# haidog-yaqub/EzAudio

Hardware: AMD Instinct MI355X
Metric: denoising steps/sec (EzAudio-XL, 10 s latent, CFG on) (higher is better)
Workload: dtype bf16

## Files before the change

ezaudio_amd/build.py:

```python
import concurrent.futures
import os
import subprocess
import sys

HERE = os.path.dirname(os.path.abspath(__file__))
CSRC = os.path.join(HERE, 'csrc')
OBJ = os.path.join(HERE, 'csrc', 'build')
LIB = os.path.join(HERE, 'libezaudio_hip.so')
SOURCES = ['gemm.hip', 'attn.hip', 'rowops.hip', 'api.hip', 'vae.hip', 't5.hip']
FLAGS = ['--offload-arch=gfx950', '-O3', '-std=c++17', '-fPIC', '-Wall', '-Wno-unused-function']
if os.environ.get('EZAUDIO_ABLATE'):
    FLAGS.append('-DEZ_ABLATE')
if os.environ.get('EZAUDIO_DIAG'):
    FLAGS.append('-DEZ_DIAG')


def source_hash():
    import hashlib
    h = hashlib.sha256()
    files = sorted(os.path.join(CSRC, f) for f in os.listdir(CSRC) if f.endswith(('.hip', '.h')))
    files.append(os.path.join(HERE, '..', 'include', 'ezdit.h'))
    for f in files:
        h.update(os.path.basename(f).encode())
        with open(f, 'rb') as fh:
            h.update(fh.read())
    return h.hexdigest()[:16]


def _hipcc():
    for cand in (os.environ.get('HIPCC'), '/opt/rocm/bin/hipcc', 'hipcc'):
        if cand and (os.path.isabs(cand) and os.path.exists(cand) or not os.path.isabs(cand)):
            return cand
    raise RuntimeError('hipcc not found')


def _stale(target, deps):
    if not os.path.exists(target):
        return True
    t = os.path.getmtime(target)
    return any(os.path.getmtime(d) > t for d in deps)


def build(force=False, verbose=True):
    os.makedirs(OBJ, exist_ok=True)
    headers = [os.path.join(CSRC, f) for f in sorted(os.listdir(CSRC)) if f.endswith('.h')] + [os.path.join(HERE, '..', 'include', 'ezdit.h')]
    hipcc = _hipcc()
    jobs = []
    for src in SOURCES:
        s = os.path.join(CSRC, src)
        o = os.path.join(OBJ, src.replace('.hip', '.o'))
        if force or _stale(o, [s] + headers):
            jobs.append((s, o))

    def compile_one(job):
        s, o = job
        cmd = [hipcc] + FLAGS + ['-c', s, '-o', o]
        r = subprocess.run(cmd, capture_output=True, text=True)
        return job, r

    if jobs:
        with concurrent.futures.ThreadPoolExecutor(max_workers=len(jobs)) as ex:
            for (s, o), r in ex.map(compile_one, jobs):
                if verbose and r.stderr.strip():
                    sys.stderr.write(r.stderr)
                if r.returncode != 0:
                    raise RuntimeError(f'hipcc failed on {s}:\n{r.stderr}')
    objs = [os.path.join(OBJ, s.replace('.hip', '.o')) for s in SOURCES]
    if force or jobs or _stale(LIB, objs):
        cmd = [hipcc, '--offload-arch=gfx950', '-shared', '-fPIC', '-o', LIB] + objs
        r = subprocess.run(cmd, capture_output=True, text=True)
        if r.returncode != 0:
            raise RuntimeError(f'link failed:\n{r.stderr}')
    return LIB


if __name__ == '__main__':
    print(build(force='--force' in sys.argv))
```

ezaudio_amd/csrc/api.hip:

```cpp
#include "../../include/ezdit.h"
#include "common.h"

#include <cmath>
#include <cstdarg>
#include <cstdio>
#include <cstring>
#include <map>
#include <string>
#include <vector>

static thread_local std::string g_err;

int ez_fail(int code, const char* fmt, ...) {
    char buf[512];
    va_list ap;
    va_start(ap, fmt);
    vsnprintf(buf, sizeof buf, fmt, ap);
    va_end(ap);
    g_err = buf;
    return code;
}
#define fail ez_fail

namespace {

#define HIPCHK(expr)                                                                            \
    do {                                                                                        \
        hipError_t e_ = (expr);                                                                 \
        if (e_ != hipSuccess) return fail(EZDIT_E_HIP, "%s failed: %s", #expr, hipGetErrorString(e_)); \
    } while (0)

inline long rup(long x, long a) { return (x + a - 1) / a * a; }

struct Buf {
    size_t off = 0, bytes = 0;
};

}

struct WRef {
    const bf16_t* W = nullptr; int ld = 0; int rows = 0;
};
struct BlkW {
    const float *bskip, *aqnw, *aqnb, *aknw, *aknb, *bo, *n2w, *n2b, *cqnw, *cqnb, *bo2, *b1, *b2, *snw, *snb, *zb;
    WRef wskip, wqkv, wo, wq2, wo2, w1, w2, zw;
};
struct WsPtrs {
    int* ints; float *rope_cos, *rope_sin, *coef, *cfgpart;
    bf16_t* ape; float *h, *skips; bf16_t *u, *ucat; float* qkv; bf16_t *q, *k, *v, *ao, *act; float *part, *y, *pred;
    uint8_t* kmask; bf16_t *kc, *vc; float *mod, *modf;
    float *cembed, *cnres; bf16_t* skipbf;
    float2* zstat; float *zt_qkv, *zt_geglu, *zt_q2;
    float2* zstat_skip; float* zt_skip; bf16_t* ucat_z;
    float* spc;
    float* zd;
};

static void drop_graph(ezdit_handle* h);

template <typename T>
struct Table {
    bool on = false;
    std::vector<T> host;
    T* dev = nullptr;
    const T* read() const { return on ? dev : nullptr; }
    void set(ezdit_handle* owner, bool to, bool rearm = false) {
        if (to != on || (to && rearm)) drop_graph(owner);
        on = to;
    }
};

static unsigned long long* g_gemm_ts = nullptr;
static long g_gemm_ts_cap = 0;

struct ezdit_handle {
    ezdit_config cfg;
    int D, H, dh, nblk, nhalf, I, C, Cin, Cctx, r6;
    int DQK, DV;
    int ldD, ld2D, ldI, ldPE, ldCtx;
    float scaling;

    std::vector<ezdit_param_info_t> params;
    std::map<std::string, int> pidx;
    size_t param_bytes = 0;
    const char* wblob = nullptr;

    char* ws = nullptr;
    size_t ws_bytes = 0;
    int B = 0, L = 0, Lc = 0, n_slots = 0, M = 0, Mp = 0, Lp = 0, Lcp = 0, Mc = 0;
    std::map<std::string, Buf> bufs;
    bool ctx_ready = false, ts_ready = false, cond_ready = false;
    bool z_tables_ready = false;
    bool skip_tables_ready = false;
    int n_ts = 0, per_row = 0;

    float* latents = nullptr;
    const float* noise = nullptr;
    const float* s_gt = nullptr;
    const uint8_t* s_gt_mask = nullptr;
    int P = 0, n_steps = 0;
    float gscale = 0.f, grescale = 0.f;
    hipGraphExec_t graph_exec = nullptr;
    hipGraph_t graph = nullptr;

    Table<int> lens;
    const int* lens_dev() const { return lens.read(); }
    Table<float> cns;
    Table<float> tl;
    int2* tlsup = nullptr;
    int tl_S = 0;
    Table<float> sp;
    static int sp_cap(int B) { return B / 2 + 1; }
    Table<float> coef;
    float* ms_hist = nullptr;
    Table<int> start;
    int start_min = 0;
    Table<int> canvas;
    int canvas_T = 0, canvas_ramp = 1;
    bool canvas_loop = false;
    Table<float> cw;
    int cw_K = 1;

    int launches = 0;
    bool is_cn = false;
    int c0 = 0, c0m = 0, c1 = 0;
    ezdit_handle* cn = nullptr;
    float cn_scale = 1.0f;
    float fwd_cn_scale = 1.0f;
    std::vector<ezdit_handle*> cn_users;
    const float* ext_mask_embed = nullptr;
    static constexpr int kSplitK = 3, kTileF32 = 25, kTilePE = 70, kTileFin = 73;
    static constexpr int kTilePartialBig = 60, kSplitBig = 2, kZTile = 70, kZBigM = 2048;
    int opt_tile_partial = 9;
    int opt_gemm_pp = 3;
    int opt_zfuse = 1;
    int opt_skip_z = 1;
    bool skip_z_usable() const { return opt_skip_z && !is_cn && nhalf > 0 && zparts() <= (ztile() == kZTile ? 16 : 8); }
    int opt_geglu_co = 0;
    int opt_qkv_co = 1;
    int opt_qkv_form = 1;
    int qkv_tile() const { return (opt_qkv_co == 2 || (opt_qkv_co == 1 && M > kCoM)) ? 66 : (opt_qkv_form == 1 && M <= kCoM) ? 67 : 61; }
    static constexpr int kCoM = 2048;
    int geglu_tile() const { return !(opt_gemm_pp & 1) ? 13 : (opt_geglu_co == 2 || (opt_geglu_co == 1 && M > kCoM)) ? 66 : 60; }
    int opt_xkey1 = 1;
    bool xkey1 = false;
    int act_b0 = 0, act_b1 = 0;
#ifdef EZ_DIAG
    int opt_zfake = 0;
#endif
    bool qk_perm() const { return D % (2 * dh) == 0; }
    int qkv_mode() const { return qk_perm() ? 2 : 0; }
    bool q2_fused(int nb) const { return opt_fuse_q2 && ((long)nb * H * ((L + 63) / 64) <= 512 || opt_fuse_q2 == 2) && Lcp % 128 == 0; }
    bool zfuse_usable() const {
        return opt_zfuse && zparts() <= Z_MAXP && (opt_gemm_pp & 1) && qkv_mode() == 2 && (q2_fused(B) || opt_q2_pp);
    }
    int ztile() const { return (M > kZBigM && !per_row) ? 61 : kZTile; }
    int zwidth() const { return ztile() == 61 ? 144 : 96; }
    int zparts() const { return (D + zwidth() - 1) / zwidth(); }
    struct ZTab { float *G, *C; long slot_stride; };
    static long ztab_floats(int items, long N) { return (long)items * 2 * N; }
    static ZTab ztab(float* base, int item, long N, long slot_stride) { float* G = base + ztab_floats(item, N); return {G, G + N, slot_stride}; }
    ZTab zt_qkv_of(int b) const { return ztab(p.zt_qkv, b, 3L * D, ztab_floats(nblk, 3L * D)); }
    ZTab zt_geglu_of(int b) const { return ztab(p.zt_geglu, b, 2L * I, ztab_floats(nblk, 2L * I)); }
    ZTab zt_q2_of(int b) const { return ztab(p.zt_q2, b, D, 0); }
    ZTab zt_skip_of(int j) const { return ztab(p.zt_skip, j, D, 0); }
    static size_t zrange(long Mp_) { return (size_t)Z_MAXP * Mp_; }
    float2* zstat_xhalf() const { return p.zstat + zrange(Mp); }
    float2* zstat_skip_of(int i) const { return p.zstat_skip + (size_t)i * zrange(Mp); }
    size_t ucat_elems(long Mp_) const { return (size_t)Mp_ * ld2D; }
    bf16_t* ucat_of(int j) const { return p.ucat_z + (size_t)j * ucat_elems(Mp); }
    int opt_wt = 2;
    int wt() const { return opt_wt == 2 ? (B * L <= 2048) : opt_wt; }
    int opt_fuse_q2 = 1;
    int opt_attn_nkh = 0;
    int opt_q2_pp = 1;
// ... 116 lines not shown
        const long c0 = h->c0, c0m = h->c0m, c1 = h->c1, ci = h->cfg.cond_in;
        add_param(h, "cn.cin.w", {"controlnet_pre.conv_in.weight"}, F, c0, ci);
        add_param(h, "cn.cin.b", {"controlnet_pre.conv_in.bias"}, F, 1, c0);
        if (h->cfg.cond_mask) add_param(h, "cn.mask_embed", {"controlnet_pre.mask_embed"}, F, 1, c0);
        add_param(h, "cn.c0.w", {"controlnet_pre.blocks.0.0.weight"}, F, c0m, c0m * 3);
        add_param(h, "cn.c0.b", {"controlnet_pre.blocks.0.0.bias"}, F, 1, c0m);
        add_param(h, "cn.c1.w", {"controlnet_pre.blocks.0.2.weight"}, F, c1, c0m * 3);
        add_param(h, "cn.c1.b", {"controlnet_pre.blocks.0.2.bias"}, F, 1, c1);
        add_param(h, "cn.cout.w", {"controlnet_pre.conv_out.weight"}, F, D, c1);
        add_param(h, "cn.cout.b", {"controlnet_pre.conv_out.bias"}, F, 1, D);
        for (int b = 0; b < h->nblk; ++b) {
            char k[64];
            snprintf(k, sizeof k, "controlnet_zero_blocks.%d", b);
            add_param(h, bn(b, "zw"), {std::string(k) + ".weight"}, Bf, D, D);
            add_param(h, bn(b, "zb"), {std::string(k) + ".bias"}, F, 1, D);
        }
    }
    struct V { const char* name; const char* key; long n; };
    const V vecs[] = {
        {"n1w", "norm1.weight", D}, {"n1b", "norm1.bias", D}, {"n2w", "norm2.weight", D}, {"n2b", "norm2.bias", D},
        {"n3w", "norm3.weight", D}, {"n3b", "norm3.bias", D}, {"ncw", "norm_context.weight", D},
        {"ncb", "norm_context.bias", D},
        {"a.qnw", "attn.norm_q.weight", dh}, {"a.qnb", "attn.norm_q.bias", dh}, {"a.knw", "attn.norm_k.weight", dh},
        {"a.knb", "attn.norm_k.bias", dh}, {"c.qnw", "cross_attn.norm_q.weight", dh},
        {"c.qnb", "cross_attn.norm_q.bias", dh}, {"c.knw", "cross_attn.norm_k.weight", dh},
        {"c.knb", "cross_attn.norm_k.bias", dh},
        {"bo", "attn.proj.bias", D}, {"bo2", "cross_attn.proj.bias", D}, {"b2", "mlp.net.2.bias", D},
        {"table", "adaln.scale_shift_table", 6 * D},
    };
    for (const V& v : vecs)
        for (int b = 0; b < h->nblk; ++b) add_param(h, bn(b, v.name), {blk_prefix(h, b) + "." + v.key}, F, 1, v.n);
    for (int b = 0; b < h->nblk; ++b) {
        const std::string p = blk_prefix(h, b);
        add_param(h, bn(b, "b1"), {p + ".mlp.net.0.proj.bias"}, F, 1, 2 * I, EZDIT_T_GEGLU8);
        if (b > h->nhalf) {
            add_param(h, bn(b, "snw"), {p + ".skip_norm.weight"}, F, 1, 2 * D);
            add_param(h, bn(b, "snb"), {p + ".skip_norm.bias"}, F, 1, 2 * D);
            add_param(h, bn(b, "wskip"), {p + ".skip_linear.weight"}, Bf, D, 2 * D);
            add_param(h, bn(b, "bskip"), {p + ".skip_linear.bias"}, F, 1, D);
        }
        add_param(h, bn(b, "wqkv"), {p + ".attn.to_q.weight", p + ".attn.to_k.weight", p + ".attn.to_v.weight"}, Bf, 3 * D, D, h->qk_perm() ? EZDIT_T_QKROPE : EZDIT_T_NONE);
        add_param(h, bn(b, "wo"), {p + ".attn.proj.weight"}, Bf, D, D);
        add_param(h, bn(b, "wq2"), {p + ".cross_attn.to_q.weight"}, Bf, D, D);
        add_param(h, bn(b, "wo2"), {p + ".cross_attn.proj.weight"}, Bf, D, D);
        add_param(h, bn(b, "w1"), {p + ".mlp.net.0.proj.weight"}, Bf, 2 * I, D, EZDIT_T_GEGLU8);
        add_param(h, bn(b, "w2"), {p + ".mlp.net.2.weight"}, Bf, D, I);
    }
    for (int b = 0; b < h->nblk; ++b) {
        const std::string p = blk_prefix(h, b);
        add_param(h, bn(b, "wkv2"), {p + ".cross_attn.to_k.weight", p + ".cross_attn.to_v.weight"}, Bf, 2 * D, D);
        add_param(h, bn(b, "lora_a"), {p + ".adaln.lora_a.weight"}, F, r6, D);
        add_param(h, bn(b, "lora_b"), {p + ".adaln.lora_b.weight"}, F, 6 * D, r6);
    }
}

size_t carve(const ezdit_handle* h, int B, int L, int Lc, int n_slots, std::map<std::string, Buf>* out) {
    size_t off = 0;
    auto add = [&](const char* name, size_t bytes) {
        Buf b;
        b.off = off;
        b.bytes = bytes;
        if (out) (*out)[name] = b;
        off += (size_t)rup((long)bytes, 256);
    };
    const long D = h->D, C = h->C, H = h->H;
    const long M = (long)B * L, Mp = rup(M, 128), Lp = rup(L, 128), Lcp = rup(Lc, 128);
    const long Mc = (long)B * Lc, Mcp = rup(Mc, 128);
    const int nblk = h->nblk;
    add("ints", 256 * sizeof(int));
    add("rope_cos", (size_t)h->cfg.max_len * (h->dh / 2) * 4);
    add("rope_sin", (size_t)h->cfg.max_len * (h->dh / 2) * 4);
    add("coef", (size_t)(n_slots > 0 ? n_slots : 1) * 8 * 4);
    add("cfgpart", (size_t)B * 64 * 4 * 4);
    add("sink", 256);
    if (h->is_cn) {
        const long Lc2 = 2L * L;
        add("cn_e0", (size_t)B * h->c0 * Lc2 * 4);
        add("cn_e1", (size_t)B * h->c0m * Lc2 * 4);
        add("cn_e2", (size_t)B * h->c1 * L * 4);
        add("cembed", (size_t)rup((long)B * L, 128) * h->D * 4);
        add("cnres", (size_t)h->nhalf * rup((long)B * L, 128) * h->D * 4);
        add("skipbf", (size_t)rup((long)B * L, 128) * h->ldD * 2);
    }
    add("ape", Mp * h->ldPE * 2);
    add("h", Mp * D * 4);
    add("skips", (size_t)h->nhalf * Mp * D * 4);
    add("u", Mp * h->ldD * 2);
    add("ucat", Mp * h->ld2D * 2);
    add("qkv", Mp * 3 * D * 4);
    add("q", (size_t)B * H * Lp * h->DQK * 2);
    add("k", (size_t)B * H * Lp * h->DQK * 2);
    add("v", (size_t)B * H * Lp * h->DV * 2);
    add("ao", Mp * h->ldD * 2);
    add("act", Mp * h->ldI * 2);
    add("part", (size_t)8 * Mp * D * 4);
    add("y", Mp * C * 4);
    add("pred", (size_t)B * C * L * 4);
    add("kmask", rup(Mc, 256));
    add("ctx_bf", Mcp * h->ldCtx * 2);
    add("c1", Mcp * D * 4);
    add("c1b", Mcp * h->ldD * 2);
    add("c2", Mcp * D * 4);
    add("cu", Mcp * h->ldD * 2);
    add("ckv", Mcp * 2 * D * 4);
    add("kc", (size_t)nblk * B * H * Lcp * h->DQK * 2);
    add("vc", (size_t)nblk * B * H * Lcp * h->DV * 2);
    const long ns = n_slots > 0 ? n_slots : 1;
    add("ts", ns * 4);
    add("t1", ns * D * 4);
    add("tt", ns * D * 4);
    add("ada", ns * 6 * D * 4);
    add("adaf", ns * 2 * D * 4);
    add("la", ns * h->r6 * 4);
    add("lora", ns * nblk * 6 * D * 4);
    add("mod", ns * nblk * 6 * D * 4);
    add("modf", ns * 2 * D * 4);
    {
        const long I2 = 2L * h->I, N3 = 3L * D, nmax = I2 > N3 ? I2 : N3;
        const size_t zr = ezdit_handle::zrange(Mp), z64 = (size_t)Mp * ((2 * D + 63) / 64), nskip = h->nhalf > 0 ? h->nhalf : 1;
        add("zstat", (z64 > 2 * zr ? z64 : 2 * zr) * 8);
        add("zt_qkv", (size_t)ns * ezdit_handle::ztab_floats(nblk, N3) * 4);
        add("zt_geglu", (size_t)ns * ezdit_handle::ztab_floats(nblk, I2) * 4);
        add("zt_q2", (size_t)ezdit_handle::ztab_floats(nblk, D) * 4);
        add("zd", (size_t)nblk * B * D * 4);
        add("zA", (size_t)rup(4 * ns, 128) * h->ldD * 2);
        add("ztmp", (size_t)rup(4 * ns, 128) * nmax * 4);
#ifdef EZ_DIAG
        add("zneutral", zr * 8);
        add("zzeros", (size_t)nmax * 4);
#endif
        add("ucat_z", (h->is_cn ? 1 : nskip) * h->ucat_elems(Mp) * 2);
        add("zstat_skip", nskip * zr * 8);
        add("zt_skip", (size_t)ezdit_handle::ztab_floats((int)nskip, D) * 4);
        add("lens", 256 * sizeof(int));
        add("spg", (size_t)ezdit_handle::sp_cap(B) * 2 * 4);
        add("spc", (size_t)ns * ezdit_handle::sp_cap(B) * 8 * 4);
        add("cns", 256 * sizeof(float));
        add("start", 256 * sizeof(int));
        add("canvas", 256 * sizeof(int));
        add("tlb", (size_t)B * (Lcp / 128) * L * 4);
        add("tlsup", (size_t)B * (Lcp / 128) * 8);
        add("cw", (size_t)B * sizeof(float));
    }
    return off;
}

struct Ctx {
    ezdit_handle* h;
    hipStream_t st;
    const int* cur = nullptr; const int* row_slot = nullptr;
    hipError_t err = hipSuccess;
    int rc = EZDIT_OK;
    const char* where = nullptr;
    unsigned long long* stamps() const { return (g_gemm_ts && h->launches == h->opt_stamp_launch) ? g_gemm_ts : nullptr; }
    void launched(const char* what, int launch_rc = 0) {
        if (h->opt_trace_launches) fprintf(stderr, "launch %d %s\n", h->launches, what);
        h->launches++;
        if (launch_rc != 0 && rc == EZDIT_OK) { rc = launch_rc; where = what; }
        const hipError_t e = hipGetLastError();
        if (e != hipSuccess && err == hipSuccess) { err = e; where = what; }
    }
    bool bad() const { return err != hipSuccess || rc != EZDIT_OK; }
    int result() const {
        if (rc != EZDIT_OK) return fail(rc, "%s: configuration not supported by the HIP kernels", where ? where : "?");
        if (err != hipSuccess) return fail(EZDIT_E_HIP, "launch of %s failed: %s", where ? where : "?", hipGetErrorString(err));
        return EZDIT_OK;
    }
};

struct ZIn {
    ezdit_handle::ZTab t{};
    const float2* stat = nullptr;
    int row0 = 0, b0 = 0;
};

void gemm(Ctx& c, const bf16_t* A, int lda, const WRef& w, const float* bias, void* out, int ldo, int M, int N,
          int epi, int tile, const HeadNormArgs* hn = nullptr, const ZIn& z = ZIn{}, int splitk = 1, long slab = 0, bool panel = false) {
    ezdit_handle* h = c.h;
    GemmArgs g;
    memset(&g, 0, sizeof g);
    g.A = A;
    g.lda = lda;
    g.W = w.W;
    g.ldw = w.ld;
    g.wrows = w.rows;
    g.bias = bias;
    g.out = out;
    g.ldo = ldo;
    g.slab_stride = slab;
    g.M = M;
    g.N = N;
    g.K = w.ld;
    g.splitk = splitk;
    g.epi = epi;
    g.tile = tile;
    g.xcd_map = 1;
    g.part_bf16 = (epi == EPI_PARTIAL) ? 1 : 0;
    g.wt = h->wt();
    g.epi_lds = h->opt_epi_lds;
    g.rows_per_b = 1;
    if (hn) g.hn = *hn;
    g.xcd_panel = panel ? 1 : 0;
#ifdef EZ_DIAG
    if (!z.stat && h->opt_zfake && (epi == EPI_QKV || epi == EPI_GEGLU) && (tile == 60 || tile == 61 || tile == 66) && h->zparts() <= Z_MAXP) {
        g.zw = h->zwidth(); g.zstat_in = h->buf<float2>("zneutral"); g.zs_stride = h->Mp; g.zparts = h->zparts(); g.zD = h->D;
        g.zG = h->buf<float>("zzeros"); g.zC = bias ? bias : g.zG; g.zt_slot_stride = 0; g.zeps = 1e-5f; g.rows_per_b = h->L;
    }
#endif
    if (z.stat) {
        g.zw = h->zwidth(); g.zstat_in = z.stat + z.row0; g.zs_stride = h->Mp; g.zparts = h->zparts(); g.zD = h->D; g.zG = z.t.G; g.zC = z.t.C; g.zt_slot_stride = z.t.slot_stride; g.zeps = 1e-5f;
        g.cur_step = c.cur ? c.cur : h->p.ints; g.row_slot = c.cur ? c.row_slot : (h->per_row ? h->p.ints + 16 : nullptr); g.rows_per_b = h->L;
        if (g.row_slot) g.row_slot += z.b0;
    }
    g.ts = c.stamps(); g.ts_cap = g_gemm_ts_cap;
    c.launched(epi == EPI_GEGLU ? "k_gemm (GEGLU)" : epi == EPI_QKV ? "k_gemm (QKV)" : epi == EPI_PARTIAL ? "k_gemm (split-K slabs)" : "k_gemm", launch_gemm(g, c.st));
}

int tile_for(const ezdit_handle* h, int M, bool partial) {
    if (M <= 2048) return partial ? h->opt_tile_partial : ezdit_handle::kTileF32;
    return partial ? ezdit_handle::kTilePartialBig : ezdit_handle::kTileF32;
}

int pick_splitk(const ezdit_handle* h, int M, int N, int K) {
    const int tiles = ((M + 127) / 128) * ((N + 63) / 64);
    const int nk = K / 64;
    if (M > 2048) return ezdit_handle::kSplitBig < nk ? ezdit_handle::kSplitBig : nk;
    if (tiles >= 256) return 1;
    return ezdit_handle::kSplitK < nk ? ezdit_handle::kSplitK : nk;
}

int gemm_partial(Ctx& c, const bf16_t* A, int lda, const WRef& w, int M, int N) {
    ezdit_handle* h = c.h;
    const int K = w.ld;
    const int s = pick_splitk(h, M, N, K);
    const int shape_bit = K >= 4 * N ? 4 : K >= 2 * N ? 2 : 1;
    const bool panel = (h->opt_gemm_panel & shape_bit) && M <= 1024;
    gemm(c, A, lda, w, nullptr, h->p.part, h->D, M, N, EPI_PARTIAL, tile_for(h, M, true), nullptr, ZIn{}, s, (long)h->Mp * h->D, panel);
    return s;
}

GemmArgs resid_args(int tile, const bf16_t* A, int lda, const bf16_t* W, int ldw, int wrows, const float* bias, const float* h_in, const float* gate, const float* zg,
                    float* h_out, bf16_t* zu, int ld_zu, float2* zstat_out, long zs_stride, int M, int N, int K) {
    GemmArgs g;
    memset(&g, 0, sizeof g);
    g.A = A; g.lda = lda; g.W = W; g.ldw = ldw; g.wrows = wrows; g.bias = bias;
    g.out = h_out; g.ldo = N; g.M = M; g.N = N; g.K = K; g.splitk = 1; g.epi = EPI_RESID; g.tile = tile; g.xcd_map = 1;
    g.resid = h_in; g.ldr = N; g.gate = gate; g.rows_per_b = 1;
    g.zu = zu; g.ld_zu = ld_zu; g.zg = zg; g.zstat_out = zstat_out; g.zs_stride = zs_stride;
    return g;
}

struct Edge {
    const char* name = nullptr;
    bool algebra = false;
    const bf16_t* A = nullptr; int lda = 0; const WRef* w = nullptr; const float* bias = nullptr;
    const float* h_in = nullptr; float* h_out = nullptr;
    const float* gate = nullptr; long gate_stride = 0;
    const float *ln_g = nullptr, *ln_c = nullptr; long ln_stride = 0;
    int b0 = 0, nb = -1;
    int dual_blk = -1;
    bf16_t* zu = nullptr; int ld_zu = 0;
    float2* zstat_out = nullptr;
    bf16_t* zu2 = nullptr; int ld_zu2 = 0; const float* zg2 = nullptr;
    const float2 *zin = nullptr, *zin2 = nullptr; const float* zG = nullptr;
    const float *skip = nullptr, *cn = nullptr;
};

void resolve_weights(ezdit_handle* h) {
    h->blk.assign(h->nblk, BlkW{});
    for (int b = 0; b < h->nblk; ++b) {
        BlkW& k = h->blk[b];
        k.aqnw = h->w<float>(bn(b, "a.qnw")); k.aqnb = h->w<float>(bn(b, "a.qnb"));
        k.aknw = h->w<float>(bn(b, "a.knw")); k.aknb = h->w<float>(bn(b, "a.knb"));
        k.cqnw = h->w<float>(bn(b, "c.qnw")); k.cqnb = h->w<float>(bn(b, "c.qnb"));
        k.bo = h->w<float>(bn(b, "bo")); k.bo2 = h->w<float>(bn(b, "bo2")); k.b2 = h->w<float>(bn(b, "b2"));
        k.n2w = h->w<float>(bn(b, "n2w")); k.n2b = h->w<float>(bn(b, "n2b"));
        k.b1 = h->w<float>(bn(b, "b1"));
        k.wqkv = h->wref(bn(b, "wqkv")); k.wo = h->wref(bn(b, "wo")); k.wq2 = h->wref(bn(b, "wq2"));
        k.wo2 = h->wref(bn(b, "wo2")); k.w1 = h->wref(bn(b, "w1")); k.w2 = h->wref(bn(b, "w2"));
        if (!h->is_cn && b > h->nhalf) {
            k.snw = h->w<float>(bn(b, "snw")); k.snb = h->w<float>(bn(b, "snb"));
            k.wskip = h->wref(bn(b, "wskip")); k.bskip = h->w<float>(bn(b, "bskip"));
        }
        if (h->is_cn) { k.zw = h->wref(bn(b, "zw")); k.zb = h->w<float>(bn(b, "zb")); }
    }
    h->w_pe = h->wref("pe.w"); h->b_pe = h->w<float>("pe.b");
    if (!h->is_cn) {
        h->w_fin = h->wref("fin.w"); h->b_fin = h->w<float>("fin.b");
        h->w_fin_cw = h->w<float>("fin.cw"); h->w_fin_cb = h->w<float>("fin.cb");
        h->w_mask_embed = h->w<float>("mask_embed");
    }
}

void resolve_workspace(ezdit_handle* h) {
    WsPtrs& p = h->p;
    memset(&p, 0, sizeof p);
    p.ints = h->buf<int>("ints"); p.rope_cos = h->buf<float>("rope_cos"); p.rope_sin = h->buf<float>("rope_sin");
    p.coef = h->buf<float>("coef"); p.cfgpart = h->buf<float>("cfgpart");
    p.ape = h->buf<bf16_t>("ape"); p.h = h->buf<float>("h"); p.skips = h->buf<float>("skips"); p.u = h->buf<bf16_t>("u"); p.ucat = h->buf<bf16_t>("ucat");
    p.qkv = h->buf<float>("qkv"); p.q = h->buf<bf16_t>("q"); p.k = h->buf<bf16_t>("k"); p.v = h->buf<bf16_t>("v");
    p.ao = h->buf<bf16_t>("ao"); p.act = h->buf<bf16_t>("act"); p.part = h->buf<float>("part"); p.y = h->buf<float>("y");
    p.pred = h->buf<float>("pred"); p.kmask = h->buf<uint8_t>("kmask"); p.kc = h->buf<bf16_t>("kc"); p.vc = h->buf<bf16_t>("vc");
    p.mod = h->buf<float>("mod"); p.modf = h->buf<float>("modf");
    p.zd = h->buf<float>("zd"); p.spc = h->buf<float>("spc");
    h->lens.dev = h->buf<int>("lens"); h->cns.dev = h->buf<float>("cns"); h->sp.dev = h->buf<float>("spg"); h->coef.dev = p.coef;
    h->start.dev = h->buf<int>("start"); h->canvas.dev = h->buf<int>("canvas");
    h->tl.dev = h->buf<float>("tlb"); h->tlsup = h->buf<int2>("tlsup");
    h->cw.dev = h->buf<float>("cw");
    p.zstat = h->buf<float2>("zstat"); p.zt_qkv = h->buf<float>("zt_qkv"); p.zt_geglu = h->buf<float>("zt_geglu"); p.zt_q2 = h->buf<float>("zt_q2");
    p.zstat_skip = h->buf<float2>("zstat_skip"); p.zt_skip = h->buf<float>("zt_skip"); p.ucat_z = h->buf<bf16_t>("ucat_z");
    if (h->is_cn) { p.cembed = h->buf<float>("cembed"); p.cnres = h->buf<float>("cnres"); p.skipbf = h->buf<bf16_t>("skipbf"); }
}

template <typename Launch>
int hook_launch(const char* kernel, const char* config, Launch launch) {
    (void)hipGetLastError();
    if (launch()) return fail(EZDIT_E_UNSUPPORTED, "%s not supported", config);
    const hipError_t e = hipGetLastError();
    if (e != hipSuccess) return fail(EZDIT_E_HIP, "launch of %s failed: %s", kernel, hipGetErrorString(e));
    return EZDIT_OK;
}

CfgDdimArgs standalone_step(const float* pred, float* latents, const float* noise, int P, int n, const int32_t* lens = nullptr, int L = 0) {
    CfgDdimArgs a;
    a.pred = pred; a.latents = latents; a.noise = noise;
    a.P = P; a.n = n;
    a.lens = lens; a.L = lens ? L : n;
    return a;
}

enum class Needs { Bound, BoundBackbone, Begun };

int setter_checks(const ezdit_handle* h, const char* fn, Needs needs, hipStream_t st) {
    if (!h) return fail(EZDIT_E_INVALID, "null handle");
    if (needs == Needs::BoundBackbone && h->is_cn) return fail(EZDIT_E_INVALID, "first argument must be a backbone handle");
    if (needs == Needs::Begun ? !h->latents : !h->ws) return fail(EZDIT_E_STATE, needs == Needs::Begun ? "ezdit_sampler_begin first" : "bind workspace first");
    hipStreamCaptureStatus cs = hipStreamCaptureStatusNone;
    if (hipStreamIsCapturing(st, &cs) != hipSuccess) { (void)hipGetLastError(); cs = hipStreamCaptureStatusNone; }
    if (cs != hipStreamCaptureStatusNone) return fail(EZDIT_E_STATE, "%s inside a stream capture (it uploads from host memory and waits)", fn);
    return EZDIT_OK;
}

template <typename T>
int upload_table(Table<T>& t, std::vector<T> v, hipStream_t st, size_t head = 0, T* tail = nullptr) {
    HIPCHK(hipStreamSynchronize(st));
    t.host.swap(v);
    if (!tail) head = t.host.size();
    HIPCHK(hipMemcpyAsync(t.dev, t.host.data(), head * sizeof(T), hipMemcpyHostToDevice, st));
    if (tail) HIPCHK(hipMemcpyAsync(tail, t.host.data() + head, (t.host.size() - head) * sizeof(T), hipMemcpyHostToDevice, st));
    HIPCHK(hipStreamSynchronize(st));
    return EZDIT_OK;
}

template <typename T>
std::vector<T> per_row(const T* src, int n, int B) {
    std::vector<T> v((size_t)B);
    for (int b = 0; b < B; ++b) v[b] = src[b % n];
    return v;
}

int expand_lengths(const ezdit_handle* h, const int32_t* lengths, int n, std::vector<int>* v) {
    if (n < 0 || n > h->B || h->B % n) return fail(EZDIT_E_INVALID, "%d lengths do not divide B = %d", n, h->B);
    for (int i = 0; i < n; ++i)
        if (lengths[i] < 1 || lengths[i] > h->L) return fail(EZDIT_E_INVALID, "lengths[%d] = %d outside [1, L = %d]", i, (int)lengths[i], h->L);
    *v = per_row<int>(lengths, n, h->B);
    return EZDIT_OK;
}

int timeline_table(const float* w, int B, int S, int L, const int* lens, const uint8_t* mask, std::vector<float>* out) {
    const size_t nb = (size_t)B * S * L;
    out->assign(nb + (size_t)B * S * 2, 0.f);
    std::vector<int> sup((size_t)B * S * 2, 0);
    for (int b = 0; b < B; ++b) {
        const int len = lens ? lens[b] : L;
        bool has_key[TL_MAXS];
        for (int s = 0; s < S; ++s) {
            has_key[s] = !mask;
            for (int j = 0; mask && j < 128 && !has_key[s]; ++j) has_key[s] = mask[((size_t)b * S + s) * 128 + j] != 0;
        }
        for (int i = 0; i < L; ++i) {
            const int f = i < len ? i : len - 1;
            double mx = 0.0;
            bool seen = false;
            for (int s = 0; s < S; ++s) {
                const float x = w[((size_t)b * S + s) * L + f];
                if (!std::isfinite(x) || x < 0.f) return fail(EZDIT_E_INVALID, "weights[%d][%d][%d] = %g: a weight is finite and >= 0", b, s, f, (double)x);
                mx = x > mx ? x : mx;
                seen = seen || (x > 0.f && has_key[s]);
            }
            if (!seen) return fail(EZDIT_E_INVALID, "frame %d of batch element %d weights no prompt that has a valid key", f, b);
            for (int s = 0; s < S; ++s) {
                const float x = w[((size_t)b * S + s) * L + f];
                (*out)[((size_t)b * S + s) * L + i] = x > 0.f ? (float)std::log2((double)x / mx) : TL_OFF;
                if (x > 0.f) {
                    int* fs = &sup[((size_t)b * S + s) * 2];
                    if (fs[1] == 0) fs[0] = i;
                    fs[1] = i + 1;
                }
            }
        }
    }
    memcpy(out->data() + nb, sup.data(), sup.size() * sizeof(int));
    return EZDIT_OK;
}

void clear_cn_lengths(ezdit_handle* cn) {
    if (cn->lens.on) cn->cond_ready = false;
    cn->lens.set(cn, false);
    cn->lens.host.clear();
}

void reset_call_state(ezdit_handle* h) {
    h->sp.set(h, false);
    h->coef.set(h, false); h->ms_hist = nullptr;
    h->start.set(h, false); h->start_min = 0;
    h->canvas.set(h, false); h->canvas_loop = false;
    h->cw.set(h, false); h->cw_K = 1;
}

int check_compose_weights(const float* w, int P, int K) {
    for (int p = 0; p < P; ++p)
        for (int k = 0; k < K; ++k) {
            const float x = w[(size_t)p * K + k];
            if (!std::isfinite(x)) return fail(EZDIT_E_INVALID, "weights[%d][%d] is not finite", p, k);
            if (k == 0 && !(x > 0.f)) return fail(EZDIT_E_INVALID, "weights[%d][0] = %g: the primary condition's weight is above 0", p, (double)x);
        }
    return EZDIT_OK;
}

void reset_bind_state(ezdit_handle* h) {
    h->lens.set(h, false); h->lens.host.clear();
    h->cns.set(h, false);
    h->tl.set(h, false); h->tl.host.clear(); h->tl_S = 0;
    h->coef.host.clear();
    h->latents = nullptr; h->noise = nullptr; h->s_gt = nullptr; h->s_gt_mask = nullptr;
    h->P = 0; h->n_steps = 0;
    drop_graph(h);
}

}

extern "C" {

int ezdit_abi_version(void) { return EZDIT_ABI_VERSION; }
const char* ezdit_last_error(void) { return g_err.c_str(); }

int ezdit_create(const ezdit_config* cfg, ezdit_handle** out) {
    if (!cfg || !out) return fail(EZDIT_E_INVALID, "null argument");
    if (cfg->embed_dim <= 0 || cfg->num_heads <= 0 || cfg->embed_dim % cfg->num_heads)
        return fail(EZDIT_E_INVALID, "embed_dim %d not divisible by num_heads %d", cfg->embed_dim, cfg->num_heads);
    const int dh = cfg->embed_dim / cfg->num_heads;
    if (dh != 64 && dh != 72) return fail(EZDIT_E_UNSUPPORTED, "head_dim %d: only 64 and 72 are implemented", dh);
    if (cfg->embed_dim > 1280 || cfg->embed_dim % 4) return fail(EZDIT_E_UNSUPPORTED, "embed_dim %d > 1280", cfg->embed_dim);
    if (cfg->in_chans != 2 * cfg->out_chans + 1)
        return fail(EZDIT_E_UNSUPPORTED, "in_chans %d != 2*out_chans+1 (MaskDiT concat)", cfg->in_chans);
    if (cfg->depth < 2 || cfg->depth % 2) return fail(EZDIT_E_UNSUPPORTED, "depth %d must be even", cfg->depth);
    if (cfg->mlp_ratio != 4.0f) return fail(EZDIT_E_UNSUPPORTED, "mlp_ratio %g", (double)cfg->mlp_ratio);
    ezdit_handle* h = new ezdit_handle();
    h->cfg = *cfg;
    if (h->cfg.max_len <= 0) h->cfg.max_len = 2048;
    h->D = cfg->embed_dim;
    h->H = cfg->num_heads;
    h->dh = dh;
    h->nhalf = cfg->depth / 2;
    h->is_cn = cfg->controlnet != 0;
    h->nblk = h->is_cn ? cfg->depth / 2 : cfg->depth + 1;
    if (h->is_cn) {
        if (cfg->cond_in <= 0 || cfg->cond_c0 <= 0 || cfg->cond_c1 <= 0) {
            delete h;
            return fail(EZDIT_E_INVALID, "controlnet needs cond_in / cond_blocks");
// ... 1542 lines not shown
```

ezaudio_amd/csrc/common.h:

```cpp
#pragma once
#include <hip/hip_runtime.h>
#include <stdint.h>

typedef __attribute__((ext_vector_type(8))) __bf16 bf16x8;
typedef __attribute__((ext_vector_type(4))) __bf16 bf16x4;
typedef __attribute__((ext_vector_type(16))) float f32x16;
typedef __attribute__((ext_vector_type(2))) float f32x2;
typedef __attribute__((ext_vector_type(4))) float f32x4;
typedef uint16_t bf16_t;

#define EZ_WAVE 64

typedef __attribute__((ext_vector_type(2))) __bf16 bf16x2;
__device__ __forceinline__ uint16_t f2bf(float f) { return __builtin_bit_cast(uint16_t, (__bf16)f); }
__device__ __forceinline__ float bf2f(uint16_t b) { return __uint_as_float(((uint32_t)b) << 16); }
__device__ __forceinline__ uint32_t pack_bf2(float lo, float hi) {
    bf16x2 v;
    v[0] = (__bf16)lo;
    v[1] = (__bf16)hi;
    return __builtin_bit_cast(uint32_t, v);
}

__device__ __forceinline__ void st16_wt(void* p, float4 v) {
    f32x4 x = {v.x, v.y, v.z, v.w};
    asm volatile("global_store_dwordx4 %0, %1, off sc1\n\ts_nop 1" ::"v"(p), "v"(x) : "memory");
}
typedef __attribute__((ext_vector_type(2))) unsigned u32x2_t;
__device__ __forceinline__ void st8_wt(void* p, uint2 v) {
    u32x2_t x = {v.x, v.y};
    asm volatile("global_store_dwordx2 %0, %1, off sc1\n\ts_nop 1" ::"v"(p), "v"(x) : "memory");
}
__device__ __forceinline__ void st4_wt(void* p, uint32_t v) {
    asm volatile("global_store_dword %0, %1, off sc1\n\ts_nop 0" ::"v"(p), "v"(v) : "memory");
}

__device__ __forceinline__ float wave_sum(float v) {
#pragma unroll
    for (int o = 32; o > 0; o >>= 1) v += __shfl_xor(v, o, 64);
    return v;
}

__device__ __forceinline__ unsigned long long ez_stamp_start() {
    const unsigned hw = __builtin_amdgcn_s_getreg((31 << 11) | 4), xcc = __builtin_amdgcn_s_getreg((31 << 11) | 20);
    const unsigned long long id = ((unsigned long long)(xcc & 15u) << 8) | ((hw >> 8) & 255u);
    return (__builtin_amdgcn_s_memrealtime() & 0xffffffffffffull) | (id << 48);
}

inline unsigned ez_magic(int d) { return d <= 1 ? 0u : (unsigned)((0x100000000ull + (unsigned)d - 1) / (unsigned)d); }
__device__ __forceinline__ int ez_div(int x, unsigned m) { return m ? (int)__umulhi((unsigned)x, m) : x; }


int ez_fail(int code, const char* fmt, ...);

enum GemmEpi {
    EPI_F32 = 0,
    EPI_PARTIAL = 1,
    EPI_GEGLU = 2,
    EPI_RESID = 4,
    EPI_QKV = 3
};

constexpr int BK = 64;
constexpr int Z_MAXP = 12;

constexpr int Z_PT = Z_MAXP / 4;
static_assert(Z_PT * 4 == Z_MAXP, "four threads per row");
struct ZStatRegs { float2 v[Z_PT]; };
__device__ __forceinline__ float quad_xor1(float x) { return __builtin_bit_cast(float, __builtin_amdgcn_update_dpp(0, __builtin_bit_cast(int, x), 0xB1, 0xF, 0xF, true)); }
__device__ __forceinline__ float quad_xor2(float x) { return __builtin_bit_cast(float, __builtin_amdgcn_update_dpp(0, __builtin_bit_cast(int, x), 0x4E, 0xF, 0xF, true)); }
__device__ __forceinline__ float oct_sum(float s) {
    s += quad_xor1(s);
    s += quad_xor2(s);
    return s + __builtin_bit_cast(float, __builtin_amdgcn_update_dpp(0, __builtin_bit_cast(int, s), 0x141, 0xF, 0xF, true));
}
__device__ __forceinline__ uint32_t quad_xor1_u32(uint32_t x) { return (uint32_t)__builtin_amdgcn_update_dpp(0, (int)x, 0xB1, 0xF, 0xF, true); }
__device__ __forceinline__ void z_row_stats_load(const float2* __restrict__ st , long stride, int parts, int pg, ZStatRegs& z) {
#pragma unroll
    for (int k = 0; k < Z_PT; ++k) {
        const int p = pg + 4 * k;
        z.v[k] = st[(p < parts ? p : parts - 1) * stride];
    }
}
__device__ __forceinline__ float2 z_row_stats_finish(ZStatRegs& z, int parts, int pg, int D, float eps) {
#pragma unroll
    for (int k = 0; k < Z_PT; ++k) asm volatile("" : "+v"(z.v[k].x), "+v"(z.v[k].y));
    const float inv_d = __builtin_amdgcn_rcpf((float)D);
    float s = 0.f, q = 0.f;
#pragma unroll
    for (int k = 0; k < Z_PT; ++k) {
        const bool on = pg + 4 * k < parts;
        s += on ? z.v[k].x : 0.f;
        q += on ? z.v[k].y : 0.f;
    }
    s += quad_xor1(s); s += quad_xor2(s);
    q += quad_xor1(q); q += quad_xor2(q);
    const float mu = s * inv_d;
    const float var = fmaxf(fmaf(q, inv_d, -mu * mu), 0.f);
    return make_float2(mu, rsqrtf(var + eps));
}

template <int ROWS, int NT>
__device__ __forceinline__ void stage_offsets(uint32_t (&off)[(ROWS * 8 + NT - 1) / NT], int ld, int row0, int max_row, int tid) {
#pragma unroll
    for (int i = 0; i < (ROWS * 8 + NT - 1) / NT; ++i) {
        const int q = i * NT + tid;
        const int row = q >> 3;
        const int c = q & 7;
        int grow = row0 + row;
        grow = grow < max_row ? grow : max_row;
        const int gc = c ^ ((row >> 1) & 7);
        off[i] = (uint32_t)(grow * ld + gc * 8) * 2u;
    }
}

template <int ROWS, int NT>
__device__ __forceinline__ void stage_tile(const char* __restrict__ gbase ,
                                           const uint32_t (&off)[(ROWS * 8 + NT - 1) / NT], char* lds_wave , int tid) {
#pragma unroll
    for (int i = 0; i < (ROWS * 8 + NT - 1) / NT; ++i) {
        if ((ROWS * 8) % NT != 0 && i * NT + tid >= ROWS * 8) break;
        __builtin_amdgcn_global_load_lds((const __attribute__((address_space(1))) void*)(gbase + off[i]),
                                         (__attribute__((address_space(3))) void*)(lds_wave + i * NT * 16), 16, 0, 0);
    }
}


struct HeadNormArgs {
    const float* x; int ldx;
    int q_col, k_col, v_col;
    const float* qn_w; const float* qn_b; const float* kn_w; const float* kn_b;
    const float* rope_cos; const float* rope_sin;
    bf16_t* q; bf16_t* k; bf16_t* v;
    int B, H, L, Lp, dh;
    int perm;
};

struct RowArgs {
    const float* h_in; float* h_out;
    const float* part; int nsplit; long part_stride; int ld_part;
    int part_bf16;
    const float* bias;
    const float* gate; long gate_slot_stride;
    int mode;
    const float* ln_g; const float* ln_c; long ln_slot_stride;
    float cn_scale;
    const float* skip; const float* cn;
    bf16_t* u; int ld_u;
    int M, D, L;
    const int* cur_step; const int* row_slot;
    int wt;
    int variant;
    int affine;
    const float* cn_tab;
};

struct GemmArgs {
    const bf16_t* A; int lda;
    const bf16_t* W; int ldw;
    int wrows;
    const float* bias;
    void* out; int ldo;
    long slab_stride;
    int M, N, K;
    int splitk;
    int epi;
    int tile;
    int debug;
    int conv_cpb; long conv_tap_bytes;
    const float* resid; int ldr;
    const float* gate; long gate_slot_stride; const int* cur_step; const int* row_slot; int rows_per_b;
    int xcd_map; int pm, pn, pz, bm, bn, bz;
    unsigned mbm, mbn, msplit, mG;
    int wt;
    HeadNormArgs hn;
    int part_bf16;
    int xcd_panel;
    bf16_t* zu; int ld_zu;
    const float* zg; long zg_slot_stride;
    float2* zstat_out;
    long zs_stride;
    const float* zd; long zd_stride; const float* zg2; long zg2_slot_stride; int act_row0, act_row1;
    const float2* zstat_in; int zparts; int zD; int zw;
    const float* zG; const float* zC; long zt_slot_stride;
    float zeps;
    unsigned long long* ts;
    long ts_cap;
    int epi_lds;
    bf16_t* zu2; int ld_zu2;
    const float2* zstat_in2;
};
int launch_gemm(const GemmArgs& a, hipStream_t st);

struct AttnArgs {
    const bf16_t* q;
    const bf16_t* k;
    const bf16_t* v;
    const uint8_t* kmask;
    bf16_t* out; int ldo;
    int B, H, Lq, Lk, Lqp, Lkp, dh;
    const float* q_raw; int ld_qraw; const float* qn_w; const float* qn_b;
    int nkh;
    const bf16_t* xu; int ldu; const bf16_t* xw; int ldw; int xw_rows; int xK;
    int xcd_map; int nq, ppx;
    unsigned mnq, mH;
    int wt;
// ... 109 lines not shown
```

ezaudio_amd/csrc/gemm.hip:

```cpp
#include "common.h"
#include "gemm_pp.h"
#include "gemm_ks.h"
#include "gemm_co.h"

#include <atomic>
#include <type_traits>

namespace {

template <int PER, int MAXY>
__device__ __forceinline__ void wait_tiles(int younger) {
    if constexpr (MAXY >= 5) { if (younger >= 5) { wait_vmcnt<5 * PER>(); return; } }
    if constexpr (MAXY >= 4) { if (younger >= 4) { wait_vmcnt<4 * PER>(); return; } }
    if constexpr (MAXY >= 3) { if (younger >= 3) { wait_vmcnt<3 * PER>(); return; } }
    if constexpr (MAXY >= 2) { if (younger >= 2) { wait_vmcnt<2 * PER>(); return; } }
    if constexpr (MAXY >= 1) { if (younger >= 1) { wait_vmcnt<PER>(); return; } }
    wait_vmcnt<0>();
}

template <int FM, int FN, int TM, int TN, int EPI>
__device__ __forceinline__ void store_tile(const GemmArgs& a, f32x16 (&acc)[FM][FN], int row0, int col0, int wm, int wn, int lane, int z) {
    const int row_in = lane & 31, hi = lane >> 5;
    if constexpr (EPI == EPI_GEGLU) {
        bf16_t* out = reinterpret_cast<bf16_t*>(a.out);
// ... 149 lines not shown
    constexpr int TM = BM / WM, TN = BN / WN;
    constexpr int FM = TM / 32, FN = TN / 32;
    constexpr int A_BYTES = BM * 128, B_BYTES = BN * 128;
    constexpr int STAGE_BYTES = A_BYTES + B_BYTES;
    extern __shared__ __attribute__((aligned(16))) char smem[];

    const int tid = threadIdx.x;
    const int lane = tid & 63;
    const int wave = tid >> 6;
    const int wm = wave / WN, wn = wave % WN;

    const int tilesM = (a.M + BM - 1) / BM;
    const int tilesN = (a.N + BN - 1) / BN;
    int tm, tn, z;
    if (EPI == EPI_PARTIAL && a.xcd_panel) {
        panel_of_block(a, tilesN, tm, tn, z);
        if (tm >= tilesM) return;
    } else if (!tile_of_block(a, tilesM, tilesN, tm, tn, z)) return;
    const int row0 = tm * BM, col0 = tn * BN;

    const int nk = a.K / BK;
    int kb, ke;
    ksplit_range(a, nk, z, kb, ke);
    const int nt = ke - kb;

    f32x16 acc[FM][FN];
#pragma unroll
    for (int i = 0; i < FM; ++i)
#pragma unroll
        for (int j = 0; j < FN; ++j)
#pragma unroll
            for (int r = 0; r < 16; ++r) acc[i][j][r] = 0.f;

    uint32_t aoff[(BM * 8 + NT - 1) / NT], boff[(BN * 8 + NT - 1) / NT];
    stage_offsets<BM, NT>(aoff, a.lda, row0, a.M - 1, tid);
    stage_offsets<BN, NT>(boff, a.ldw, col0, a.wrows - 1, tid);
    const int wave_u = __builtin_amdgcn_readfirstlane(wave);
    const char* gA = reinterpret_cast<const char*>(a.A);
    const char* gW = reinterpret_cast<const char*>(a.W) + (long)kb * BK * 2;
    auto stage = [&](int t) {
        char* dst = smem + (t % NS) * STAGE_BYTES + wave_u * 1024;
        const long a_off = a.conv_cpb ? (long)((kb + t) / a.conv_cpb) * a.conv_tap_bytes + (long)((kb + t) % a.conv_cpb) * (BK * 2)
                                      : (long)(kb + t) * (BK * 2);
        stage_tile<BM, NT>(gA + a_off, aoff, dst, tid);
        stage_tile<BN, NT>(gW + t * (BK * 2), boff, dst + A_BYTES, tid);
    };
#pragma unroll
    for (int t = 0; t < NS - 1; ++t)
        if (t < nt) stage(t);

    const int r32 = lane & 31, hi = lane >> 5;
    uint32_t foff[4];
#pragma unroll
    for (int ks = 0; ks < 4; ++ks) foff[ks] = r32 * 128 + (((2 * ks + hi) ^ ((r32 >> 1) & 7)) << 4);
    const int a_base = wm * TM * 128, b_base = A_BYTES + wn * TN * 128;

    auto wait_landed = [&](int t) {
        const int younger = nt - 1 - t;
        if constexpr (((BM + BN) * 8) % NT != 0) {
            constexpr int REM_WAVES = (((BM * 8) % NT) + ((BN * 8) % NT)) / 64;
            static_assert(((BM * 8) % NT == 0) || ((BN * 8) % NT == 0), "at most one ragged operand");
            constexpr int LO = (BM * 8) / NT + (BN * 8) / NT;
            static_assert(NS <= 3, "ragged staging supports rings up to 3");
            if (NS >= 3 && younger >= 1) {
                if (wave_u < REM_WAVES) wait_vmcnt<LO + 1>(); else wait_vmcnt<LO>();
            } else {
                wait_vmcnt<0>();
            }
        } else {
            constexpr int MAXY = NS - 2 < 5 ? NS - 2 : 5;
            static_assert(MAXY * LPT < 64, "ring too deep for the 6-bit vmcnt");
            wait_tiles<LPT, MAXY>(younger);
        }
    };
    auto tile_top = [&](int t) {
        wait_landed(t);
        __builtin_amdgcn_s_barrier();
    };
    auto ktile = [&](int t, auto RF) {
        constexpr bool rf = decltype(RF)::value;
        f32x16 (&acc_r)[FM][FN] = acc;
        const char* cT = smem + (t % NS) * STAGE_BYTES;
        if constexpr (rf) stage(t + NS - 1);
        bf16x8 af[2][FM], bfr[2][FN];
#pragma unroll
        for (int i = 0; i < FM; ++i) af[0][i] = *reinterpret_cast<const bf16x8*>(cT + foff[0] + a_base + i * 4096);
#pragma unroll
        for (int j = 0; j < FN; ++j) bfr[0][j] = *reinterpret_cast<const bf16x8*>(cT + foff[0] + b_base + j * 4096);
        __builtin_amdgcn_sched_group_barrier(0x100, FM + FN, 0);
#pragma unroll
        for (int ks = 0; ks < 4; ++ks) {
            if (ks < 3) {
#pragma unroll
                for (int i = 0; i < FM; ++i)
                    af[(ks + 1) & 1][i] = *reinterpret_cast<const bf16x8*>(cT + foff[ks + 1] + a_base + i * 4096);
#pragma unroll
                for (int j = 0; j < FN; ++j)
                    bfr[(ks + 1) & 1][j] = *reinterpret_cast<const bf16x8*>(cT + foff[ks + 1] + b_base + j * 4096);
            }
#pragma unroll
            for (int i = 0; i < FM; ++i)
#pragma unroll
                for (int j = 0; j < FN; ++j)
                    acc[i][j] = __builtin_amdgcn_mfma_f32_32x32x16_bf16(bfr[ks & 1][j], af[ks & 1][i], acc[i][j], 0, 0, 0);
            if (ks < 3) __builtin_amdgcn_sched_group_barrier(0x100, FM + FN, 0);
            __builtin_amdgcn_sched_group_barrier(0x008, FM * FN, 0);
        }
#pragma unroll
        for (int i = 0; i < FM; ++i)
#pragma unroll
            for (int j = 0; j < FN; ++j) asm volatile("" : "+a"(acc_r[i][j]));
    };
    const int nt_refill = nt - (NS - 1) > 0 ? nt - (NS - 1) : 0;
    {
        int t = 0;
        for (; t < nt_refill; ++t) { tile_top(t); ktile(t, std::true_type{}); }
        for (; t < nt; ++t) { tile_top(t); ktile(t, std::false_type{}); }
    }

    {
        constexpr bool lds_ok = (EPI == EPI_GEGLU || EPI == EPI_PARTIAL) && BM * ((EPI == EPI_GEGLU ? BN / 2 : BN) + 8) * 2 <= NS * STAGE_BYTES;
        if constexpr (lds_ok) {
            if (a.epi_lds && (EPI == EPI_GEGLU || a.part_bf16)) {
                store_tile_lds<BM, BN, FM, FN, TM, TN, NT, EPI>(a, acc, smem, row0, col0, wm, wn, lane, tid, z);
                return;
            }
        }
        store_tile<FM, FN, TM, TN, EPI>(a, acc, row0, col0, wm, wn, lane, z);
    }
}

int pick_boxes(GemmArgs& a, int BM, int BN) {
    const int tilesM = (a.M + BM - 1) / BM;
    const int tilesN = (a.N + BN - 1) / BN;
    const int S = a.splitk;
    double best = 1e30;
    for (int pm = 1; pm <= 8; pm *= 2)
        for (int pn = 1; pm * pn <= 8; pn *= 2) {
            const int pz = 8 / (pm * pn);
            if (pz > S && pz != 1) continue;
            if (a.xcd_map == 0 && !(pm == 1 && pn == 8)) continue;
            const int bm = (tilesM + pm - 1) / pm, bn = (tilesN + pn - 1) / pn, bz = (S + pz - 1) / pz;
            const double rows = (double)(bm * BM < a.M ? bm * BM : a.M) + (double)(bn * BN < a.N ? bn * BN : a.N);
            double fp = rows * ((double)a.K * bz / S) * 2.0;
            const int slots = bm * bn * bz * 8, work = tilesM * tilesN * S;
            fp *= (double)slots / work;
            if (pm == 1 && pn == 8) fp *= 0.9;
            if (fp < best) { best = fp; a.pm = pm; a.pn = pn; a.pz = pz; a.bm = bm; a.bn = bn; a.bz = bz; }
        }
    a.mbm = ez_magic(a.bm); a.mbn = ez_magic(a.bn); a.msplit = ez_magic(a.splitk); a.mG = ez_magic(((a.N + BN - 1) / BN) * a.splitk);
    return 8 * a.bm * a.bn * a.bz;
}

template <int BM, int BN, int WM, int WN, int NS, int EPI, int SCHED, int VAR = 0>
int launch_pp(const GemmArgs& a0, hipStream_t st) {
    GemmArgs a = a0;
    dim3 grid(pick_boxes(a, BM, BN), 1, 1);
    if (EPI == EPI_PARTIAL && a.xcd_panel && BM == 128) grid.x = 8 * ((a.N + BN - 1) / BN) * a.splitk * (((a.M + BM - 1) / BM + 7) / 8);
    else a.xcd_panel = 0;
    constexpr int SMEM = pp_smem_bytes<BM, BN, NS, EPI>();
    static_assert(SMEM <= 160 * 1024, "LDS budget of a CU");
    static std::atomic<bool> attr_set[32];
    int dev = 0;
    (void)hipGetDevice(&dev);
    if (dev < 0 || dev >= 32) return 1;
    if (!attr_set[dev].load(std::memory_order_acquire)) {
        if (hipFuncSetAttribute(reinterpret_cast<const void*>(k_gemm_pp<BM, BN, WM, WN, NS, EPI, SCHED, VAR>),
                                hipFuncAttributeMaxDynamicSharedMemorySize, SMEM) != hipSuccess) return 1;
        attr_set[dev].store(true, std::memory_order_release);
    }
    if (a.ts && (long)grid.x > a.ts_cap) a.ts = nullptr;
    hipLaunchKernelGGL((k_gemm_pp<BM, BN, WM, WN, NS, EPI, SCHED, VAR>), grid, dim3(512), SMEM, st, a);
    return 0;
}

template <int BM, int BN, int EPI, int VAR = 0>
int launch_co(const GemmArgs& a0, hipStream_t st) {
    GemmArgs a = a0;
    a.xcd_panel = 0;
    dim3 grid(pick_boxes(a, BM, BN), 1, 1);
    constexpr int SMEM = co_smem_bytes<BM, BN>();
    static std::atomic<bool> attr_set[32];
    int dev = 0;
    (void)hipGetDevice(&dev);
    if (dev < 0 || dev >= 32) return 1;
    if (!attr_set[dev].load(std::memory_order_acquire)) {
        if (hipFuncSetAttribute(reinterpret_cast<const void*>(k_gemm_co<BM, BN, EPI, VAR>), hipFuncAttributeMaxDynamicSharedMemorySize, SMEM) != hipSuccess) return 1;
        attr_set[dev].store(true, std::memory_order_release);
    }
    if (a.ts && (long)grid.x > a.ts_cap) a.ts = nullptr;
    hipLaunchKernelGGL((k_gemm_co<BM, BN, EPI, VAR>), grid, dim3(256), SMEM, st, a);
    return 0;
}

template <int FM, int FN, int EPI, bool GATE, bool RES, int CK, int X = KS_PLAIN>
int launch_ks(const GemmArgs& a0, hipStream_t st) {
    GemmArgs a = a0;
    a.xcd_panel = 0; a.splitk = 1;
    constexpr int BM = 16 * FM, BN = 16 * FN;
    (void)pick_boxes(a, BM, BN);
    const int tilesM = (a.M + BM - 1) / BM, tilesN = (a.N + BN - 1) / BN;
    const int gw = a.bn < tilesN ? a.bn : tilesN;
    dim3 grid(8 * ((tilesM * gw + a.pm - 1) / a.pm), 1, 1);
    constexpr int SMEM = 8 * (BM + BN) * 128;
    static_assert(SMEM <= 160 * 1024, "LDS budget of a CU");
    static std::atomic<bool> attr_set[32];
    int dev = 0;
    (void)hipGetDevice(&dev);
    if (dev < 0 || dev >= 32) return 1;
    if (!attr_set[dev].load(std::memory_order_acquire)) {
        if (hipFuncSetAttribute(reinterpret_cast<const void*>(k_gemm_ks<FM, FN, EPI, GATE, RES, CK, X>),
                                hipFuncAttributeMaxDynamicSharedMemorySize, SMEM) != hipSuccess) return 1;
        attr_set[dev].store(true, std::memory_order_release);
    }
    if (a.ts && (long)grid.x > a.ts_cap) a.ts = nullptr;
    hipLaunchKernelGGL((k_gemm_ks<FM, FN, EPI, GATE, RES, CK, X>), grid, dim3(512), SMEM, st, a);
    return 0;
}
template <int EPI, bool GATE, bool RES>
int launch_ks_tile(const GemmArgs& a, hipStream_t st) {
    switch (a.tile) {
        case 70: return launch_ks<3, 6, EPI, GATE, RES, 64>(a, st);
        case 72: return launch_ks<2, 6, EPI, GATE, RES, 64>(a, st);
        case 73: return launch_ks<3, 4, EPI, GATE, RES, 64>(a, st);
        default: return 1;
    }
}

template <int BM, int BN, int WM, int WN, int NS, int EPI>
int launch_t(const GemmArgs& a0, hipStream_t st) {
    GemmArgs a = a0;
    const int tilesM = (a.M + BM - 1) / BM;
    const int tilesN = (a.N + BN - 1) / BN;
    const int S = a.splitk;
    dim3 grid(pick_boxes(a, BM, BN), 1, 1);
    if (EPI == EPI_PARTIAL && a.xcd_panel) grid.x = 8 * tilesN * S * ((tilesM + 7) / 8);
    else a.xcd_panel = 0;
    constexpr int SMEM = NS * (BM + BN) * 128;
    static_assert(SMEM <= 160 * 1024, "LDS budget of a CU");
    static std::atomic<bool> attr_set[32];
    int dev = 0;
    (void)hipGetDevice(&dev);
    if (dev < 0 || dev >= 32) return 1;
    if (!attr_set[dev].load(std::memory_order_acquire)) {
        if (hipFuncSetAttribute(reinterpret_cast<const void*>(k_gemm<BM, BN, WM, WN, NS, EPI>),
                                hipFuncAttributeMaxDynamicSharedMemorySize, SMEM) != hipSuccess) return 1;
        attr_set[dev].store(true, std::memory_order_release);
    }
    hipLaunchKernelGGL((k_gemm<BM, BN, WM, WN, NS, EPI>), grid, dim3(64 * WM * WN), SMEM, st, a);
    return 0;
}

template <int EPI>
int launch_e(const GemmArgs& a, hipStream_t st) {
#ifdef EZ_ABLATE
#define EZ_PP_ABL(BM_, BN_, WM_, WN_, NS_, SC_)                                                    \
            case 8: return launch_pp<BM_, BN_, WM_, WN_, NS_, EPI, SC_, 8>(a, st);                \
            case 16: return launch_pp<BM_, BN_, WM_, WN_, NS_, EPI, SC_, 16>(a, st);              \
            case 32: return launch_pp<BM_, BN_, WM_, WN_, NS_, EPI, SC_, 32>(a, st);              \
            case 24: return launch_pp<BM_, BN_, WM_, WN_, NS_, EPI, SC_, 24>(a, st);              \
            case 40: return launch_pp<BM_, BN_, WM_, WN_, NS_, EPI, SC_, 40>(a, st);              \
            case 48: return launch_pp<BM_, BN_, WM_, WN_, NS_, EPI, SC_, 48>(a, st);              \
            case 56: return launch_pp<BM_, BN_, WM_, WN_, NS_, EPI, SC_, 56>(a, st);
#else
#define EZ_PP_ABL(BM_, BN_, WM_, WN_, NS_, SC_)
#endif
#define EZ_PP(BM_, BN_, WM_, WN_, NS_, SC_)                                                        \
        switch (a.debug >> 8) {                                                                    \
            case 0: return launch_pp<BM_, BN_, WM_, WN_, NS_, EPI, SC_, 0>(a, st);                \
            EZ_PP_ABL(BM_, BN_, WM_, WN_, NS_, SC_)                                                \
            default: return 1;                                                                     \
        }
    switch (a.tile) {
        case 6: return launch_t<128, 64, 4, 1, 2, EPI>(a, st);
        case 9: return launch_t<128, 128, 4, 2, 3, EPI>(a, st);
        case 13: return launch_t<128, 288, 4, 3, 3, EPI>(a, st);
        case 25: return launch_t<128, 64, 4, 2, 4, EPI>(a, st);
        case 60: EZ_PP(128, 288, 4, 2, 3, 1)
        case 61: EZ_PP(128, 144, 4, 1, 4, 2)
        case 62: EZ_PP(128, 128, 4, 2, 3, 1)
        case 66:
            if constexpr (EPI == EPI_GEGLU) {
                if ((a.debug >> 8) == 1) return launch_co<128, 144, EPI, 1>(a, st);
                if ((a.debug >> 8) == 2) return launch_co<128, 144, EPI, 2>(a, st);
            }
            return launch_co<128, 144, EPI>(a, st);
        default: break;
    }
#undef EZ_PP
#undef EZ_PP_ABL
    return 1;
}

}

int launch_gemm(const GemmArgs& a, hipStream_t st) {
    if (a.K <= 0 || a.K % BK) return 1;
    if (a.epi == EPI_QKV && a.tile >= 60) {
        if (a.zstat_in && !(a.zG && a.zC && a.zparts > 0 && a.zparts <= Z_MAXP && a.zs_stride > 0 && a.zw > 0)) return 1;
        if (a.tile == 66) {
            if (!a.hn.perm) return 1;
            if (a.hn.dh == 72) return a.zstat_in ? launch_co<128, 144, EPI_QKV, 64>(a, st) : launch_co<128, 144, EPI_QKV, 0>(a, st);
            if (a.hn.dh == 64) return a.zstat_in ? launch_co<128, 128, EPI_QKV, 64>(a, st) : launch_co<128, 128, EPI_QKV, 0>(a, st);
            return 1;
        }
        if (a.tile == 67) {
            if (!a.hn.perm) return 1;
            if (a.hn.dh == 72) return a.zstat_in ? launch_pp<128, 144, 8, 1, 4, EPI_QKV, 1, 64>(a, st) : launch_pp<128, 144, 8, 1, 4, EPI_QKV, 1>(a, st);
            if (a.hn.dh == 64) return a.zstat_in ? launch_pp<128, 128, 8, 1, 4, EPI_QKV, 1, 64>(a, st) : launch_pp<128, 128, 8, 1, 4, EPI_QKV, 1>(a, st);
            return 1;
        }
        if (a.hn.dh == 72) return a.zstat_in ? launch_pp<128, 144, 4, 1, 4, EPI_QKV, 2, 64>(a, st) : launch_pp<128, 144, 4, 1, 4, EPI_QKV, 2>(a, st);
        if (a.hn.dh == 64) return a.zstat_in ? launch_pp<128, 128, 4, 1, 4, EPI_QKV, 2, 64>(a, st) : launch_pp<128, 128, 4, 1, 4, EPI_QKV, 2>(a, st);
        return 1;
    }
    if (a.epi == EPI_QKV) return 1;
    if (a.epi == EPI_RESID && a.tile >= 70) {
        if (!a.zu || !a.zg || !a.zstat_out || a.zs_stride <= 0 || !a.bias || a.splitk != 1 || (a.gate && !a.resid)) return 1;
        if (a.zd) {
            if (!a.gate || !a.zg2 || a.tile != 70 || a.rows_per_b <= 0) return 1;
            return launch_ks<3, 6, EPI_RESID, true, true, 64, KS_DUAL>(a, st);
        }
        if (a.zu2) {
            if (!a.gate || !a.zg2 || a.tile != 70 || a.ld_zu2 <= 0) return 1;
            return launch_ks<3, 6, EPI_RESID, true, true, 64, KS_COPY2>(a, st);
        }
        if (a.zstat_in2) {
            if (a.gate || a.resid || a.tile != 70 || !a.zstat_in || !a.zG || a.zparts <= 0 || a.zparts > 16 || a.zD <= 0) return 1;
            return launch_ks<3, 6, EPI_RESID, false, false, 64, KS_ZIN>(a, st);
        }
        if (a.gate) return launch_ks_tile<EPI_RESID, true, true>(a, st);
        if (a.resid) return launch_ks_tile<EPI_RESID, false, true>(a, st);
        return launch_ks_tile<EPI_RESID, false, false>(a, st);
    }
    if (a.epi == EPI_F32 && a.tile >= 70 && a.tile < 80) {
        if (a.resid || a.conv_cpb) return 1;
        return launch_ks_tile<EPI_F32, false, false>(a, st);
    }
    if (a.epi == EPI_RESID && a.tile == 61) {
        if (!a.zu || !a.zg || !a.zstat_out || a.zs_stride <= 0 || !a.bias || a.splitk != 1 || (a.gate && !a.resid) || a.row_slot) return 1;
        if (a.zd) {
            if (!a.gate || !a.zg2 || a.rows_per_b <= 0) return 1;
            return launch_pp<128, 144, 4, 1, 4, EPI_RESID, 2, 64 + 128 + 256>(a, st);
        }
        if (a.zu2) {
            if (!a.gate || !a.zg2 || a.ld_zu2 <= 0) return 1;
            return launch_pp<128, 144, 4, 1, 4, EPI_RESID, 2, 64 + 128 + 512>(a, st);
        }
        if (a.zstat_in2) {
            if (a.gate || a.resid || !a.zstat_in || !a.zG || a.zparts <= 0 || a.zparts > 8 || a.zD <= 0) return 1;
            return launch_pp<128, 144, 4, 1, 4, EPI_RESID, 2, 1024>(a, st);
        }
        if (a.gate) return launch_pp<128, 144, 4, 1, 4, EPI_RESID, 2, 64 + 128>(a, st);
        if (a.resid) return launch_pp<128, 144, 4, 1, 4, EPI_RESID, 2, 128>(a, st);
        return launch_pp<128, 144, 4, 1, 4, EPI_RESID, 2, 0>(a, st);
    }
    if (a.epi == EPI_RESID) return 1;
    if (a.epi == EPI_GEGLU && a.zstat_in) {
        if ((a.tile != 60 && a.tile != 66) || !(a.zG && a.zC && a.zparts > 0 && a.zparts <= Z_MAXP && a.zs_stride > 0 && a.zw > 0)) return 1;
        if (a.tile == 66) return launch_co<128, 144, EPI_GEGLU, 64>(a, st);
        return launch_pp<128, 288, 4, 2, 3, EPI_GEGLU, 1, 64>(a, st);
    }
    if (a.epi == EPI_GEGLU) return launch_e<EPI_GEGLU>(a, st);
    if (a.epi == EPI_PARTIAL) return launch_e<EPI_PARTIAL>(a, st);
    if (a.epi == EPI_F32) return launch_e<EPI_F32>(a, st);
    return 1;
}
```

ezaudio_amd/csrc/gemm_co.h:

```cpp
#pragma once
#include "gemm_pp.h"

namespace {

template <int BM, int BN>
constexpr int co_smem_bytes() {
    return 2 * ((BM + BN + 31) / 32) * 4096 + BM * 8 + 2 * BN * 4 + 1024;
}

template <int BM, int BN, int EPI, int VAR>
__global__ __launch_bounds__(256, 2) void k_gemm_co(GemmArgs a) {
    constexpr int NT = 256;
    constexpr int WM = 4, TM = BM / WM, TN = BN, FM = TM / 16, FN = TN / 16;
    static_assert(TM * WM == BM && TM % 16 == 0 && TN % 16 == 0, "tile geometry: four waves, each TM rows x the whole tile width");
    constexpr int NP = (BM + BN + 31) / 32;
    constexpr int PA = BM / 32;
    constexpr int STAGE = NP * 4096;
    static_assert(BM % 32 == 0, "whole A pieces");
    static_assert(2 * co_smem_bytes<BM, BN>() <= 160 * 1024, "TWO workgroups per CU");
    static_assert(NP < 32, "vmcnt range");
    extern __shared__ __attribute__((aligned(16))) char smem[];

    int M_ = a.M;
    asm("" : "+s"(M_) : "s"(a.A), "s"(a.W), "s"(a.lda), "s"(a.ldw), "s"(a.wrows), "s"(a.N), "s"(a.K), "s"(a.splitk), "s"(a.pm), "s"(a.pn), "s"(a.bm), "s"(a.bn), "s"(a.bz),
        "s"(a.cur_step), "s"(a.ts), "s"(a.row_slot), "s"(a.mbm), "s"(a.mbn), "s"(a.msplit));
    const int slot0 = a.cur_step ? *a.cur_step : 0;
    const float *zG_ = a.zG, *zC_ = a.zC;
    asm("" : "+s"(M_), "+s"(zG_), "+s"(zC_));
    const int tid = threadIdx.x;
    const int lane = tid & 63;
    const int wave = __builtin_amdgcn_readfirstlane(tid >> 6);
    const int wm = wave;

    const int tilesM = (M_ + BM - 1) / BM;
    const int tilesN = (a.N + BN - 1) / BN;
    int tm, tn, z;
    if (!tile_of_block(a, tilesM, tilesN, tm, tn, z)) return;
    const int row0 = tm * BM, col0 = tn * BN;
    const int nk = a.K / BK;
    int kb, ke;
    ksplit_range(a, nk, z, kb, ke);
    const int nt = ke - kb;

    constexpr bool ZM = (VAR & 64) != 0 && (EPI == EPI_GEGLU || EPI == EPI_QKV);
    float* zgc = reinterpret_cast<float*>(smem + 2 * STAGE + BM * 8);
    constexpr int NZT = ZM ? FM * Z_PT : 0;
    ZLaneRegs<FM> zlr;
    const bool z_shared_slot = a.row_slot == nullptr;
    constexpr int ZNV = 2 * (BN / 4);
    const bool zx = ZM && z_shared_slot && wave * 64 < ZNV;
    auto z_late_load = [&]() {
        if constexpr (ZM) {
            static_assert(2 * (BN / 4) <= NT, "one float4 of G' or C' per thread");
            if (z_shared_slot && tid < ZNV) {
                const int which = tid >= BN / 4, t4 = tid - which * (BN / 4);
                int cp = col0 + 4 * t4;
                cp = cp < a.N - 4 ? cp : a.N - 4;
                __builtin_amdgcn_global_load_lds((const __attribute__((address_space(1))) void*)((which ? zC_ : zG_) + (long)slot0 * a.zt_slot_stride + cp),
                                                 (__attribute__((address_space(3))) void*)(reinterpret_cast<char*>(zgc) + wave * 1024), 16, 0, 0);
            }
            z_lane_load<FM>(a.zstat_in, a.zs_stride, a.zparts, row0 + wm * TM + (lane & 15), a.M - 1, lane >> 4, zlr);
        }
    };
    unsigned long long* ts = (a.ts && wave == 0) ? a.ts + 8 * (long)blockIdx.x : nullptr;
    if (ts && lane == 0) { ts[0] = __builtin_readcyclecounter(); ts[6] = ez_stamp_start(); }
    f32x4 acc[FM][FN];
#pragma unroll
    for (int i = 0; i < FM; ++i)
#pragma unroll
        for (int j = 0; j < FN; ++j) acc[i][j] = f32x4{0.f, 0.f, 0.f, 0.f};

    uint32_t poff[NP];
#pragma unroll
    for (int p = 0; p < NP; ++p) {
        const int q = p * NT + tid;
        const int row = q >> 3, c = q & 7;
        if (p < PA) {
            int grow = row0 + row;
            grow = grow < a.M ? grow : a.M - 1;
            poff[p] = (uint32_t)(grow * a.lda + ((c ^ ((row >> 1) & 7)) << 3)) * 2u;
        } else {
            const int r2 = row - BM;
            int gr = col0 + r2;
            gr = gr < a.wrows ? gr : a.wrows - 1;
            poff[p] = (uint32_t)(gr * a.ldw + ((c ^ ((r2 >> 1) & 7)) << 3)) * 2u;
        }
    }
    const char* gA = reinterpret_cast<const char*>(a.A) + (long)kb * (BK * 2);
    const char* gW = reinterpret_cast<const char*>(a.W) + (long)kb * (BK * 2);
    auto issue = [&](int t) {
        char* dst = smem + (t & 1) * STAGE + wave * 1024;
        const long koff = (long)t * (BK * 2);
#pragma unroll
        for (int p = 0; p < NP; ++p) {
            const char* src = (p < PA ? gA : gW) + koff + poff[p];
            __builtin_amdgcn_global_load_lds((const __attribute__((address_space(1))) void*)src,
                                             (__attribute__((address_space(3))) void*)(dst + p * 4096), 16, 0, 0);
        }
    };
    const int r16 = lane & 15, kq = lane >> 4;
    uint32_t foff[2];
#pragma unroll
    for (int ks = 0; ks < 2; ++ks) foff[ks] = r16 * 128 + (((4 * ks + kq) ^ (r16 >> 1)) << 4);
    const int a_base = wm * TM * 128, b_base = BM * 128;
    auto barrier = [&]() {
        __builtin_amdgcn_sched_barrier(0);
        __builtin_amdgcn_s_barrier();
        __builtin_amdgcn_sched_barrier(0);
    };

    if constexpr ((VAR & 3) != 0) {
        const unsigned lds_base = __builtin_amdgcn_s_getreg((7 << 11) | 6) ;
        if (lds_base != 0) {
            if constexpr ((VAR & 1) != 0) __builtin_amdgcn_s_sleep(12);
            if constexpr ((VAR & 2) != 0) { if (blockIdx.x < 512) { __builtin_amdgcn_s_sleep(100); __builtin_amdgcn_s_sleep(100); __builtin_amdgcn_s_sleep(100); } }
        }
    }
    issue(0);
    z_late_load();
    if (nt > 1) issue(1);
    if (nt > 1) { if (zx) wait_vmcnt<NP + NZT + 1>(); else wait_vmcnt<NP + NZT>(); } else wait_vmcnt<0>();
    barrier();
    if (ts && lane == 0) ts[1] = __builtin_readcyclecounter();
    auto step = [&](int t, auto MODE_) {
        constexpr int MODE = decltype(MODE_)::value;
        const char* cT = smem + (t & 1) * STAGE;
        bf16x8 af[FM][2], bfr[FN][2];
#pragma unroll
        for (int ks = 0; ks < 2; ++ks) {
#pragma unroll
            for (int i = 0; i < FM; ++i) af[i][ks] = *reinterpret_cast<const bf16x8*>(cT + foff[ks] + a_base + i * 2048);
#pragma unroll
            for (int j = 0; j < FN; ++j) bfr[j][ks] = *reinterpret_cast<const bf16x8*>(cT + foff[ks] + b_base + j * 2048);
        }
        __builtin_amdgcn_sched_barrier(0);
        asm volatile("s_waitcnt lgkmcnt(0)" ::: "memory");
        if constexpr (MODE == 2) {
            barrier();
            issue(t + 2);
        }
        __builtin_amdgcn_sched_barrier(0);
#pragma unroll
        for (int ks = 0; ks < 2; ++ks)
#pragma unroll
            for (int i = 0; i < FM; ++i)
#pragma unroll
                for (int j = 0; j < FN; ++j)
                    asm volatile("v_mfma_f32_16x16x32_bf16 %0, %1, %2, %0" : "+a"(acc[i][j]) : "v"(bfr[j][ks]), "v"(af[i][ks]));
        __builtin_amdgcn_sched_barrier(0);
        if constexpr (MODE >= 1) {
            if constexpr (MODE == 2) wait_vmcnt<NP>(); else wait_vmcnt<0>();
            barrier();
        }
    };
    {
        int t = 0;
        for (; t + 2 < nt; ++t) step(t, std::integral_constant<int, 2>{});
        if (t + 1 < nt) { step(t, std::integral_constant<int, 1>{}); ++t; }
        step(t, std::integral_constant<int, 0>{});
    }
    if (ts && lane == 0) ts[2] = __builtin_readcyclecounter();

#pragma unroll
    for (int i = 0; i < FM; ++i)
#pragma unroll
        for (int j = 0; j < FN; ++j) asm volatile("" : "+a"(acc[i][j]));
    asm volatile("s_nop 7\n\ts_nop 7\n\ts_nop 3" ::: "memory");
#pragma unroll
    for (int i = 0; i < FM; ++i)
#pragma unroll
        for (int j = 0; j < FN; ++j) asm volatile("" : "+a"(acc[i][j]));
    float2 zmr[FM];
    if constexpr (ZM) {
        asm volatile("s_waitcnt vmcnt(0)" ::: "memory");
        z_lane_finish<FM>(zlr, a.zparts, lane >> 4, a.zD, a.zeps, zmr);
    }
    if constexpr (EPI == EPI_QKV) {
        static_assert(BM * (BN + 8) * 2 <= 2 * STAGE, "bf16 staging tile must fit the ring");
        QkvOperands<BN / 2, FM> qop;
        qkv_request<BN / 2, FM>(a, col0, row0 + wm * TM + (lane & 15), lane, tid, qop);
        pp_store_qkv_reg<BM, BN, BN / 2, FM, FN, TM, TN, NT, ZM>(a, acc, smem, row0, col0, wm, lane, tid, zmr, zgc, reinterpret_cast<float*>(smem + 2 * STAGE + BM * 8 + 2 * BN * 4), slot0, qop, ts);
        if (ts && lane == 0) { asm volatile("s_waitcnt vmcnt(0)" ::: "memory"); ts[3] = __builtin_readcyclecounter(); ts[7] = __builtin_amdgcn_s_memrealtime(); }
        return;
    }
    if constexpr (EPI == EPI_GEGLU || EPI == EPI_PARTIAL) {
        static_assert(BM * ((EPI == EPI_GEGLU ? BN / 2 : BN) + 8) * 2 <= 2 * STAGE, "output tile must fit the ring");
        if (EPI == EPI_GEGLU || a.part_bf16) {
            pp_store_lds<BM, BN, FM, FN, TM, TN, NT, EPI, ZM>(a, acc, smem, row0, col0, wm, 0, lane, tid, z, zmr, zgc, slot0, ts);
            if (ts && lane == 0) { ts[3] = __builtin_readcyclecounter(); ts[7] = __builtin_amdgcn_s_memrealtime(); }
            return;
        }
    }
    if constexpr (EPI == EPI_F32 || EPI == EPI_PARTIAL) pp_store_direct<FM, FN, TM, TN, EPI>(a, acc, row0, col0, wm, 0, lane, z);
    if (ts && lane == 0) { asm volatile("s_waitcnt vmcnt(0)" ::: "memory"); ts[3] = __builtin_readcyclecounter(); ts[7] = __builtin_amdgcn_s_memrealtime(); }
}

}
```

ezaudio_amd/csrc/gemm_ks.h:

```cpp
#pragma once
#include "common.h"

namespace {

template <int SL>
struct KsOperands {
    f32x4 b[SL], r[SL], g[SL], z[SL];
    f32x2 st[4];
};
constexpr int KS_PLAIN = 0;
constexpr int KS_DUAL = 1;
constexpr int KS_COPY2 = 2;
constexpr int KS_ZIN = 3;
__device__ __forceinline__ f32x4 ks_ld16_agpr(const float* p) {
    f32x4 v;
    asm volatile("global_load_dwordx4 %0, %1, off" : "=a"(v) : "v"(p) : "memory");
    return v;
}
__device__ __forceinline__ f32x2 ks_ld8_agpr(const float2* p) {
    f32x2 v;
    asm volatile("global_load_dwordx2 %0, %1, off" : "=a"(v) : "v"(p) : "memory");
    return v;
}
template <int SL, int EPI, bool GATE, bool RES, int X>
__device__ __forceinline__ void ks_operands_wait(KsOperands<SL>& op) {
    if constexpr (X == KS_ZIN) asm volatile("s_waitcnt vmcnt(0)" : "+a"(op.st[0]), "+a"(op.st[1]), "+a"(op.st[2]), "+a"(op.st[3]));
#pragma unroll
    for (int q = 0; q < SL; ++q) {
        if constexpr (EPI == EPI_RESID) {
            if constexpr (X == KS_ZIN) asm volatile("s_waitcnt vmcnt(0)" : "+a"(op.b[q]), "+a"(op.g[q]), "+a"(op.z[q]));
            else if constexpr (GATE && RES) asm volatile("s_waitcnt vmcnt(0)" : "+a"(op.b[q]), "+a"(op.r[q]), "+a"(op.g[q]), "+a"(op.z[q]));
            else if constexpr (RES) asm volatile("s_waitcnt vmcnt(0)" : "+a"(op.b[q]), "+a"(op.r[q]), "+a"(op.z[q]));
            else asm volatile("s_waitcnt vmcnt(0)" : "+a"(op.b[q]), "+a"(op.z[q]));
        } else {
            asm volatile("s_waitcnt vmcnt(0)" : "+a"(op.b[q]));
        }
    }
}

template <int SL>
__device__ __forceinline__ int ks_slot_of(int q, int j) {
    constexpr int NP = SL / 2;
    return q < 2 * NP ? 16 * (q >> 1) + 2 * j + (q & 1) : 16 * NP + j;
}

__device__ __forceinline__ bool ks_tile_of_block(const GemmArgs& a, int tilesM, int tilesN, int& tm, int& tn) {
    const int xcd = blockIdx.x & 7, l = blockIdx.x >> 3;
    const int lpm = __builtin_ctz(a.pm);
    const int xm = xcd & (a.pm - 1), gn = xcd >> lpm;
    const int n0 = gn * a.bn;
    int gw = tilesN - n0;
    gw = gw < a.bn ? gw : a.bn;
    if (gw <= 0) return false;
    const int T = tilesM * gw, run = (T + a.pm - 1) >> lpm;
    const int t = xm * run + l;
    if (l >= run || t >= T) return false;
    tm = (int)(((float)t + 0.5f) * __builtin_amdgcn_rcpf((float)gw));
    tn = n0 + (t - tm * gw);
    return true;
}

template <int FM, int FN, int EPI, bool GATE, bool RES, int CK, int X = KS_PLAIN>
__global__ __launch_bounds__(512) void k_gemm_ks(GemmArgs a) {
    constexpr bool DUAL = X == KS_DUAL;
    static_assert(EPI == EPI_F32 || EPI == EPI_RESID, "epilogues");
    static_assert(!DUAL || (EPI == EPI_RESID && GATE && RES), "DUAL: the gated residual projection only");
    static_assert(X == KS_PLAIN || EPI == EPI_RESID, "forms of the residual epilogue");
    static_assert(X != KS_ZIN || (!GATE && !RES), "ZIN: the gate's register slot carries G'");
    static_assert(FN % 2 == 0 && FM >= 1 && FM <= 4, "tile geometry: 8 lanes per output row, FN / 2 column slots each");
    static_assert(CK == 64 || CK == 32, "chunk width");
    constexpr int BM = 16 * FM, BN = 16 * FN;
    constexpr int RPP = 1024 / (2 * CK);
    constexpr int LPR = 64 / RPP;
    constexpr int NPC = (BM + BN) / RPP;
    constexpr int PA = BM / RPP;
    static_assert(BM % RPP == 0 && BN % RPP == 0, "whole pieces");
    constexpr int NSL = 64 / CK;
    constexpr int CHUNK = (BM + BN) * 2 * CK;
    constexpr int SLOT = NSL * CHUNK;
    constexpr int KSTEPS = CK / 32;
    static_assert(BM * BN * 4 <= SLOT, "partial tile must fit the slot");
    static_assert(8 * SLOT <= 160 * 1024, "LDS budget of a CU");
    constexpr int SL = FN / 2;
    constexpr int S4 = BN / 4;
    extern __shared__ __attribute__((aligned(16))) char smem[];

    const int tid = threadIdx.x;
    const int lane = tid & 63;
    const int wave = __builtin_amdgcn_readfirstlane(tid >> 6);

    int M_ = a.M;
    asm("" : "+s"(M_) : "s"(a.A), "s"(a.W), "s"(a.lda), "s"(a.ldw), "s"(a.wrows), "s"(a.N), "s"(a.K), "s"(a.pm), "s"(a.bn), "s"(a.cur_step), "s"(a.ts), "s"(a.ts_cap),
        "s"(a.row_slot), "s"(a.bias), "s"(a.resid), "s"(a.ldr), "s"(a.gate), "s"(a.zg));
    int slot0 = 0;
    if constexpr (EPI == EPI_RESID) slot0 = a.cur_step ? *a.cur_step : 0;
    const int tilesM = (M_ + BM - 1) / BM;
    const int tilesN = (a.N + BN - 1) / BN;
    int tm, tn;
    if (!ks_tile_of_block(a, tilesM, tilesN, tm, tn)) return;
    const int row0 = tm * BM, col0 = tn * BN;
    const int nk = a.K / CK;
    unsigned long long* ts = (a.ts && wave == 0) ? a.ts + 8 * (long)blockIdx.x : nullptr;
    unsigned long long t_start = 0, t_sum = 0;
    if (ts && lane == 0) { t_start = __builtin_readcyclecounter(); ts[0] = t_start; ts[6] = ez_stamp_start(); }

    const int er = tid >> 3, ej = tid & 7;
    const bool epi_thread = tid < 8 * BM;
    int erow = row0 + er;
    const bool row_ok = epi_thread && erow < a.M;
    erow = erow < a.M ? erow : a.M - 1;
    const int ncl = a.N - 4;

    const char* gA = reinterpret_cast<const char*>(a.A);
    const char* gW = reinterpret_cast<const char*>(a.W);
    char* slot = smem + wave * SLOT;
    const int nmine = wave < nk ? (nk - wave + 7) / 8 : 0;
    uint32_t poff[NPC];
#pragma unroll
    for (int p = 0; p < NPC; ++p) {
        const int row = RPP * p + lane / LPR, c = lane % LPR;
        const int r2 = p < PA ? row : row - BM;
        const int gc = CK == 64 ? (c ^ ((r2 >> 1) & 7)) : (c ^ ((r2 >> 2) & 3));
        if (p < PA) {
            int grow = row0 + row;
            grow = grow < a.M ? grow : a.M - 1;
            poff[p] = (uint32_t)(grow * a.lda + (gc << 3)) * 2u;
        } else {
            int gr = col0 + r2;
            gr = gr < a.wrows ? gr : a.wrows - 1;
            poff[p] = (uint32_t)(gr * a.ldw + (gc << 3)) * 2u;
        }
        if (nmine > 0)
            __builtin_amdgcn_global_load_lds((const __attribute__((address_space(1))) void*)((p < PA ? gA : gW) + (long)wave * (CK * 2) + poff[p]),
                                             (__attribute__((address_space(3))) void*)(slot + p * 1024), 16, 0, 0);
    }
    auto issue = [&](int c, char* dst) {
        const long koff = (long)c * (CK * 2);
#pragma unroll
        for (int p = 0; p < NPC; ++p) {
            const char* src = (p < PA ? gA : gW) + koff + poff[p];
            __builtin_amdgcn_global_load_lds((const __attribute__((address_space(1))) void*)src,
                                             (__attribute__((address_space(3))) void*)(dst + p * 1024), 16, 0, 0);
        }
    };
    const int r16 = lane & 15, kq = lane >> 4;
    uint32_t foff[KSTEPS];
#pragma unroll
    for (int ks = 0; ks < KSTEPS; ++ks)
        foff[ks] = CK == 64 ? r16 * 128 + (((4 * ks + kq) ^ (r16 >> 1)) << 4) : r16 * 64 + ((kq ^ ((r16 >> 2) & 3)) << 4);
    constexpr int FRAG = 16 * 2 * CK;

    f32x4 acc[FM][FN];
#pragma unroll
    for (int i = 0; i < FM; ++i)
#pragma unroll
        for (int j = 0; j < FN; ++j) acc[i][j] = f32x4{0.f, 0.f, 0.f, 0.f};

#pragma unroll
    for (int i = 1; i < NSL; ++i)
        if (i < nmine) issue(wave + 8 * i, slot + i * CHUNK);
    constexpr int NOPL = SL * (1 + (EPI == EPI_RESID ? 1 + (RES ? 1 : 0) + (GATE || X == KS_ZIN ? 1 : 0) : 0)) + (X == KS_ZIN ? 4 : 0);
    KsOperands<SL> op;
    bool alt = false;
    int brow = 0;
    __builtin_amdgcn_sched_barrier(0);
    {
        const float* bsrc = a.bias ? a.bias : reinterpret_cast<const float*>(a.W);
        const float* gsrc = nullptr;
        const float* zsrc = nullptr;
        auto request = [&](int slot_m) {
            if constexpr (EPI == EPI_RESID) {
                if constexpr (GATE) gsrc = a.gate + (long)slot_m * a.gate_slot_stride;
                zsrc = a.zg + (long)slot_m * a.zg_slot_stride;
                if constexpr (DUAL) {
                    alt = erow < a.act_row0 || erow >= a.act_row1;
                    brow = (int)(((float)erow + 0.5f) * __builtin_amdgcn_rcpf((float)a.rows_per_b));
                    if (alt) zsrc = a.zg2 + (long)slot_m * a.zg2_slot_stride;
                }
            }
#pragma unroll
            for (int q = 0; q < SL; ++q) {
                int col = col0 + 4 * ks_slot_of<SL>(q, ej);
                col = col < ncl ? col : ncl;
                op.b[q] = ks_ld16_agpr(bsrc + col);
                if constexpr (EPI == EPI_RESID) {
                    if constexpr (RES) op.r[q] = ks_ld16_agpr(a.resid + (long)erow * a.ldr + col);
                    if constexpr (GATE) op.g[q] = ks_ld16_agpr(gsrc + col);
                    if constexpr (X == KS_ZIN) op.g[q] = ks_ld16_agpr(a.zG + col);
                    op.z[q] = ks_ld16_agpr(zsrc + col);
                }
            }
            if constexpr (X == KS_ZIN) {
                const int p0 = ej < a.zparts ? ej : a.zparts - 1;
                const int p1 = ej + 8 < a.zparts ? ej + 8 : a.zparts - 1;
                op.st[0] = ks_ld8_agpr(a.zstat_in + (long)p0 * a.zs_stride + erow);
                op.st[1] = ks_ld8_agpr(a.zstat_in + (long)p1 * a.zs_stride + erow);
                op.st[2] = ks_ld8_agpr(a.zstat_in2 + (long)p0 * a.zs_stride + erow);
                op.st[3] = ks_ld8_agpr(a.zstat_in2 + (long)p1 * a.zs_stride + erow);
            }
        };
        if (EPI == EPI_RESID && a.row_slot) {
            request(slot0 + a.row_slot[erow / a.rows_per_b]);
            asm volatile("; per-row slot" ::: "memory");
        } else {
            request(slot0);
            asm volatile("; shared slot" ::: "memory");
        }
    }
    __builtin_amdgcn_sched_barrier(0);
    if (ts && lane == 0) ts[1] = __builtin_readcyclecounter();
    for (int i = 0; i < nmine; ++i) {
        {
            const bool nxt = NSL == 2 && i + 1 < nmine;
            if (i < NSL) {
                if (nxt) asm volatile("s_waitcnt vmcnt(%0)" ::"n"(NPC + NOPL) : "memory");
                else asm volatile("s_waitcnt vmcnt(%0)" ::"n"(NOPL) : "memory");
            } else {
                if (nxt) asm volatile("s_waitcnt vmcnt(%0)" ::"n"(NPC) : "memory");
                else asm volatile("s_waitcnt vmcnt(0)" ::: "memory");
            }
        }
        char* cur = slot + (NSL == 2 ? (i & 1) * CHUNK : 0);
        bf16x8 af[FM][KSTEPS], bfr[FN][KSTEPS];
#pragma unroll
        for (int ks = 0; ks < KSTEPS; ++ks) {
#pragma unroll
            for (int ii = 0; ii < FM; ++ii) af[ii][ks] = *reinterpret_cast<const bf16x8*>(cur + foff[ks] + ii * FRAG);
#pragma unroll
            for (int j = 0; j < FN; ++j) bfr[j][ks] = *reinterpret_cast<const bf16x8*>(cur + BM * 2 * CK + foff[ks] + j * FRAG);
        }
        __builtin_amdgcn_sched_barrier(0);
        asm volatile("s_waitcnt lgkmcnt(0)" ::: "memory");
        __builtin_amdgcn_sched_barrier(0);
        if (i + NSL < nmine) issue(wave + 8 * (i + NSL), cur);
        __builtin_amdgcn_sched_barrier(0);
#pragma unroll
        for (int ks = 0; ks < KSTEPS; ++ks)
#pragma unroll
            for (int ii = 0; ii < FM; ++ii)
#pragma unroll
                for (int j = 0; j < FN; ++j) {
                    if (ks == KSTEPS - 1 && ii == FM - 1 && j == FN - 1)
                        asm volatile("v_mfma_f32_16x16x32_bf16 %0, %1, %2, %0\n\ts_nop 7\n\ts_nop 7\n\ts_nop 3" : "+a"(acc[ii][j]) : "v"(bfr[j][ks]), "v"(af[ii][ks]));
                    else
                        asm volatile("v_mfma_f32_16x16x32_bf16 %0, %1, %2, %0" : "+a"(acc[ii][j]) : "v"(bfr[j][ks]), "v"(af[ii][ks]));
                }
    }
    if (ts && lane == 0) ts[2] = __builtin_readcyclecounter();

    ks_operands_wait<SL, EPI, GATE, RES, X>(op);
    {
        float4* mine = reinterpret_cast<float4*>(slot);
#pragma unroll
        for (int i = 0; i < FM; ++i)
#pragma unroll
            for (int j = 0; j < FN; ++j) {
                const int r = 16 * i + r16, s = 4 * j + kq;
                mine[r * S4 + (s ^ (r & 7))] = make_float4(acc[i][j][0], acc[i][j][1], acc[i][j][2], acc[i][j][3]);
            }
    }
    f32x4 dv[SL];
    if constexpr (DUAL || X == KS_COPY2) {
        const float* dsrc = DUAL ? a.zd + (long)brow * a.zd_stride : a.zg2;
#pragma unroll
        for (int q = 0; q < SL; ++q) {
            int col = col0 + 4 * ks_slot_of<SL>(q, ej);
            col = col < ncl ? col : ncl;
            asm volatile("global_load_dwordx4 %0, %1, off" : "=v"(dv[q]) : "v"(dsrc + col) : "memory");
        }
    }
    __syncthreads();
    if (ts && lane == 0) ts[4] = __builtin_readcyclecounter();
    if constexpr (X == KS_COPY2) {
#pragma unroll
        for (int q = 0; q < SL; ++q) asm volatile("s_waitcnt vmcnt(0)" : "+v"(dv[q]));
    }
    if (!epi_thread) return;

    float4 v[SL];
#pragma unroll
    for (int q = 0; q < SL; ++q) {
        const int s = ks_slot_of<SL>(q, ej);
        const float4* p0 = reinterpret_cast<const float4*>(smem) + er * S4 + (s ^ (er & 7));
        float4 t = p0[0];
#pragma unroll
        for (int w = 1; w < 8; ++w) {
            const float4 u = p0[w * (SLOT / 16)];
            t.x += u.x; t.y += u.y; t.z += u.z; t.w += u.w;
        }
        v[q] = t;
    }
    if (ts && lane == 0) {
        asm volatile("" :: "v"(v[SL - 1].w));
        t_sum = __builtin_readcyclecounter();
    }
    float* out = reinterpret_cast<float*>(a.out);
    if constexpr (DUAL) {
#pragma unroll
        for (int q = 0; q < SL; ++q) asm volatile("s_waitcnt vmcnt(0)" : "+v"(dv[q]));
    }
    if constexpr (EPI == EPI_F32) {
#pragma unroll
        for (int q = 0; q < SL; ++q) {
            const int col = col0 + 4 * ks_slot_of<SL>(q, ej);
            const f32x4 bb = a.bias ? op.b[q] : f32x4{0.f, 0.f, 0.f, 0.f};
            const float4 o = make_float4(v[q].x + bb[0], v[q].y + bb[1], v[q].z + bb[2], v[q].w + bb[3]);
            if (row_ok && col < a.N) {
                float* dst = out + (long)erow * a.ldo + col;
                if (a.wt) st16_wt(dst, o); else *reinterpret_cast<float4*>(dst) = o;
            }
        }
    } else {
        float zmu = 0.f, zr = 1.f;
        if constexpr (X == KS_ZIN) {
            const bool one = ej < a.zparts, two = ej + 8 < a.zparts;
            float zs = ((one ? op.st[0][0] : 0.f) + (two ? op.st[1][0] : 0.f)) + ((one ? op.st[2][0] : 0.f) + (two ? op.st[3][0] : 0.f));
            float zq = ((one ? op.st[0][1] : 0.f) + (two ? op.st[1][1] : 0.f)) + ((one ? op.st[2][1] : 0.f) + (two ? op.st[3][1] : 0.f));
            zs = oct_sum(zs);
            zq = oct_sum(zq);
            const float inv_d = __builtin_amdgcn_rcpf((float)a.zD);
            zmu = zs * inv_d;
            zr = rsqrtf(fmaxf(fmaf(zq, inv_d, -zmu * zmu), 0.f) + a.zeps);
        }
        float s1 = 0.f;
#pragma unroll
        for (int q = 0; q < SL; ++q) {
            const int col = col0 + 4 * ks_slot_of<SL>(q, ej);
            const bool ok = col < a.N;
            if constexpr (X == KS_ZIN) {
                v[q].x = zr * fmaf(-zmu, op.g[q][0], v[q].x); v[q].y = zr * fmaf(-zmu, op.g[q][1], v[q].y);
                v[q].z = zr * fmaf(-zmu, op.g[q][2], v[q].z); v[q].w = zr * fmaf(-zmu, op.g[q][3], v[q].w);
            }
            float4 x = make_float4(v[q].x + op.b[q][0], v[q].y + op.b[q][1], v[q].z + op.b[q][2], v[q].w + op.b[q][3]);
            if constexpr (GATE) { x.x *= op.g[q][0]; x.y *= op.g[q][1]; x.z *= op.g[q][2]; x.w *= op.g[q][3]; }
            if constexpr (RES) { x.x += op.r[q][0]; x.y += op.r[q][1]; x.z += op.r[q][2]; x.w += op.r[q][3]; }
            if constexpr (DUAL) {
                x.x += alt ? dv[q][0] : 0.f; x.y += alt ? dv[q][1] : 0.f; x.z += alt ? dv[q][2] : 0.f; x.w += alt ? dv[q][3] : 0.f;
            }
            v[q] = ok ? x : make_float4(0.f, 0.f, 0.f, 0.f);
            s1 += (v[q].x + v[q].y) + (v[q].z + v[q].w);
            if (row_ok && ok && out) {
                float* dst = out + (long)erow * a.ldo + col;
                if (a.wt) st16_wt(dst, v[q]); else *reinterpret_cast<float4*>(dst) = v[q];
            }
        }
        float s2 = 0.f;
#pragma unroll
        for (int q = 0; q < SL; ++q) s2 = fmaf(v[q].x, v[q].x, fmaf(v[q].y, v[q].y, fmaf(v[q].z, v[q].z, fmaf(v[q].w, v[q].w, s2))));
        s1 = oct_sum(s1);
        s2 = oct_sum(s2);
        if (ej == 0 && row_ok) a.zstat_out[(long)tn * a.zs_stride + erow] = make_float2(s1, s2);
        uint2 pk[SL];
#pragma unroll
        for (int q = 0; q < SL; ++q) {
            pk[q].x = pack_bf2(v[q].x * op.z[q][0], v[q].y * op.z[q][1]);
            pk[q].y = pack_bf2(v[q].z * op.z[q][2], v[q].w * op.z[q][3]);
        }
        bf16_t* zrow = a.zu + (long)erow * a.ld_zu;
        auto store8 = [&](int col, uint2 lo, uint2 hi, bf16_t* rowp) {
            if (!row_ok || col >= a.N) return;
            bf16_t* dst = rowp + col;
            if (col + 8 <= a.N) {
                const float4 f = make_float4(__uint_as_float(lo.x), __uint_as_float(lo.y), __uint_as_float(hi.x), __uint_as_float(hi.y));
                if (a.wt) st16_wt(dst, f); else *reinterpret_cast<float4*>(dst) = f;
            } else {
                *reinterpret_cast<uint2*>(dst) = lo;
            }
        };
        auto store_row = [&](bf16_t* rowp) {
#pragma unroll
            for (int q = 0; q + 1 < 2 * (SL / 2); q += 2) store8(col0 + 4 * ks_slot_of<SL>(q, ej), pk[q], pk[q + 1], rowp);
            if constexpr (SL & 1) {
                const uint2 mine = pk[SL - 1];
                uint2 other;
                other.x = quad_xor1_u32(mine.x);
                other.y = quad_xor1_u32(mine.y);
                if ((ej & 1) == 0) store8(col0 + 4 * ks_slot_of<SL>(SL - 1, ej), mine, other, rowp);
            }
        };
        store_row(zrow);
        if constexpr (X == KS_COPY2) {
#pragma unroll
            for (int q = 0; q < SL; ++q) {
                pk[q].x = pack_bf2(v[q].x * dv[q][0], v[q].y * dv[q][1]);
                pk[q].y = pack_bf2(v[q].z * dv[q][2], v[q].w * dv[q][3]);
            }
            store_row(a.zu2 + (long)erow * a.ld_zu2);
        }
    }
    if (ts && lane == 0) {
        const unsigned long long t_iss = __builtin_readcyclecounter();
        asm volatile("s_waitcnt vmcnt(0)" ::: "memory");
        ts[3] = __builtin_readcyclecounter(); ts[7] = __builtin_amdgcn_s_memrealtime();
        ts[5] = ((t_iss - t_start) << 32) | ((t_sum - t_start) & 0xffffffffull);
    }
}

}
```

ezaudio_amd/csrc/gemm_pp.h:

```cpp
#pragma once
#include "common.h"

#include <type_traits>

namespace {

template <int N>
__device__ __forceinline__ void wait_vmcnt() {
    static_assert(N >= 0 && N < 64, "vmcnt is a 6-bit counter");
    asm volatile("s_waitcnt vmcnt(%0)" ::"n"(N) : "memory");
}

template <int PER, int MAXY, int EXTRA = 0>
__device__ __forceinline__ void wait_younger(int younger) {
    if constexpr (MAXY >= 3) { if (younger >= 3) { wait_vmcnt<3 * PER + EXTRA>(); return; } }
    if constexpr (MAXY >= 2) { if (younger >= 2) { wait_vmcnt<2 * PER + EXTRA>(); return; } }
    if constexpr (MAXY >= 1) { if (younger >= 1) { wait_vmcnt<PER + EXTRA>(); return; } }
    wait_vmcnt<EXTRA>();
}

__device__ __forceinline__ f32x2 ld8_blind(const void* p) {
    f32x2 v;
    asm volatile("global_load_dwordx2 %0, %1, off" : "=a"(v) : "v"(p) : "memory");
    return v;
}

template <int PER, int MAXY, int BASE>
__device__ __forceinline__ void wait_younger_x(int younger, int extra ) {
    if (extra >= 2) wait_younger<PER, MAXY, BASE + 2>(younger);
    else if (extra == 1) wait_younger<PER, MAXY, BASE + 1>(younger);
    else wait_younger<PER, MAXY, BASE>(younger);
}

__device__ __forceinline__ float gelu_erf(float x) {
    const float z = fabsf(x) * 0.70710678118654752440f;
    const float t = __builtin_amdgcn_rcpf(fmaf(0.3275911f, z, 1.0f));
    float p = fmaf(1.061405429f, t, -1.453152027f);
    p = fmaf(p, t, 1.421413741f);
    p = fmaf(p, t, -0.284496736f);
    p = fmaf(p, t, 0.254829592f);
    const float e = __builtin_amdgcn_exp2f(-1.4426950408889634f * z * z);
    const float erf_abs = 1.0f - p * t * e;
    return 0.5f * x * (1.0f + copysignf(erf_abs, x));
}

__device__ __forceinline__ f32x2 gelu_erf2(f32x2 x) {
    const f32x2 z = __builtin_elementwise_abs(x) * f32x2{0.70710678118654752440f, 0.70710678118654752440f};
    const f32x2 d = __builtin_elementwise_fma(f32x2{0.3275911f, 0.3275911f}, z, f32x2{1.0f, 1.0f});
    const f32x2 t = {__builtin_amdgcn_rcpf(d[0]), __builtin_amdgcn_rcpf(d[1])};
    f32x2 p = __builtin_elementwise_fma(f32x2{1.061405429f, 1.061405429f}, t, f32x2{-1.453152027f, -1.453152027f});
    p = __builtin_elementwise_fma(p, t, f32x2{1.421413741f, 1.421413741f});
    p = __builtin_elementwise_fma(p, t, f32x2{-0.284496736f, -0.284496736f});
    p = __builtin_elementwise_fma(p, t, f32x2{0.254829592f, 0.254829592f});
    const f32x2 a = (z * f32x2{-1.4426950408889634f, -1.4426950408889634f}) * z;
    const f32x2 e = {__builtin_amdgcn_exp2f(a[0]), __builtin_amdgcn_exp2f(a[1])};
    const f32x2 erf_abs = __builtin_elementwise_fma(-(p * t), e, f32x2{1.0f, 1.0f});
    const f32x2 s = {copysignf(erf_abs[0], x[0]), copysignf(erf_abs[1], x[1])};
    return (x * f32x2{0.5f, 0.5f}) * (s + f32x2{1.0f, 1.0f});
}

__device__ __forceinline__ bool tile_of_block(const GemmArgs& a, int tilesM, int tilesN, int& tm, int& tn, int& z) {
    const int xcd = blockIdx.x & 7;
    const int l = blockIdx.x >> 3;
    const int lpm = __builtin_ctz(a.pm), lpn = __builtin_ctz(a.pn);
    const int xm = xcd & (a.pm - 1), xn = (xcd >> lpm) & (a.pn - 1), xz = xcd >> (lpm + lpn);
    const int t1 = ez_div(l, a.mbm), lm = l - t1 * a.bm;
    const int lz = ez_div(t1, a.mbn), ln = t1 - lz * a.bn;
    tm = xm * a.bm + lm;
    tn = xn * a.bn + ln;
    z = xz * a.bz + lz;
    return tm < tilesM && tn < tilesN && z < a.splitk;
}
__device__ __forceinline__ void panel_of_block(const GemmArgs& a, int tilesN, int& tm, int& tn, int& z) {
    const int G = tilesN * a.splitk, l = blockIdx.x >> 3;
    const int lg = ez_div(l, a.mG), r = l - lg * G;
    tm = (blockIdx.x & 7) + 8 * lg;
    tn = ez_div(r, a.msplit);
    z = r - tn * a.splitk;
}
__device__ __forceinline__ void ksplit_range(const GemmArgs& a, int nk, int z, int& kb, int& ke) {
    if (a.splitk == 1) { kb = 0; ke = nk; return; }
    kb = ez_div(nk * z, a.msplit);
    ke = ez_div(nk * (z + 1), a.msplit);
}

template <int NT>
__device__ __forceinline__ void copy_out_bf16(const bf16_t* tile, int pitch, int rows, int oc , bf16_t* out, int ldo,
                                              int grow0, int gcol0, int M, int ncols, int wt, int tid) {
    const int cpr = oc / 8;
    for (int q = tid; q < rows * cpr; q += NT) {
        const int r = q / cpr, c = (q % cpr) * 8;
        const int grow = grow0 + r, gcol = gcol0 + c;
        if (grow < M && gcol < ncols) {
            const uint4 v = *reinterpret_cast<const uint4*>(tile + r * pitch + c);
            bf16_t* dst = out + (long)grow * ldo + gcol;
            if (gcol + 8 <= ncols) {
                if (wt) st16_wt(dst, make_float4(__uint_as_float(v.x), __uint_as_float(v.y), __uint_as_float(v.z), __uint_as_float(v.w)));
                else *reinterpret_cast<uint4*>(dst) = v;
            } else {
                const bf16_t* src = tile + r * pitch + c;
                for (int e = 0; e < ncols - gcol; ++e) dst[e] = src[e];
            }
        }
    }
}

__device__ __forceinline__ void divmod_rows(int m, int L, float rcpL, int& b, int& l) {
    b = (int)(((float)m + 0.5f) * rcpL);
    l = m - b * L;
}

__device__ __forceinline__ int z_slot(const GemmArgs& a, int slot0, int rowc) {
    return slot0 + (a.row_slot ? a.row_slot[rowc / a.rows_per_b] : 0);
}

template <int FM, int FN, int TM, int TN, int EPI>
__device__ __forceinline__ void pp_store_direct(const GemmArgs& a, f32x4 (&acc)[FM][FN], int row0, int col0, int wm, int wn, int lane, int z) {
    static_assert(EPI == EPI_F32 || EPI == EPI_PARTIAL, "fp32 outputs");
    const int m_in = lane & 15, cg = lane >> 4;
    float* out = reinterpret_cast<float*>(a.out);
    if constexpr (EPI == EPI_PARTIAL) out += (long)z * a.slab_stride;
    float4 b4[FN], g4[FN];
    const int ncl = a.N - 4;
    if constexpr (EPI == EPI_F32) {
#pragma unroll
        for (int j = 0; j < FN; ++j) {
            int col = col0 + wn * TN + j * 16 + 4 * cg;
            col = col < ncl ? col : ncl;
            b4[j] = a.bias ? *reinterpret_cast<const float4*>(a.bias + col) : make_float4(0.f, 0.f, 0.f, 0.f);
        }
    }
#pragma unroll
    for (int i = 0; i < FM; ++i) {
        const int row = row0 + wm * TM + i * 16 + m_in;
        const int rowc = row < a.M ? row : a.M - 1;
        float4 r4[FN];
        if constexpr (EPI == EPI_F32) {
            if (a.resid) {
#pragma unroll
                for (int j = 0; j < FN; ++j) {
                    int col = col0 + wn * TN + j * 16 + 4 * cg;
                    col = col < ncl ? col : ncl;
                    r4[j] = *reinterpret_cast<const float4*>(a.resid + (long)rowc * a.ldr + col);
                }
                if (a.gate) {
                    const int slot = (a.cur_step ? *a.cur_step : 0) + (a.row_slot ? a.row_slot[rowc / a.rows_per_b] : 0);
#pragma unroll
                    for (int j = 0; j < FN; ++j) {
                        int col = col0 + wn * TN + j * 16 + 4 * cg;
                        col = col < ncl ? col : ncl;
                        g4[j] = *reinterpret_cast<const float4*>(a.gate + (long)slot * a.gate_slot_stride + col);
                    }
                }
            }
        }
#pragma unroll
        for (int j = 0; j < FN; ++j) {
            const int col = col0 + wn * TN + j * 16 + 4 * cg;
            float4 v = make_float4(acc[i][j][0], acc[i][j][1], acc[i][j][2], acc[i][j][3]);
            if constexpr (EPI == EPI_F32) {
                v.x += b4[j].x; v.y += b4[j].y; v.z += b4[j].z; v.w += b4[j].w;
                if (a.resid) {
                    if (a.gate) { v.x *= g4[j].x; v.y *= g4[j].y; v.z *= g4[j].z; v.w *= g4[j].w; }
                    v.x += r4[j].x; v.y += r4[j].y; v.z += r4[j].z; v.w += r4[j].w;
                }
            }
            if (row < a.M && col < a.N) {
                float* dst = out + (long)row * a.ldo + col;
                if (a.wt) st16_wt(dst, v); else *reinterpret_cast<float4*>(dst) = v;
            }
        }
    }
}

template <int BM, int BN, int FM, int FN, int TM, int TN, int NT, int EPI, bool ZC>
__device__ __forceinline__ void pp_store_lds(const GemmArgs& a, f32x4 (&acc)[FM][FN], char* smem, int row0, int col0, int wm, int wn, int lane, int tid, int z,
                                             const float2* zmr , const float* zgc, int slot0, unsigned long long* ts = nullptr) {
    static_assert(EPI == EPI_GEGLU || EPI == EPI_PARTIAL, "bf16 outputs only");
    constexpr int OC = EPI == EPI_GEGLU ? BN / 2 : BN;
    static_assert(OC % 8 == 0, "16-byte row chunks");
    constexpr int PITCH = OC + 8;
    bf16_t* tile = reinterpret_cast<bf16_t*>(smem);
    const int m_in = lane & 15, cg = lane >> 4;
    uint32_t pk[FM][FN];
    if constexpr (EPI == EPI_GEGLU) {
        const int ncl = a.N - 4;
        float4 c4[FN], g4[FN];
        const bool shared_slot = !ZC || !a.row_slot;
        if (shared_slot) {
            const long so = ZC ? (long)slot0 * a.zt_slot_stride : 0;
#pragma unroll
            for (int j = 0; j < FN; ++j) {
                int cp = col0 + wn * TN + j * 16 + 4 * cg;
                cp = cp < ncl ? cp : ncl;
                if constexpr (ZC) {
                    (void)so;
                    g4[j] = *reinterpret_cast<const float4*>(zgc + (wn * TN + j * 16 + 4 * cg));
                    c4[j] = *reinterpret_cast<const float4*>(zgc + BN + (wn * TN + j * 16 + 4 * cg));
                } else {
                    g4[j] = make_float4(0.f, 0.f, 0.f, 0.f);
                    c4[j] = a.bias ? *reinterpret_cast<const float4*>(a.bias + cp) : make_float4(0.f, 0.f, 0.f, 0.f);
                }
            }
        }
#pragma unroll
        for (int i = 0; i < FM; ++i) {
            float mu = 0.f, r = 1.f;
            if constexpr (ZC) {
                const int rl = wm * TM + i * 16 + m_in;
                if (!shared_slot) {
                    int row = row0 + rl;
                    row = row < a.M ? row : a.M - 1;
                    const long so = (long)z_slot(a, slot0, row) * a.zt_slot_stride;
#pragma unroll
                    for (int j = 0; j < FN; ++j) {
                        int cp = col0 + wn * TN + j * 16 + 4 * cg;
                        cp = cp < ncl ? cp : ncl;
                        g4[j] = *reinterpret_cast<const float4*>(a.zG + so + cp);
                        c4[j] = *reinterpret_cast<const float4*>(a.zC + so + cp);
                    }
                }
                const float2 mr = zmr[i];
                mu = mr.x; r = mr.y;
            }
// ... 343 lines not shown
    const HeadNormArgs& hn = a.hn;
    const int cg = lane >> 4;
    const int part = col0 / (hn.H * DH);
    const bool rope = part < 2 && hn.rope_cos != nullptr;
    const float* w = part == 1 ? hn.kn_w : hn.qn_w;
    {
        const int t = tid < 32 * NF ? tid : 0;
        op.aff = ((t & 4) ? (part == 1 ? hn.kn_b : hn.qn_b) : w)[qkv_aff_index<DH>(t)];
    }
    const float rcpL = __builtin_amdgcn_rcpf((float)hn.L);
#pragma unroll
    for (int i = 0; i < FM; ++i) {
        int m = first_row + i * 16;
        m = m < a.M ? m : a.M - 1;
        int b_, l;
        divmod_rows(m, hn.L, rcpL, b_, l);
        const float* ct = (rope ? hn.rope_cos + (long)l * HALF : w);
        const float* st = (rope ? hn.rope_sin + (long)l * HALF : w);
#pragma unroll
        for (int q = 0; q < NF; ++q) {
            const int f = q < FH ? 8 * q + 2 * cg : 8 * FH + 2 * (cg & 1);
            op.cs[i][q] = *reinterpret_cast<const f32x2*>(ct + f);
            op.sn[i][q] = *reinterpret_cast<const f32x2*>(st + f);
        }
    }
}

template <int BM, int BN, int DH, int FM, int FN, int TM, int TN, int NT, bool ZC>
__device__ __forceinline__ void pp_store_qkv_reg(const GemmArgs& a, f32x4 (&acc)[FM][FN], char* smem, int row0, int col0, int wm, int lane, int tid,
                                                 const float2* zmr, const float* zgc, float* aff_l, int slot0, const QkvOperands<DH, FM>& op, unsigned long long* ts = nullptr) {
    constexpr int NH = 2, DQK = DH == 72 ? 80 : 64, DV = DH == 72 ? 96 : 64, FH = DH / 16, MID = (DH % 16) != 0;
    static_assert(NH * DH == BN && TN == BN && FN == 2 * FH + MID && (DH % 16 == 0 || DH % 16 == 8), "two whole heads per tile, a wave holds whole rows");
    constexpr int PITCH = BN + 8;
    bf16_t* tile = reinterpret_cast<bf16_t*>(smem);
    if (ts && lane == 0) ts[4] = __builtin_readcyclecounter();
    const int m_in = lane & 15, cg = lane >> 4;
    const HeadNormArgs& hn = a.hn;
    const float rcpL = __builtin_amdgcn_rcpf((float)hn.L);
    const int D = hn.H * DH;
    const int part = col0 / D;
    const int head0 = (col0 % D) / DH;
    const bool rope = part < 2 && hn.rope_cos != nullptr;
    const auto& cs = op.cs; const auto& sn = op.sn;
    constexpr int NF = QkvOperands<DH, FM>::NF;
    static_assert(32 * NF <= NT, "one table element per thread");
    if (tid < 32 * NF) aff_l[tid] = op.aff;
    const float4* aff4 = reinterpret_cast<const float4*>(aff_l) + cg * NF * 2;
    __syncthreads();
    const bool mid0 = cg < 2;
#pragma unroll
    for (int i = 0; i < FM; ++i) {
        if constexpr (ZC) {
            const int ncl = a.N - 4;
            const int rl = wm * TM + i * 16 + m_in;
            const float2 mr = zmr[i];
            const float r = mr.y, rm = mr.y * mr.x;
            if (!a.row_slot) {
#pragma unroll
                for (int j = 0; j < FN; ++j) {
                    const float4 g4 = *reinterpret_cast<const float4*>(zgc + (j * 16 + 4 * cg)), c4 = *reinterpret_cast<const float4*>(zgc + BN + (j * 16 + 4 * cg));
                    acc[i][j][0] = fmaf(r, acc[i][j][0], fmaf(-rm, g4.x, c4.x));
                    acc[i][j][1] = fmaf(r, acc[i][j][1], fmaf(-rm, g4.y, c4.y));
                    acc[i][j][2] = fmaf(r, acc[i][j][2], fmaf(-rm, g4.z, c4.z));
                    acc[i][j][3] = fmaf(r, acc[i][j][3], fmaf(-rm, g4.w, c4.w));
                }
            } else {
                int row = row0 + rl;
                row = row < a.M ? row : a.M - 1;
                const long so = (long)z_slot(a, slot0, row) * a.zt_slot_stride;
#pragma unroll
                for (int j = 0; j < FN; ++j) {
                    int cp = col0 + j * 16 + 4 * cg;
                    cp = cp < ncl ? cp : ncl;
                    const float4 g4 = *reinterpret_cast<const float4*>(a.zG + so + cp), c4 = *reinterpret_cast<const float4*>(a.zC + so + cp);
                    acc[i][j][0] = fmaf(r, acc[i][j][0], fmaf(-rm, g4.x, c4.x));
                    acc[i][j][1] = fmaf(r, acc[i][j][1], fmaf(-rm, g4.y, c4.y));
                    acc[i][j][2] = fmaf(r, acc[i][j][2], fmaf(-rm, g4.z, c4.z));
                    acc[i][j][3] = fmaf(r, acc[i][j][3], fmaf(-rm, g4.w, c4.w));
                }
            }
        }
        bf16_t* trow = tile + (wm * TM + i * 16 + m_in) * PITCH + 4 * cg;
        if (part < 2) {
            float s0 = 0.f, s1 = 0.f, sm = 0.f;
#pragma unroll
            for (int j = 0; j < FH; ++j) {
                s0 += (acc[i][j][0] + acc[i][j][1]) + (acc[i][j][2] + acc[i][j][3]);
                s1 += (acc[i][FH + MID + j][0] + acc[i][FH + MID + j][1]) + (acc[i][FH + MID + j][2] + acc[i][FH + MID + j][3]);
            }
            if constexpr (MID) sm = (acc[i][FH][0] + acc[i][FH][1]) + (acc[i][FH][2] + acc[i][FH][3]);
            const float mean0 = row4_sum(s0 + (mid0 ? sm : 0.f)) * (1.f / DH), mean1 = row4_sum(s1 + (mid0 ? 0.f : sm)) * (1.f / DH);
            float q0 = 0.f, q1 = 0.f, qm = 0.f;
            const float meanm = mid0 ? mean0 : mean1;
#pragma unroll
            for (int j = 0; j < FH; ++j)
#pragma unroll
                for (int x = 0; x < 4; ++x) {
                    const float d0 = acc[i][j][x] - mean0, d1 = acc[i][FH + MID + j][x] - mean1;
                    q0 = fmaf(d0, d0, q0); q1 = fmaf(d1, d1, q1);
                }
            if constexpr (MID) {
#pragma unroll
                for (int x = 0; x < 4; ++x) { const float d = acc[i][FH][x] - meanm; qm = fmaf(d, d, qm); }
            }
            const float rstd0 = rsqrtf(row4_sum(q0 + (mid0 ? qm : 0.f)) * (1.f / DH) + 1e-5f), rstd1 = rsqrtf(row4_sum(q1 + (mid0 ? 0.f : qm)) * (1.f / DH) + 1e-5f);
#pragma unroll
            for (int j = 0; j < FN; ++j) {
                const bool is_mid = MID && j == FH;
                const int q = is_mid ? FH : (j < FH ? j : j - FH - MID);
                const float mean = is_mid ? meanm : (j < FH ? mean0 : mean1);
                const float rstd = is_mid ? (mid0 ? rstd0 : rstd1) : (j < FH ? rstd0 : rstd1);
                const float4 w4 = aff4[2 * q], b4 = aff4[2 * q + 1];
                float y0 = (acc[i][j][0] - mean) * rstd * w4.x + b4.x, y1 = (acc[i][j][1] - mean) * rstd * w4.z + b4.z;
                float y2 = (acc[i][j][2] - mean) * rstd * w4.y + b4.y, y3 = (acc[i][j][3] - mean) * rstd * w4.w + b4.w;
                if (rope) {
                    const float o0 = y0 * cs[i][q][0] - y1 * sn[i][q][0], o1 = y1 * cs[i][q][0] + y0 * sn[i][q][0];
                    const float o2 = y2 * cs[i][q][1] - y3 * sn[i][q][1], o3 = y3 * cs[i][q][1] + y2 * sn[i][q][1];
                    y0 = o0; y1 = o1; y2 = o2; y3 = o3;
                }
                *reinterpret_cast<uint2*>(trow + j * 16) = make_uint2(pack_bf2(y0, y1), pack_bf2(y2, y3));
            }
        } else {
#pragma unroll
            for (int j = 0; j < FN; ++j)
                *reinterpret_cast<uint2*>(trow + j * 16) = make_uint2(pack_bf2(acc[i][j][0], acc[i][j][1]), pack_bf2(acc[i][j][2], acc[i][j][3]));
        }
    }
    if (ts && lane == 0) ts[5] = __builtin_readcyclecounter();
    __syncthreads();

    constexpr int CP = DH / 8;
    bf16_t* dstbase = part == 0 ? hn.q : part == 1 ? hn.k : hn.v;
    const int pitch = part < 2 ? DQK : DV;
    for (int q = tid; q < BM * NH * CP; q += NT) {
        const int c8 = q % CP, hh = (q / CP) % NH, r = q / (CP * NH);
        const int m = row0 + r;
        if (m < a.M) {
            int b, l;
            divmod_rows(m, hn.L, rcpL, b, l);
            bf16_t* dst = dstbase + (((long)b * hn.H + head0 + hh) * hn.Lp + l) * pitch + c8 * 8;
            const uint4 v = *reinterpret_cast<const uint4*>(tile + r * PITCH + hh * DH + c8 * 8);
            if (a.wt) st16_wt(dst, make_float4(__uint_as_float(v.x), __uint_as_float(v.y), __uint_as_float(v.z), __uint_as_float(v.w)));
            else *reinterpret_cast<uint4*>(dst) = v;
        }
    }
}

template <int BM, int BN, int NS, int EPI>
constexpr int pp_smem_bytes() {
    return NS * ((BM + BN + 31) / 32) * 4096 + BM * 8 + (EPI == EPI_RESID ? 4 : 2) * BN * 4 + (EPI == EPI_QKV ? 8 * 256 + 1024 : 0);
}

template <int BM, int BN, int WM, int WN, int NS, int EPI, int SCHED, int VAR>
__global__ __launch_bounds__(512) void k_gemm_pp(GemmArgs a) {
    static_assert(SCHED == 1 || SCHED == 2, "schedule");
    static_assert(WM * WN == (SCHED == 1 ? 8 : 4), "SCHED 1: 8 waves tile the block; SCHED 2: each group of 4 tiles it");
    constexpr int NT = 512, NTG = 256;
    constexpr int TM = BM / WM, TN = BN / WN, FM = TM / 16, FN = TN / 16;
    static_assert(BM % 32 == 0 && TM % 16 == 0 && TN % 16 == 0 && TM * WM == BM && TN * WN == BN, "tile geometry");
    static_assert(SCHED == 1 || FM % 2 == 0, "SCHED 2 splits the wave tile's row fragments between the groups after the loop");
    constexpr int NP = (BM + BN + 31) / 32;
    constexpr int PA = BM / 32;
    constexpr int STAGE = NP * 4096;
    constexpr int PD = NS - 1;
    static_assert(NS >= 3 && NS <= 6, "ring depth");
    static_assert(pp_smem_bytes<BM, BN, NS, EPI>() <= 160 * 1024, "LDS budget of a CU (ring + per-row LayerNorm statistics + G' / C' (or bias / gate / gain) of the tile's columns [+ EPI_QKV: sink of the table warm-up])");
    constexpr int P0 = SCHED == 1 ? (NP + 1) / 2 : NP;
    extern __shared__ __attribute__((aligned(16))) char smem[];

    int M_ = a.M;
    asm("" : "+s"(M_) : "s"(a.A), "s"(a.W), "s"(a.lda), "s"(a.ldw), "s"(a.wrows), "s"(a.N), "s"(a.K), "s"(a.splitk), "s"(a.pm), "s"(a.pn), "s"(a.bm), "s"(a.bn), "s"(a.bz),
        "s"(a.cur_step), "s"(a.ts), "s"(a.xcd_panel), "s"(a.row_slot), "s"(a.mbm), "s"(a.mbn), "s"(a.msplit), "s"(a.mG));
    const int slot0 = a.cur_step ? *a.cur_step : 0;
    const float *zG_ = a.zG, *zC_ = a.zC;
    asm("" : "+s"(M_), "+s"(zG_), "+s"(zC_));
    const float *rb_ = a.bias, *rg_ = a.gate, *rz_ = a.zg, *rz2_ = a.zg2;
    if constexpr (EPI == EPI_RESID) asm("" : "+s"(M_), "+s"(rb_), "+s"(rg_), "+s"(rz_), "+s"(rz2_));
    const float *rc_ = a.hn.rope_cos, *rs_ = a.hn.rope_sin;
    if constexpr (EPI == EPI_QKV) asm("" : "+s"(M_), "+s"(rc_), "+s"(rs_));
    const int tid = threadIdx.x;
    const int lane = tid & 63;
    const int wave = __builtin_amdgcn_readfirstlane(tid >> 6);
    const int grp = wave >> 2, wg = wave & 3;
    const int tg = tid & (NTG - 1);
    const int wt = SCHED == 1 ? wave : wg;
    const int wm = wt / WN, wn = wt % WN;

    const int tilesM = (M_ + BM - 1) / BM;
    const int tilesN = (a.N + BN - 1) / BN;
    int tm, tn, z;
    if (EPI == EPI_PARTIAL && a.xcd_panel) {
        panel_of_block(a, tilesN, tm, tn, z);
        if (tm >= tilesM) return;
    } else if (!tile_of_block(a, tilesM, tilesN, tm, tn, z)) return;
    const int row0 = tm * BM, col0 = tn * BN;
    const int nk = a.K / BK;
    int kb, ke;
    ksplit_range(a, nk, z, kb, ke);
    const int nt = ke - kb;

    constexpr bool ZM = (VAR & 64) != 0;
    float* zgc = reinterpret_cast<float*>(smem + NS * STAGE + BM * 8);
    constexpr bool ZMC = ZM && (EPI == EPI_GEGLU || EPI == EPI_QKV);
    constexpr int FMR = SCHED == 1 ? FM : FM / 2;
    constexpr int NZT = ZMC ? FMR * Z_PT : 0;
    ZLaneRegs<FMR> zlr;
    const bool z_shared_slot = a.row_slot == nullptr;
    constexpr int ZNV = EPI == EPI_RESID ? ((VAR & (256 | 512)) ? 4 : 3) * (BN / 4) : 2 * (BN / 4);
    const bool z_warm = EPI == EPI_QKV && rc_ && col0 < 2 * a.hn.H * a.hn.dh;
    const int zx = nt >= 2 ? ((((ZMC && z_shared_slot) || EPI == EPI_RESID) && wave * 64 < ZNV) ? 1 : 0) + (z_warm ? 1 : 0) : -1;
    constexpr bool RGATE = EPI == EPI_RESID && (VAR & 64) != 0, RRES = EPI == EPI_RESID && (VAR & 128) != 0, RDUAL = EPI == EPI_RESID && (VAR & 256) != 0;
    constexpr bool RCOPY2 = EPI == EPI_RESID && (VAR & 512) != 0, RZIN = EPI == EPI_RESID && (VAR & 1024) != 0;
    static_assert(!RDUAL || (RGATE && RRES), "DUAL: the gated residual projection only");
    static_assert(!(RDUAL && RCOPY2) && !(RZIN && (RGATE || RRES || RDUAL || RCOPY2)), "forms of the residual epilogue");
    auto z_late_load = [&]() {
        if constexpr (EPI == EPI_QKV) {
            const HeadNormArgs& hn = a.hn;
            if (z_warm) {
                const int r = tid >> 2, which = tid & 3;
                int m = row0 + r;
                m = m < a.M ? m : a.M - 1;
                int b_, l_;
                divmod_rows(m, hn.L, __builtin_amdgcn_rcpf((float)hn.L), b_, l_);
                const char* src = reinterpret_cast<const char*>((which & 2) ? rs_ : rc_) + ((long)l_ * (hn.dh / 2) + ((which & 1) ? hn.dh / 2 - 1 : 0)) * 4;
                __builtin_amdgcn_global_load_lds((const __attribute__((address_space(1))) void*)src,
                                                 (__attribute__((address_space(3))) void*)(smem + NS * STAGE + BM * 8 + 2 * BN * 4 + wave * 256), 4, 0, 0);
            }
        }
        if constexpr (EPI == EPI_RESID) {
            static_assert(4 * (BN / 4) <= NT, "one float4 per thread");
            if (tid < ZNV) {
                const int which = tid / (BN / 4), t4 = tid - which * (BN / 4);
                int cp = col0 + 4 * t4;
                cp = cp < a.N - 4 ? cp : a.N - 4;
                const float* src = which == 0 ? rb_ : which == 1 ? (RGATE ? rg_ + (long)slot0 * a.gate_slot_stride : RZIN ? zG_ : rb_) : which == 2 ? rz_ + (long)slot0 * a.zg_slot_stride
                                   : ((RDUAL || RCOPY2) ? rz2_ + (long)slot0 * a.zg2_slot_stride : rb_);
                __builtin_amdgcn_global_load_lds((const __attribute__((address_space(1))) void*)(src + cp),
                                                 (__attribute__((address_space(3))) void*)(reinterpret_cast<char*>(zgc) + wave * 1024), 16, 0, 0);
            }
        }
        if constexpr (ZM && (EPI == EPI_GEGLU || EPI == EPI_QKV)) {
            static_assert(2 * (BN / 4) <= NT, "one float4 of G' or C' per thread");
            if (z_shared_slot && tid < ZNV) {
                const int which = tid >= BN / 4, t4 = tid - which * (BN / 4);
                int cp = col0 + 4 * t4;
                cp = cp < a.N - 4 ? cp : a.N - 4;
                __builtin_amdgcn_global_load_lds((const __attribute__((address_space(1))) void*)((which ? zC_ : zG_) + (long)slot0 * a.zt_slot_stride + cp),
                                                 (__attribute__((address_space(3))) void*)(reinterpret_cast<char*>(zgc) + wave * 1024), 16, 0, 0);
            }
            const int frow = SCHED == 1 ? row0 + wm * TM + (lane & 15) : row0 + (wm * 2 + grp) * (TM / 2) + (lane & 15);
            z_lane_load<FMR>(a.zstat_in, a.zs_stride, a.zparts, frow, a.M - 1, lane >> 4, zlr);
        }
    };
    unsigned long long* ts = (a.ts && wave == 0) ? a.ts + 8 * (long)blockIdx.x : nullptr;
    if (ts && lane == 0) { ts[0] = __builtin_readcyclecounter(); ts[6] = ez_stamp_start(); }
    f32x4 acc[FM][FN];
#pragma unroll
    for (int i = 0; i < FM; ++i)
#pragma unroll
        for (int j = 0; j < FN; ++j) acc[i][j] = f32x4{0.f, 0.f, 0.f, 0.f};

    constexpr int PMAX = P0;
    uint32_t poff[PMAX];
    const int pbeg = (SCHED == 1 && grp == 1) ? P0 : 0;
#pragma unroll
    for (int i = 0; i < PMAX; ++i) {
        const int p = pbeg + i;
        const int q = p * NTG + tg;
        const int row = q >> 3, c = q & 7;
        if (p < PA) {
            int grow = row0 + row;
            grow = grow < a.M ? grow : a.M - 1;
            poff[i] = (uint32_t)(grow * a.lda + ((c ^ ((row >> 1) & 7)) << 3)) * 2u;
        } else {
            const int r2 = row - BM;
            int gr = col0 + r2;
            gr = gr < a.wrows ? gr : a.wrows - 1;
            poff[i] = (uint32_t)(gr * a.ldw + ((c ^ ((r2 >> 1) & 7)) << 3)) * 2u;
        }
    }
    const char* gA = reinterpret_cast<const char*>(a.A) + (long)kb * (BK * 2);
    const char* gW = reinterpret_cast<const char*>(a.W) + (long)kb * (BK * 2);

    auto issue = [&](int t, auto PB_, auto PE_) {
        constexpr int PB = decltype(PB_)::value, PE = decltype(PE_)::value;
        char* dst = smem + (t % NS) * STAGE + wg * 1024;
        const long koff = (long)t * (BK * 2);
#pragma unroll
        for (int p = PB; p < PE; ++p) {
            const char* src = (p < PA ? gA : gW) + koff + poff[p - PB];
            __builtin_amdgcn_global_load_lds((const __attribute__((address_space(1))) void*)src,
                                             (__attribute__((address_space(3))) void*)(dst + p * 4096), 16, 0, 0);
        }
    };

    const int r16 = lane & 15, kq = lane >> 4;
    uint32_t foff[2];
#pragma unroll
    for (int ks = 0; ks < 2; ++ks) foff[ks] = r16 * 128 + (((4 * ks + kq) ^ (r16 >> 1)) << 4);
    const int a_base = wm * TM * 128, b_base = BM * 128 + wn * TN * 128;

    auto issue_piece = [&](int t, int p, int pi) {
        char* dst = smem + (t % NS) * STAGE + wg * 1024;
        const char* src = (p < PA ? gA : gW) + (long)t * (BK * 2) + poff[pi];
        __builtin_amdgcn_global_load_lds((const __attribute__((address_space(1))) void*)src,
                                         (__attribute__((address_space(3))) void*)(dst + p * 4096), 16, 0, 0);
    };
    bf16x8 af[FM][2], bfr[FN][2];
    if constexpr (VAR & 16) {
        const bf16x8 f0 = *reinterpret_cast<const bf16x8*>(smem + lane * 16);
#pragma unroll
        for (int ks = 0; ks < 2; ++ks) {
#pragma unroll
            for (int i = 0; i < FM; ++i) { af[i][ks] = f0; asm volatile("" : "+v"(af[i][ks])); }
#pragma unroll
            for (int j = 0; j < FN; ++j) { bfr[j][ks] = f0; asm volatile("" : "+v"(bfr[j][ks])); }
        }
    }
    auto load_phase = [&](int t, int tr, bool refill, auto PB_, auto PE_) {
        constexpr int PB = decltype(PB_)::value, PE = decltype(PE_)::value, PG = PE - PB;
        constexpr int NR = 2 * (FM + FN), STRIDE = NR / (PG > 0 ? PG : 1) > 0 ? NR / (PG > 0 ? PG : 1) : 1;
        const char* cT = smem + (t % NS) * STAGE;
#pragma unroll
        for (int r = 0; r < NR; ++r) {
            const int ks = r / (FM + FN), idx = r % (FM + FN);
            if constexpr (!(VAR & 16)) {
                if (idx < FM) af[idx][ks] = *reinterpret_cast<const bf16x8*>(cT + foff[ks] + a_base + idx * 2048);
                else bfr[idx - FM][ks] = *reinterpret_cast<const bf16x8*>(cT + foff[ks] + b_base + (idx - FM) * 2048);
            }
            if constexpr (!(VAR & 32)) {
                if ((r + 1) % STRIDE == 0 && (r + 1) / STRIDE - 1 < PG) {
                    if (refill) issue_piece(tr, PB + (r + 1) / STRIDE - 1, (r + 1) / STRIDE - 1);
                }
            }
        }
        if constexpr (!(VAR & 32)) {
#pragma unroll
            for (int q = NR / STRIDE; q < PG; ++q)
                if (refill) issue_piece(tr, PB + q, q);
        }
    };
    auto mfmas = [&]() {
        if constexpr (VAR & 8) {
#pragma unroll
            for (int ks = 0; ks < 2; ++ks) {
#pragma unroll
                for (int i = 0; i < FM; ++i) asm volatile("" ::"v"(af[i][ks]));
#pragma unroll
                for (int j = 0; j < FN; ++j) asm volatile("" ::"v"(bfr[j][ks]));
            }
            return;
        }
#pragma unroll
        for (int ks = 0; ks < 2; ++ks)
#pragma unroll
            for (int i = 0; i < FM; ++i)
#pragma unroll
                for (int j = 0; j < FN; ++j)
                    asm volatile("v_mfma_f32_16x16x32_bf16 %0, %1, %2, %0" : "+a"(acc[i][j]) : "v"(bfr[j][ks]), "v"(af[i][ks]));
    };
    auto fence_lds = [&]() {
        __builtin_amdgcn_sched_barrier(0);
        asm volatile("s_waitcnt lgkmcnt(0)" ::: "memory");
        __builtin_amdgcn_sched_barrier(0);
    };
    auto barrier = [&]() {
        __builtin_amdgcn_sched_barrier(0);
        __builtin_amdgcn_s_barrier();
        __builtin_amdgcn_sched_barrier(0);
    };

    if constexpr (SCHED == 1) {
        auto run = [&](auto G_) {
            constexpr int G = decltype(G_)::value;
            constexpr int PB = G == 0 ? 0 : P0, PE = G == 0 ? P0 : NP, PG = PE - PB;
            static_assert(PG * (PD - 1) < 64, "vmcnt range");
            using IB = std::integral_constant<int, PB>;
            using IE = std::integral_constant<int, PE>;
#pragma unroll
            for (int t = 0; t < PD; ++t) {
                if (t < nt) issue(t, IB{}, IE{});
                if (t == 0) z_late_load();
            }
            if (zx < 0) wait_vmcnt<0>(); else wait_younger_x<PG, PD - 1, NZT>((nt < PD ? nt : PD) - 1, zx);
            barrier();
            if constexpr (G == 1) barrier();
            auto step = [&](int t, auto RF_) {
                constexpr bool rf = decltype(RF_)::value;
                load_phase(t, t + PD, rf, IB{}, IE{});
                if constexpr (G == 1) {
                    if constexpr (rf) wait_vmcnt<PG * (PD - 1)>();
                    else if (t + 1 < nt) wait_younger<PG, PD - 1>(nt - 2 - t);
                }
                fence_lds();
                barrier();
                mfmas();
                if constexpr (G == 0) {
                    if constexpr (rf) wait_vmcnt<PG * (PD - 1)>();
                    else if (t + 1 < nt) wait_younger<PG, PD - 1>(nt - 2 - t);
                    barrier();
                } else {
                    if (rf || t + 1 < nt) barrier();
                }
            };
            if (ts && lane == 0) ts[1] = __builtin_readcyclecounter();
            int t = 0;
            for (; t + PD < nt; ++t) step(t, std::true_type{});
            for (; t < nt; ++t) step(t, std::false_type{});
            if (ts && lane == 0) ts[2] = __builtin_readcyclecounter();
        };
        if (grp == 0) run(std::integral_constant<int, 0>{});
        else run(std::integral_constant<int, 1>{});
    } else {
        using IB = std::integral_constant<int, 0>;
        using IE = std::integral_constant<int, NP>;
        static_assert(NP * ((PD - 1) / 2 + 1) < 64, "vmcnt range");
        auto own_younger = [&](int u) {
            const int last = u - 1 + PD < nt - 1 ? u - 1 + PD : nt - 1;
            return last >= u + 2 ? (last - u) / 2 : 0;
        };
        auto run = [&](auto G_) {
            constexpr int G = decltype(G_)::value;
            if constexpr ((PD & 1) != G) z_late_load();
#pragma unroll
            for (int u = 0; u < PD; ++u) {
                if (((u + PD) & 1) == G && u < nt) issue(u, IB{}, IE{});
                if (u == 0 && (PD & 1) == G) z_late_load();
            }
            {
                const int last = PD - 1 < nt - 1 ? PD - 1 : nt - 1;
                if constexpr ((PD & 1) == G) { if (zx < 0) wait_vmcnt<0>(); else wait_younger_x<NP, (PD - 1) / 2, NZT>(last >= 2 ? last / 2 : 0, zx); }
            }
            barrier();
            auto end_wait = [&](int i, auto RF_) {
                constexpr bool rf = decltype(RF_)::value;
                if constexpr (rf) {
                    wait_vmcnt<NP * ((PD - 1) / 2)>();
                } else {
                    if (i + 1 < nt) wait_younger<NP, (PD - 1) / 2>(own_younger(i + 1));
                }
            };
            if constexpr (G == 1) {
                if constexpr (PD % 2 == 0) end_wait(0, std::false_type{});
                barrier();
            }
            auto step = [&](int t, auto RF_) {
                constexpr bool rf = decltype(RF_)::value;
                load_phase(t, t + PD, rf || t + PD < nt, IB{}, IE{});
                if constexpr (PD % 2 == 1) end_wait(t, RF_);
                fence_lds();
                barrier();
                mfmas();
                if (rf || t + 1 < nt) {
                    if constexpr (PD % 2 == 0) end_wait(t + 1, RF_);
                    barrier();
                }
            };
            if (ts && lane == 0) ts[1] = __builtin_readcyclecounter();
            int t = G;
            for (; t + 1 + PD < nt; t += 2) step(t, std::true_type{});
            for (; t < nt; t += 2) step(t, std::false_type{});
            if (ts && lane == 0) ts[2] = __builtin_readcyclecounter();
        };
        if (grp == 0) run(std::integral_constant<int, 0>{});
        else run(std::integral_constant<int, 1>{});
    }

#pragma unroll
    for (int i = 0; i < FM; ++i)
#pragma unroll
        for (int j = 0; j < FN; ++j) asm volatile("" : "+a"(acc[i][j]));
    asm volatile("s_nop 7\n\ts_nop 7\n\ts_nop 3" ::: "memory");
#pragma unroll
    for (int i = 0; i < FM; ++i)
#pragma unroll
        for (int j = 0; j < FN; ++j) asm volatile("" : "+a"(acc[i][j]));
    float2 zmr[FMR];
    if constexpr (ZMC) {
        asm volatile("s_waitcnt vmcnt(0)" ::: "memory");
        z_lane_finish<FMR>(zlr, a.zparts, lane >> 4, a.zD, a.zeps, zmr);
    }
    if constexpr (SCHED == 2) {
        constexpr int HF = FM / 2;
        static_assert(8 * HF * FN * 1024 <= NS * STAGE, "exchange area must fit the ring");
        asm volatile("s_waitcnt lgkmcnt(0)" ::: "memory");
        barrier();
        f32x4* xw = reinterpret_cast<f32x4*>(smem) + (long)(wave ^ 4) * (HF * FN * 64);
        f32x4* xr = reinterpret_cast<f32x4*>(smem) + (long)wave * (HF * FN * 64);
        if (grp == 0) {
#pragma unroll
            for (int i = 0; i < HF; ++i)
#pragma unroll
                for (int j = 0; j < FN; ++j) xw[(i * FN + j) * 64 + lane] = acc[HF + i][j];
        } else {
#pragma unroll
            for (int i = 0; i < HF; ++i)
#pragma unroll
                for (int j = 0; j < FN; ++j) xw[(i * FN + j) * 64 + lane] = acc[i][j];
        }
        constexpr int RF = EPI == EPI_RESID ? FM / 2 : 1, RN = EPI == EPI_RESID ? FN : 1;
        float4 rres[RF][RN], dres[RDUAL ? RF : 1][RDUAL ? RN : 1];
        float2 zst[RF][4];
        if constexpr (RZIN) {
            const int m_in = lane & 15, cg = lane >> 4;
            const int p0 = cg < a.zparts ? cg : a.zparts - 1;
            const int p1 = cg + 4 < a.zparts ? cg + 4 : a.zparts - 1;
#pragma unroll
            for (int i = 0; i < RF; ++i) {
                int row = row0 + (wm * 2 + grp) * (TM / 2) + i * 16 + m_in;
                row = row < a.M ? row : a.M - 1;
                zst[i][0] = a.zstat_in[(long)p0 * a.zs_stride + row];
                zst[i][1] = a.zstat_in[(long)p1 * a.zs_stride + row];
                zst[i][2] = a.zstat_in2[(long)p0 * a.zs_stride + row];
                zst[i][3] = a.zstat_in2[(long)p1 * a.zs_stride + row];
            }
        }
        if constexpr (RRES) {
            const int m_in = lane & 15, cg = lane >> 4;
#pragma unroll
            for (int i = 0; i < RF; ++i) {
                int row = row0 + (wm * 2 + grp) * (TM / 2) + i * 16 + m_in;
                row = row < a.M ? row : a.M - 1;
                const float* dsrc = nullptr;
                if constexpr (RDUAL) dsrc = a.zd + (long)(int)(((float)row + 0.5f) * __builtin_amdgcn_rcpf((float)a.rows_per_b)) * a.zd_stride;
#pragma unroll
                for (int j = 0; j < RN; ++j) {
                    int col = col0 + wn * TN + j * 16 + 4 * cg;
                    col = col < a.N - 4 ? col : a.N - 4;
                    rres[i][j] = *reinterpret_cast<const float4*>(a.resid + (long)row * a.ldr + col);
                    if constexpr (RDUAL) dres[i][j] = *reinterpret_cast<const float4*>(dsrc + col);
                }
            }
        }
        constexpr int QDH = EPI == EPI_QKV ? BN / 2 : 64;
        QkvOperands<QDH, EPI == EPI_QKV ? FM / 2 : 1> qop;
        if constexpr (EPI == EPI_QKV) {
            if (a.hn.perm) qkv_request<QDH, FM / 2>(a, col0, row0 + (wm * 2 + grp) * (TM / 2) + (lane & 15), lane, tid, qop);
        }
        asm volatile("s_waitcnt lgkmcnt(0)" ::: "memory");
        barrier();
        f32x4 half[HF][FN];
        if (grp == 0) {
#pragma unroll
            for (int i = 0; i < HF; ++i)
#pragma unroll
                for (int j = 0; j < FN; ++j) half[i][j] = acc[i][j] + xr[(i * FN + j) * 64 + lane];
        } else {
#pragma unroll
            for (int i = 0; i < HF; ++i)
#pragma unroll
                for (int j = 0; j < FN; ++j) half[i][j] = acc[HF + i][j] + xr[(i * FN + j) * 64 + lane];
        }
        const int ewm = wm * 2 + grp;
        if constexpr (EPI == EPI_RESID) {
            static_assert(WN == 1, "EPI_RESID: a wave holds whole tile rows after the exchange");
            static_assert(BM * (BN + 8) * 2 <= NS * STAGE, "A' tile must fit the ring");
            if constexpr (RDUAL) pp_store_resid<BM, BN, HF, FN, TM / 2, TN, NT, RGATE, RRES, true>(a, half, smem, row0, col0, ewm, lane, tid, zgc, rres, dres, zst);
            else pp_store_resid<BM, BN, HF, FN, TM / 2, TN, NT, RGATE, RRES, false, RCOPY2, RZIN>(a, half, smem, row0, col0, ewm, lane, tid, zgc, rres, rres, zst);
        }
        if constexpr (EPI == EPI_QKV) {
            static_assert(BN == 144 || BN == 128, "EPI_QKV tiles hold two whole heads (head_dim 72 / 64)");
            static_assert(BM * (BN + 4) * 4 + BM * BN * 2 <= NS * STAGE, "epilogue tile + staging must fit the ring");
            static_assert(BM * (BN + 8) * 2 <= NS * STAGE, "bf16 staging tile must fit the ring");
            if (a.hn.perm) pp_store_qkv_reg<BM, BN, BN / 2, HF, FN, TM / 2, TN, NT, ZM>(a, half, smem, row0, col0, ewm, lane, tid, zmr, zgc, reinterpret_cast<float*>(smem + NS * STAGE + BM * 8 + 2 * BN * 4 + 8 * 256), slot0, qop, ts);
            else pp_store_qkv<BM, BN, BN / 2, HF, FN, TM / 2, TN, NT, ZM>(a, half, smem, row0, col0, ewm, wn, lane, tid, zmr, zgc, slot0);
        }
        if constexpr (EPI == EPI_GEGLU || EPI == EPI_PARTIAL) {
            constexpr bool lds_ok = BM * ((EPI == EPI_GEGLU ? BN / 2 : BN) + 8) * 2 <= NS * STAGE;
            if constexpr (lds_ok) {
                if (EPI == EPI_GEGLU || a.part_bf16) {
                    pp_store_lds<BM, BN, HF, FN, TM / 2, TN, NT, EPI, ZM>(a, half, smem, row0, col0, ewm, wn, lane, tid, z, zmr, zgc, slot0, ts);
                    if (ts && lane == 0) { ts[3] = __builtin_readcyclecounter(); ts[7] = __builtin_amdgcn_s_memrealtime(); }
                    return;
                }
            }
        }
        if constexpr (EPI == EPI_F32 || EPI == EPI_PARTIAL) pp_store_direct<HF, FN, TM / 2, TN, EPI>(a, half, row0, col0, ewm, wn, lane, z);
    } else {
        if constexpr (EPI == EPI_QKV) {
            static_assert(WN == 1 && FM == 1, "a wave holds one 16-row fragment over the whole tile width");
            static_assert(BN == 144 || BN == 128, "EPI_QKV tiles hold two whole heads (head_dim 72 / 64)");
            static_assert(BM * (BN + 8) * 2 <= NS * STAGE, "bf16 staging tile must fit the ring");
            QkvOperands<BN / 2, FM> qop;
            qkv_request<BN / 2, FM>(a, col0, row0 + wm * TM + (lane & 15), lane, tid, qop);
            pp_store_qkv_reg<BM, BN, BN / 2, FM, FN, TM, TN, NT, ZM>(a, acc, smem, row0, col0, wm, lane, tid, zmr, zgc, reinterpret_cast<float*>(smem + NS * STAGE + BM * 8 + 2 * BN * 4 + 8 * 256), slot0, qop, ts);
        }
        if constexpr (EPI == EPI_GEGLU || EPI == EPI_PARTIAL) {
            constexpr bool lds_ok = BM * ((EPI == EPI_GEGLU ? BN / 2 : BN) + 8) * 2 <= NS * STAGE;
            if constexpr (lds_ok) {
                if (EPI == EPI_GEGLU || a.part_bf16) {
                    pp_store_lds<BM, BN, FM, FN, TM, TN, NT, EPI, ZM>(a, acc, smem, row0, col0, wm, wn, lane, tid, z, zmr, zgc, slot0, ts);
                    if (ts && lane == 0) { ts[3] = __builtin_readcyclecounter(); ts[7] = __builtin_amdgcn_s_memrealtime(); }
                    return;
                }
            }
        }
        if constexpr (EPI == EPI_F32 || EPI == EPI_PARTIAL) pp_store_direct<FM, FN, TM, TN, EPI>(a, acc, row0, col0, wm, wn, lane, z);
    }
    if (ts && lane == 0) { asm volatile("s_waitcnt vmcnt(0)" ::: "memory"); ts[3] = __builtin_readcyclecounter(); ts[7] = __builtin_amdgcn_s_memrealtime(); }
}

}
```

Measured before the change: 278.5.

## Pass hot GEMM arguments as preloaded kernargs and defer the rest

```diff
diff --git a/ezaudio_amd/build.py b/ezaudio_amd/build.py
--- a/ezaudio_amd/build.py
+++ b/ezaudio_amd/build.py
@@ -13,6 +13,8 @@
     FLAGS.append('-DEZ_ABLATE')
 if os.environ.get('EZAUDIO_DIAG'):
     FLAGS.append('-DEZ_DIAG')
+PRELOAD = ['-mllvm', '-amdgpu-kernarg-preload-count=14']
+UNIT_FLAGS = {'gemm.hip': PRELOAD}
 
 
 def source_hash():
@@ -24,6 +26,8 @@
         h.update(os.path.basename(f).encode())
         with open(f, 'rb') as fh:
             h.update(fh.read())
+    for src in sorted(UNIT_FLAGS):
+        h.update((src + ' ' + ' '.join(UNIT_FLAGS[src])).encode())
     return h.hexdigest()[:16]
 
 
@@ -54,7 +58,7 @@
 
     def compile_one(job):
         s, o = job
-        cmd = [hipcc] + FLAGS + ['-c', s, '-o', o]
+        cmd = [hipcc] + FLAGS + UNIT_FLAGS.get(os.path.basename(s), []) + ['-c', s, '-o', o]
         r = subprocess.run(cmd, capture_output=True, text=True)
         return job, r
 
diff --git a/ezaudio_amd/csrc/api.hip b/ezaudio_amd/csrc/api.hip
--- a/ezaudio_amd/csrc/api.hip
+++ b/ezaudio_amd/csrc/api.hip
@@ -21,6 +21,22 @@
     return code;
 }
 #define fail ez_fail
+static thread_local std::string g_refusal;
+int ez_refuse(const char* fmt, ...) {
+    char buf[384];
+    va_list ap;
+    va_start(ap, fmt);
+    vsnprintf(buf, sizeof buf, fmt, ap);
+    va_end(ap);
+    g_refusal = buf;
+    return 1;
+}
+static std::string take_refusal() {
+    std::string r;
+    if (!g_refusal.empty()) r = " (" + g_refusal + ")";
+    g_refusal.clear();
+    return r;
+}
 
 namespace {
 
@@ -443,17 +459,18 @@
     hipError_t err = hipSuccess;
     int rc = EZDIT_OK;
     const char* where = nullptr;
+    std::string why;
     unsigned long long* stamps() const { return (g_gemm_ts && h->launches == h->opt_stamp_launch) ? g_gemm_ts : nullptr; }
     void launched(const char* what, int launch_rc = 0) {
         if (h->opt_trace_launches) fprintf(stderr, "launch %d %s\n", h->launches, what);
         h->launches++;
-        if (launch_rc != 0 && rc == EZDIT_OK) { rc = launch_rc; where = what; }
+        if (launch_rc != 0 && rc == EZDIT_OK) { rc = launch_rc; where = what; why = take_refusal(); }
         const hipError_t e = hipGetLastError();
         if (e != hipSuccess && err == hipSuccess) { err = e; where = what; }
     }
     bool bad() const { return err != hipSuccess || rc != EZDIT_OK; }
     int result() const {
-        if (rc != EZDIT_OK) return fail(rc, "%s: configuration not supported by the HIP kernels", where ? where : "?");
+        if (rc != EZDIT_OK) return fail(rc, "%s: configuration not supported by the HIP kernels%s", where ? where : "?", why.c_str());
         if (err != hipSuccess) return fail(EZDIT_E_HIP, "launch of %s failed: %s", where ? where : "?", hipGetErrorString(err));
         return EZDIT_OK;
     }
@@ -606,7 +623,8 @@
 template <typename Launch>
 int hook_launch(const char* kernel, const char* config, Launch launch) {
     (void)hipGetLastError();
-    if (launch()) return fail(EZDIT_E_UNSUPPORTED, "%s not supported", config);
+    g_refusal.clear();
+    if (launch()) return fail(EZDIT_E_UNSUPPORTED, "%s not supported%s", config, take_refusal().c_str());
     const hipError_t e = hipGetLastError();
     if (e != hipSuccess) return fail(EZDIT_E_HIP, "launch of %s failed: %s", kernel, hipGetErrorString(e));
     return EZDIT_OK;
diff --git a/ezaudio_amd/csrc/common.h b/ezaudio_amd/csrc/common.h
--- a/ezaudio_amd/csrc/common.h
+++ b/ezaudio_amd/csrc/common.h
@@ -40,17 +40,19 @@
     return v;
 }
 
-__device__ __forceinline__ unsigned long long ez_stamp_start() {
+__device__ __forceinline__ unsigned long long ez_stamp_tag(unsigned long long realtime) {
     const unsigned hw = __builtin_amdgcn_s_getreg((31 << 11) | 4), xcc = __builtin_amdgcn_s_getreg((31 << 11) | 20);
     const unsigned long long id = ((unsigned long long)(xcc & 15u) << 8) | ((hw >> 8) & 255u);
-    return (__builtin_amdgcn_s_memrealtime() & 0xffffffffffffull) | (id << 48);
-}
+    return (realtime & 0xffffffffffffull) | (id << 48);
+}
+__device__ __forceinline__ unsigned long long ez_stamp_start() { return ez_stamp_tag(__builtin_amdgcn_s_memrealtime()); }
 
 inline unsigned ez_magic(int d) { return d <= 1 ? 0u : (unsigned)((0x100000000ull + (unsigned)d - 1) / (unsigned)d); }
 __device__ __forceinline__ int ez_div(int x, unsigned m) { return m ? (int)__umulhi((unsigned)x, m) : x; }
 
 
 int ez_fail(int code, const char* fmt, ...);
+int ez_refuse(const char* fmt, ...);
 
 enum GemmEpi {
     EPI_F32 = 0,
diff --git a/ezaudio_amd/csrc/gemm.hip b/ezaudio_amd/csrc/gemm.hip
--- a/ezaudio_amd/csrc/gemm.hip
+++ b/ezaudio_amd/csrc/gemm.hip
@@ -325,6 +325,24 @@
     return 8 * a.bm * a.bn * a.bz;
 }
 
+struct PpLead { const int* step; int K; int box; };
+bool pp_lead(const GemmArgs& a, bool partial, long grid, PpLead& ld) {
+    if (!partial) {
+        if (a.splitk != 1 || a.pz != 1) return ez_refuse("split-K %d (K boxes %d) with an epilogue that writes no slabs", a.splitk, a.pz) == 0;
+        if (a.bm > PP_BOX_BM_MAX || a.bn > PP_BOX_BN_MAX) return ez_refuse("XCD boxes of %d x %d tiles do not fit the packed leading parameter (<= %d x %d)", a.bm, a.bn, PP_BOX_BM_MAX, PP_BOX_BN_MAX) == 0;
+        ld.step = a.cur_step; ld.K = a.K; ld.box = pp_pack_box(a.pm, a.pn, a.bm, a.bn);
+        return true;
+    }
+    if (a.bm > PP_PBOX_BM_MAX || a.bn > PP_PBOX_BN_MAX || a.bz > PP_PBOX_BZ_MAX || a.splitk < 1 || a.splitk > PP_PBOX_S_MAX || a.K > PP_PBOX_K_MAX || a.pm * a.pn * a.pz != 8 ||
+        grid / 8 >= (1 << 20))
+        return ez_refuse("split-K launch beyond the packed leading parameters: boxes %d x %d x %d tiles (<= %d x %d x %d), %d splits (<= %d), K = %d (<= %d), %ld workgroups (< 2^23)",
+                         a.bm, a.bn, a.bz, PP_PBOX_BM_MAX, PP_PBOX_BN_MAX, PP_PBOX_BZ_MAX, a.splitk, PP_PBOX_S_MAX, a.K, PP_PBOX_K_MAX, grid) == 0;
+    ld.step = reinterpret_cast<const int*>(static_cast<uintptr_t>((unsigned long long)a.mbn | ((unsigned long long)a.msplit << 32)));
+    ld.K = a.K | (a.splitk << 24);
+    ld.box = pp_pack_box_partial(a.pm, a.pn, a.bm, a.bn, a.bz, a.xcd_panel);
+    return true;
+}
+
 template <int BM, int BN, int WM, int WN, int NS, int EPI, int SCHED, int VAR = 0>
 int launch_pp(const GemmArgs& a0, hipStream_t st) {
     GemmArgs a = a0;
@@ -343,7 +361,9 @@
         attr_set[dev].store(true, std::memory_order_release);
     }
     if (a.ts && (long)grid.x > a.ts_cap) a.ts = nullptr;
-    hipLaunchKernelGGL((k_gemm_pp<BM, BN, WM, WN, NS, EPI, SCHED, VAR>), grid, dim3(512), SMEM, st, a);
+    PpLead ld;
+    if (!pp_lead(a, EPI == EPI_PARTIAL, (long)grid.x, ld)) return 1;
+    hipLaunchKernelGGL((k_gemm_pp<BM, BN, WM, WN, NS, EPI, SCHED, VAR>), grid, dim3(512), SMEM, st, a.A, a.W, ld.step, a.lda, a.ldw, a.wrows, a.M, a.N, ld.K, ld.box, a.mbm, a);
     return 0;
 }
 
@@ -362,7 +382,9 @@
         attr_set[dev].store(true, std::memory_order_release);
     }
     if (a.ts && (long)grid.x > a.ts_cap) a.ts = nullptr;
-    hipLaunchKernelGGL((k_gemm_co<BM, BN, EPI, VAR>), grid, dim3(256), SMEM, st, a);
+    PpLead ld;
+    if (!pp_lead(a, EPI == EPI_PARTIAL, (long)grid.x, ld)) return 1;
+    hipLaunchKernelGGL((k_gemm_co<BM, BN, EPI, VAR>), grid, dim3(256), SMEM, st, a.A, a.W, ld.step, a.lda, a.ldw, a.wrows, a.M, a.N, ld.K, ld.box, a.mbm, a);
     return 0;
 }
 
@@ -387,7 +409,8 @@
         attr_set[dev].store(true, std::memory_order_release);
     }
     if (a.ts && (long)grid.x > a.ts_cap) a.ts = nullptr;
-    hipLaunchKernelGGL((k_gemm_ks<FM, FN, EPI, GATE, RES, CK, X>), grid, dim3(512), SMEM, st, a);
+    if (a.pm > 255 || a.bn >= (1 << 23)) return ez_refuse("k_gemm_ks: XCD boxes pm = %d, bn = %d do not fit the packed leading parameter", a.pm, a.bn);
+    hipLaunchKernelGGL((k_gemm_ks<FM, FN, EPI, GATE, RES, CK, X>), grid, dim3(512), SMEM, st, a.A, a.W, a.cur_step, a.lda, a.ldw, a.wrows, a.M, a.N, a.K, a.pm | (a.bn << 8), a);
     return 0;
 }
 template <int EPI, bool GATE, bool RES>
diff --git a/ezaudio_amd/csrc/gemm_co.h b/ezaudio_amd/csrc/gemm_co.h
--- a/ezaudio_amd/csrc/gemm_co.h
+++ b/ezaudio_amd/csrc/gemm_co.h
@@ -9,7 +9,8 @@
 }
 
 template <int BM, int BN, int EPI, int VAR>
-__global__ __launch_bounds__(256, 2) void k_gemm_co(GemmArgs a) {
+__global__ __launch_bounds__(256, 2) void k_gemm_co(const bf16_t* kA, const bf16_t* kW, const int* kstep, int klda, int kldw, int kwrows, int kM, int kN, int kK, int kbox, unsigned kmbm,
+                                                    GemmArgs a) {
     constexpr int NT = 256;
     constexpr int WM = 4, TM = BM / WM, TN = BN, FM = TM / 16, FN = TN / 16;
     static_assert(TM * WM == BM && TM % 16 == 0 && TN % 16 == 0, "tile geometry: four waves, each TM rows x the whole tile width");
@@ -21,35 +22,42 @@
     static_assert(NP < 32, "vmcnt range");
     extern __shared__ __attribute__((aligned(16))) char smem[];
 
-    int M_ = a.M;
-    asm("" : "+s"(M_) : "s"(a.A), "s"(a.W), "s"(a.lda), "s"(a.ldw), "s"(a.wrows), "s"(a.N), "s"(a.K), "s"(a.splitk), "s"(a.pm), "s"(a.pn), "s"(a.bm), "s"(a.bn), "s"(a.bz),
-        "s"(a.cur_step), "s"(a.ts), "s"(a.row_slot), "s"(a.mbm), "s"(a.mbn), "s"(a.msplit));
-    const int slot0 = a.cur_step ? *a.cur_step : 0;
-    const float *zG_ = a.zG, *zC_ = a.zC;
-    asm("" : "+s"(M_), "+s"(zG_), "+s"(zC_));
+    int slot0 = 0;
+    if constexpr (EPI != EPI_PARTIAL) slot0 = kstep ? *kstep : 0;
+    const unsigned long long t_start = __builtin_readcyclecounter(), t_real = __builtin_amdgcn_s_memrealtime();
     const int tid = threadIdx.x;
     const int lane = tid & 63;
     const int wave = __builtin_amdgcn_readfirstlane(tid >> 6);
     const int wm = wave;
 
-    const int tilesM = (M_ + BM - 1) / BM;
-    const int tilesN = (a.N + BN - 1) / BN;
-    int tm, tn, z;
-    if (!tile_of_block(a, tilesM, tilesN, tm, tn, z)) return;
+    const int tilesM = (kM + BM - 1) / BM;
+    const int tilesN = (kN + BN - 1) / BN;
+    const int nk = (EPI == EPI_PARTIAL ? kK & PP_PBOX_K_MAX : kK) / BK;
+    int tm, tn, z = 0, kb = 0, ke = nk;
+    if constexpr (EPI == EPI_PARTIAL) {
+        if (!tile_of_block_lead_partial(kbox, kmbm, (unsigned long long)reinterpret_cast<uintptr_t>(kstep), kK, tilesM, tilesN, tm, tn, z, kb, ke)) return;
+    } else if (!tile_of_block_lead(kbox, kmbm, tilesM, tilesN, tm, tn)) return;
     const int row0 = tm * BM, col0 = tn * BN;
-    const int nk = a.K / BK;
-    int kb, ke;
-    ksplit_range(a, nk, z, kb, ke);
     const int nt = ke - kb;
 
     constexpr bool ZM = (VAR & 64) != 0 && (EPI == EPI_GEGLU || EPI == EPI_QKV);
     float* zgc = reinterpret_cast<float*>(smem + 2 * STAGE + BM * 8);
     constexpr int NZT = ZM ? FM * Z_PT : 0;
     ZLaneRegs<FM> zlr;
-    const bool z_shared_slot = a.row_slot == nullptr;
+    bool z_shared_slot = true;
     constexpr int ZNV = 2 * (BN / 4);
-    const bool zx = ZM && z_shared_slot && wave * 64 < ZNV;
+    bool zx = false;
+    unsigned long long* ts = nullptr;
     auto z_late_load = [&]() {
+        long late = 0;
+        asm("; late arguments" : "+s"(late) : "s"(a.ts), "s"(a.row_slot), "s"(a.zstat_in), "s"(a.zs_stride), "s"(a.zparts), "s"(a.zt_slot_stride), "s"(a.zG), "s"(a.zC));
+        const float *zG_ = a.zG + late, *zC_ = a.zC + late;
+        {
+            unsigned long long* ts_ = a.ts ? a.ts + late : nullptr;
+            ts = (ts_ && wave == 0) ? ts_ + 8 * (long)blockIdx.x : nullptr;
+            z_shared_slot = a.row_slot == nullptr;
+            zx = ZM && z_shared_slot && wave * 64 < ZNV;
+        }
         if constexpr (ZM) {
             static_assert(2 * (BN / 4) <= NT, "one float4 of G' or C' per thread");
             if (z_shared_slot && tid < ZNV) {
@@ -62,8 +70,6 @@
             z_lane_load<FM>(a.zstat_in, a.zs_stride, a.zparts, row0 + wm * TM + (lane & 15), a.M - 1, lane >> 4, zlr);
         }
     };
-    unsigned long long* ts = (a.ts && wave == 0) ? a.ts + 8 * (long)blockIdx.x : nullptr;
-    if (ts && lane == 0) { ts[0] = __builtin_readcyclecounter(); ts[6] = ez_stamp_start(); }
     f32x4 acc[FM][FN];
 #pragma unroll
     for (int i = 0; i < FM; ++i)
@@ -77,17 +83,17 @@
         const int row = q >> 3, c = q & 7;
         if (p < PA) {
             int grow = row0 + row;
-            grow = grow < a.M ? grow : a.M - 1;
-            poff[p] = (uint32_t)(grow * a.lda + ((c ^ ((row >> 1) & 7)) << 3)) * 2u;
+            grow = grow < kM ? grow : kM - 1;
+            poff[p] = (uint32_t)(grow * klda + ((c ^ ((row >> 1) & 7)) << 3)) * 2u;
         } else {
             const int r2 = row - BM;
             int gr = col0 + r2;
-            gr = gr < a.wrows ? gr : a.wrows - 1;
-            poff[p] = (uint32_t)(gr * a.ldw + ((c ^ ((r2 >> 1) & 7)) << 3)) * 2u;
-        }
-    }
-    const char* gA = reinterpret_cast<const char*>(a.A) + (long)kb * (BK * 2);
-    const char* gW = reinterpret_cast<const char*>(a.W) + (long)kb * (BK * 2);
+            gr = gr < kwrows ? gr : kwrows - 1;
+            poff[p] = (uint32_t)(gr * kldw + ((c ^ ((r2 >> 1) & 7)) << 3)) * 2u;
+        }
+    }
+    const char* gA = reinterpret_cast<const char*>(kA) + (long)kb * (BK * 2);
+    const char* gW = reinterpret_cast<const char*>(kW) + (long)kb * (BK * 2);
     auto issue = [&](int t) {
         char* dst = smem + (t & 1) * STAGE + wave * 1024;
         const long koff = (long)t * (BK * 2);
@@ -121,7 +127,7 @@
     if (nt > 1) issue(1);
     if (nt > 1) { if (zx) wait_vmcnt<NP + NZT + 1>(); else wait_vmcnt<NP + NZT>(); } else wait_vmcnt<0>();
     barrier();
-    if (ts && lane == 0) ts[1] = __builtin_readcyclecounter();
+    if (ts && lane == 0) { const unsigned long long t1 = __builtin_readcyclecounter(); ts[0] = t_start; ts[6] = ez_stamp_tag(t_real); ts[1] = t1; }
     auto step = [&](int t, auto MODE_) {
         constexpr int MODE = decltype(MODE_)::value;
         const char* cT = smem + (t & 1) * STAGE;
diff --git a/ezaudio_amd/csrc/gemm_ks.h b/ezaudio_amd/csrc/gemm_ks.h
--- a/ezaudio_amd/csrc/gemm_ks.h
+++ b/ezaudio_amd/csrc/gemm_ks.h
@@ -44,15 +44,15 @@
     return q < 2 * NP ? 16 * (q >> 1) + 2 * j + (q & 1) : 16 * NP + j;
 }
 
-__device__ __forceinline__ bool ks_tile_of_block(const GemmArgs& a, int tilesM, int tilesN, int& tm, int& tn) {
+__device__ __forceinline__ bool ks_tile_of_block(int pm, int bn, int tilesM, int tilesN, int& tm, int& tn) {
     const int xcd = blockIdx.x & 7, l = blockIdx.x >> 3;
-    const int lpm = __builtin_ctz(a.pm);
-    const int xm = xcd & (a.pm - 1), gn = xcd >> lpm;
-    const int n0 = gn * a.bn;
+    const int lpm = __builtin_ctz(pm);
+    const int xm = xcd & (pm - 1), gn = xcd >> lpm;
+    const int n0 = gn * bn;
     int gw = tilesN - n0;
-    gw = gw < a.bn ? gw : a.bn;
+    gw = gw < bn ? gw : bn;
     if (gw <= 0) return false;
-    const int T = tilesM * gw, run = (T + a.pm - 1) >> lpm;
+    const int T = tilesM * gw, run = (T + pm - 1) >> lpm;
     const int t = xm * run + l;
     if (l >= run || t >= T) return false;
     tm = (int)(((float)t + 0.5f) * __builtin_amdgcn_rcpf((float)gw));
@@ -61,7 +61,8 @@
 }
 
 template <int FM, int FN, int EPI, bool GATE, bool RES, int CK, int X = KS_PLAIN>
-__global__ __launch_bounds__(512) void k_gemm_ks(GemmArgs a) {
+__global__ __launch_bounds__(512) void k_gemm_ks(const bf16_t* kA, const bf16_t* kW, const int* kstep, int klda, int kldw, int kwrows, int kM, int kN, int kK,
+                                                 int kbox, GemmArgs a) {
     constexpr bool DUAL = X == KS_DUAL;
     static_assert(EPI == EPI_F32 || EPI == EPI_RESID, "epilogues");
     static_assert(!DUAL || (EPI == EPI_RESID && GATE && RES), "DUAL: the gated residual projection only");
@@ -89,30 +90,25 @@
     const int lane = tid & 63;
     const int wave = __builtin_amdgcn_readfirstlane(tid >> 6);
 
-    int M_ = a.M;
-    asm("" : "+s"(M_) : "s"(a.A), "s"(a.W), "s"(a.lda), "s"(a.ldw), "s"(a.wrows), "s"(a.N), "s"(a.K), "s"(a.pm), "s"(a.bn), "s"(a.cur_step), "s"(a.ts), "s"(a.ts_cap),
-        "s"(a.row_slot), "s"(a.bias), "s"(a.resid), "s"(a.ldr), "s"(a.gate), "s"(a.zg));
     int slot0 = 0;
-    if constexpr (EPI == EPI_RESID) slot0 = a.cur_step ? *a.cur_step : 0;
-    const int tilesM = (M_ + BM - 1) / BM;
-    const int tilesN = (a.N + BN - 1) / BN;
+    if constexpr (EPI == EPI_RESID) slot0 = kstep ? *kstep : 0;
+    const unsigned long long t_start = __builtin_readcyclecounter(), t_real = __builtin_amdgcn_s_memrealtime();
+    const int tilesM = (kM + BM - 1) / BM;
+    const int tilesN = (kN + BN - 1) / BN;
     int tm, tn;
-    if (!ks_tile_of_block(a, tilesM, tilesN, tm, tn)) return;
+    if (!ks_tile_of_block(kbox & 255, kbox >> 8, tilesM, tilesN, tm, tn)) return;
     const int row0 = tm * BM, col0 = tn * BN;
-    const int nk = a.K / CK;
-    unsigned long long* ts = (a.ts && wave == 0) ? a.ts + 8 * (long)blockIdx.x : nullptr;
-    unsigned long long t_start = 0, t_sum = 0;
-    if (ts && lane == 0) { t_start = __builtin_readcyclecounter(); ts[0] = t_start; ts[6] = ez_stamp_start(); }
+    const int nk = kK / CK;
 
     const int er = tid >> 3, ej = tid & 7;
     const bool epi_thread = tid < 8 * BM;
     int erow = row0 + er;
-    const bool row_ok = epi_thread && erow < a.M;
-    erow = erow < a.M ? erow : a.M - 1;
-    const int ncl = a.N - 4;
-
-    const char* gA = reinterpret_cast<const char*>(a.A);
-    const char* gW = reinterpret_cast<const char*>(a.W);
+    const bool row_ok = epi_thread && erow < kM;
+    erow = erow < kM ? erow : kM - 1;
+    const int ncl = kN - 4;
+
+    const char* gA = reinterpret_cast<const char*>(kA);
+    const char* gW = reinterpret_cast<const char*>(kW);
     char* slot = smem + wave * SLOT;
     const int nmine = wave < nk ? (nk - wave + 7) / 8 : 0;
     uint32_t poff[NPC];
@@ -123,18 +119,22 @@
         const int gc = CK == 64 ? (c ^ ((r2 >> 1) & 7)) : (c ^ ((r2 >> 2) & 3));
         if (p < PA) {
             int grow = row0 + row;
-            grow = grow < a.M ? grow : a.M - 1;
-            poff[p] = (uint32_t)(grow * a.lda + (gc << 3)) * 2u;
+            grow = grow < kM ? grow : kM - 1;
+            poff[p] = (uint32_t)(grow * klda + (gc << 3)) * 2u;
         } else {
             int gr = col0 + r2;
-            gr = gr < a.wrows ? gr : a.wrows - 1;
-            poff[p] = (uint32_t)(gr * a.ldw + (gc << 3)) * 2u;
+            gr = gr < kwrows ? gr : kwrows - 1;
+            poff[p] = (uint32_t)(gr * kldw + (gc << 3)) * 2u;
         }
         if (nmine > 0)
             __builtin_amdgcn_global_load_lds((const __attribute__((address_space(1))) void*)((p < PA ? gA : gW) + (long)wave * (CK * 2) + poff[p]),
                                              (__attribute__((address_space(3))) void*)(slot + p * 1024), 16, 0, 0);
     }
-    auto issue = [&](int c, char* dst) {
+    unsigned long long* ts_ = a.ts;
+    asm("" : "+s"(ts_) : "s"(a.ts_cap), "s"(a.row_slot), "s"(a.bias), "s"(a.resid), "s"(a.ldr), "s"(a.gate), "s"(a.zg));
+    unsigned long long* ts = (ts_ && wave == 0) ? ts_ + 8 * (long)blockIdx.x : nullptr;
+    unsigned long long t_sum = 0;
+    auto issue =[&](int c, char* dst) {
         const long koff = (long)c * (CK * 2);
 #pragma unroll
         for (int p = 0; p < NPC; ++p) {
@@ -208,7 +208,7 @@
         }
     }
     __builtin_amdgcn_sched_barrier(0);
-    if (ts && lane == 0) ts[1] = __builtin_readcyclecounter();
+    if (ts && lane == 0) { const unsigned long long t1 = __builtin_readcyclecounter(); ts[0] = t_start; ts[6] = ez_stamp_tag(t_real); ts[1] = t1; }
     for (int i = 0; i < nmine; ++i) {
         {
             const bool nxt = NSL == 2 && i + 1 < nmine;
@@ -305,7 +305,7 @@
             const int col = col0 + 4 * ks_slot_of<SL>(q, ej);
             const f32x4 bb = a.bias ? op.b[q] : f32x4{0.f, 0.f, 0.f, 0.f};
             const float4 o = make_float4(v[q].x + bb[0], v[q].y + bb[1], v[q].z + bb[2], v[q].w + bb[3]);
-            if (row_ok && col < a.N) {
+            if (row_ok && col < kN) {
                 float* dst = out + (long)erow * a.ldo + col;
                 if (a.wt) st16_wt(dst, o); else *reinterpret_cast<float4*>(dst) = o;
             }
@@ -326,7 +326,7 @@
 #pragma unroll
         for (int q = 0; q < SL; ++q) {
             const int col = col0 + 4 * ks_slot_of<SL>(q, ej);
-            const bool ok = col < a.N;
+            const bool ok = col < kN;
             if constexpr (X == KS_ZIN) {
                 v[q].x = zr * fmaf(-zmu, op.g[q][0], v[q].x); v[q].y = zr * fmaf(-zmu, op.g[q][1], v[q].y);
                 v[q].z = zr * fmaf(-zmu, op.g[q][2], v[q].z); v[q].w = zr * fmaf(-zmu, op.g[q][3], v[q].w);
@@ -358,9 +358,9 @@
         }
         bf16_t* zrow = a.zu + (long)erow * a.ld_zu;
         auto store8 = [&](int col, uint2 lo, uint2 hi, bf16_t* rowp) {
-            if (!row_ok || col >= a.N) return;
+            if (!row_ok || col >= kN) return;
             bf16_t* dst = rowp + col;
-            if (col + 8 <= a.N) {
+            if (col + 8 <= kN) {
                 const float4 f = make_float4(__uint_as_float(lo.x), __uint_as_float(lo.y), __uint_as_float(hi.x), __uint_as_float(hi.y));
                 if (a.wt) st16_wt(dst, f); else *reinterpret_cast<float4*>(dst) = f;
             } else {
diff --git a/ezaudio_amd/csrc/gemm_pp.h b/ezaudio_amd/csrc/gemm_pp.h
--- a/ezaudio_amd/csrc/gemm_pp.h
+++ b/ezaudio_amd/csrc/gemm_pp.h
@@ -70,6 +70,47 @@
     tn = xn * a.bn + ln;
     z = xz * a.bz + lz;
     return tm < tilesM && tn < tilesN && z < a.splitk;
+}
+constexpr int PP_BOX_BM_MAX = 0xffff, PP_BOX_BN_MAX = 0x7ff;
+inline int pp_pack_box(int pm, int pn, int bm, int bn) { return __builtin_ctz(pm) | (__builtin_ctz(pn) << 2) | (bm << 4) | (bn << 20); }
+__device__ __forceinline__ bool tile_of_block_lead(int box, unsigned mbm, int tilesM, int tilesN, int& tm, int& tn) {
+    const int xcd = blockIdx.x & 7;
+    const int l = blockIdx.x >> 3;
+    const int lpm = box & 3, lpn = (box >> 2) & 3, bm = (box >> 4) & PP_BOX_BM_MAX, bn = (box >> 20) & PP_BOX_BN_MAX;
+    const int xm = xcd & ((1 << lpm) - 1), xn = (xcd >> lpm) & ((1 << lpn) - 1);
+    const int t1 = ez_div(l, mbm), lm = l - t1 * bm;
+    tm = xm * bm + lm;
+    tn = xn * bn + t1;
+    return tm < tilesM && tn < tilesN && t1 < bn;
+}
+constexpr int PP_PBOX_BM_MAX = 0xfff, PP_PBOX_BN_MAX = 0xff, PP_PBOX_BZ_MAX = 0x7f, PP_PBOX_S_MAX = 0x7f, PP_PBOX_K_MAX = 0xffffff;
+inline int pp_pack_box_partial(int pm, int pn, int bm, int bn, int bz, int panel) {
+    return (int)((unsigned)__builtin_ctz(pm) | ((unsigned)__builtin_ctz(pn) << 2) | ((unsigned)bm << 4) | ((unsigned)bn << 16) | ((unsigned)bz << 24) | ((unsigned)(panel != 0) << 31));
+}
+__device__ __forceinline__ bool tile_of_block_lead_partial(int box_, unsigned mbm, unsigned long long m2, int kpacked, int tilesM, int tilesN, int& tm, int& tn, int& z, int& kb, int& ke) {
+    const unsigned box = (unsigned)box_, mbn = (unsigned)m2, msplit = (unsigned)(m2 >> 32);
+    const int S = (kpacked >> 24) & PP_PBOX_S_MAX, nk = (kpacked & PP_PBOX_K_MAX) / BK;
+    const int xcd = blockIdx.x & 7, l = blockIdx.x >> 3;
+    if (box >> 31) {
+        const int G = tilesN * S;
+        const int lg = (int)(((float)l + 0.5f) * __builtin_amdgcn_rcpf((float)G)), r = l - lg * G;
+        tm = xcd + 8 * lg;
+        tn = ez_div(r, msplit);
+        z = r - tn * S;
+        if (tm >= tilesM) return false;
+    } else {
+        const int lpm = box & 3, lpn = (box >> 2) & 3, bm = (box >> 4) & PP_PBOX_BM_MAX, bn = (box >> 16) & PP_PBOX_BN_MAX, bz = (box >> 24) & PP_PBOX_BZ_MAX;
+        const int xm = xcd & ((1 << lpm) - 1), xn = (xcd >> lpm) & ((1 << lpn) - 1), xz = xcd >> (lpm + lpn);
+        const int t1 = ez_div(l, mbm), lm = l - t1 * bm;
+        const int lz = ez_div(t1, mbn), ln = t1 - lz * bn;
+        tm = xm * bm + lm;
+        tn = xn * bn + ln;
+        z = xz * bz + lz;
+        if (!(tm < tilesM && tn < tilesN && z < S)) return false;
+    }
+    if (S == 1) { kb = 0; ke = nk; }
+    else { kb = ez_div(nk * z, msplit); ke = ez_div(nk * (z + 1), msplit); }
+    return true;
 }
 __device__ __forceinline__ void panel_of_block(const GemmArgs& a, int tilesN, int& tm, int& tn, int& z) {
     const int G = tilesN * a.splitk, l = blockIdx.x >> 3;
@@ -719,7 +760,8 @@
 }
 
 template <int BM, int BN, int WM, int WN, int NS, int EPI, int SCHED, int VAR>
-__global__ __launch_bounds__(512) void k_gemm_pp(GemmArgs a) {
+__global__ __launch_bounds__(512) void k_gemm_pp(const bf16_t* kA, const bf16_t* kW, const int* kstep, int klda, int kldw, int kwrows, int kM, int kN, int kK, int kbox, unsigned kmbm,
+                                                 GemmArgs a) {
     static_assert(SCHED == 1 || SCHED == 2, "schedule");
     static_assert(WM * WN == (SCHED == 1 ? 8 : 4), "SCHED 1: 8 waves tile the block; SCHED 2: each group of 4 tiles it");
     constexpr int NT = 512, NTG = 256;
@@ -735,16 +777,9 @@
     constexpr int P0 = SCHED == 1 ? (NP + 1) / 2 : NP;
     extern __shared__ __attribute__((aligned(16))) char smem[];
 
-    int M_ = a.M;
-    asm("" : "+s"(M_) : "s"(a.A), "s"(a.W), "s"(a.lda), "s"(a.ldw), "s"(a.wrows), "s"(a.N), "s"(a.K), "s"(a.splitk), "s"(a.pm), "s"(a.pn), "s"(a.bm), "s"(a.bn), "s"(a.bz),
-        "s"(a.cur_step), "s"(a.ts), "s"(a.xcd_panel), "s"(a.row_slot), "s"(a.mbm), "s"(a.mbn), "s"(a.msplit), "s"(a.mG));
-    const int slot0 = a.cur_step ? *a.cur_step : 0;
-    const float *zG_ = a.zG, *zC_ = a.zC;
-    asm("" : "+s"(M_), "+s"(zG_), "+s"(zC_));
-    const float *rb_ = a.bias, *rg_ = a.gate, *rz_ = a.zg, *rz2_ = a.zg2;
-    if constexpr (EPI == EPI_RESID) asm("" : "+s"(M_), "+s"(rb_), "+s"(rg_), "+s"(rz_), "+s"(rz2_));
-    const float *rc_ = a.hn.rope_cos, *rs_ = a.hn.rope_sin;
-    if constexpr (EPI == EPI_QKV) asm("" : "+s"(M_), "+s"(rc_), "+s"(rs_));
+    int slot0 = 0;
+    if constexpr (EPI != EPI_PARTIAL) slot0 = kstep ? *kstep : 0;
+    const unsigned long long t_start = __builtin_readcyclecounter(), t_real = __builtin_amdgcn_s_memrealtime();
     const int tid = threadIdx.x;
     const int lane = tid & 63;
     const int wave = __builtin_amdgcn_readfirstlane(tid >> 6);
@@ -753,17 +788,14 @@
     const int wt = SCHED == 1 ? wave : wg;
     const int wm = wt / WN, wn = wt % WN;
 
-    const int tilesM = (M_ + BM - 1) / BM;
-    const int tilesN = (a.N + BN - 1) / BN;
-    int tm, tn, z;
-    if (EPI == EPI_PARTIAL && a.xcd_panel) {
-        panel_of_block(a, tilesN, tm, tn, z);
-        if (tm >= tilesM) return;
-    } else if (!tile_of_block(a, tilesM, tilesN, tm, tn, z)) return;
+    const int tilesM = (kM + BM - 1) / BM;
+    const int tilesN = (kN + BN - 1) / BN;
+    const int nk = (EPI == EPI_PARTIAL ? kK & PP_PBOX_K_MAX : kK) / BK;
+    int tm, tn, z = 0, kb = 0, ke = nk;
+    if constexpr (EPI == EPI_PARTIAL) {
+        if (!tile_of_block_lead_partial(kbox, kmbm, (unsigned long long)reinterpret_cast<uintptr_t>(kstep), kK, tilesM, tilesN, tm, tn, z, kb, ke)) return;
+    } else if (!tile_of_block_lead(kbox, kmbm, tilesM, tilesN, tm, tn)) return;
     const int row0 = tm * BM, col0 = tn * BN;
-    const int nk = a.K / BK;
-    int kb, ke;
-    ksplit_range(a, nk, z, kb, ke);
     const int nt = ke - kb;
 
     constexpr bool ZM = (VAR & 64) != 0;
@@ -772,15 +804,32 @@
     constexpr int FMR = SCHED == 1 ? FM : FM / 2;
     constexpr int NZT = ZMC ? FMR * Z_PT : 0;
     ZLaneRegs<FMR> zlr;
-    const bool z_shared_slot = a.row_slot == nullptr;
+    bool z_shared_slot = true;
     constexpr int ZNV = EPI == EPI_RESID ? ((VAR & (256 | 512)) ? 4 : 3) * (BN / 4) : 2 * (BN / 4);
-    const bool z_warm = EPI == EPI_QKV && rc_ && col0 < 2 * a.hn.H * a.hn.dh;
-    const int zx = nt >= 2 ? ((((ZMC && z_shared_slot) || EPI == EPI_RESID) && wave * 64 < ZNV) ? 1 : 0) + (z_warm ? 1 : 0) : -1;
+    bool z_warm = false;
+    int zslot = slot0;
+    int zx = -1;
+    unsigned long long* ts = nullptr;
     constexpr bool RGATE = EPI == EPI_RESID && (VAR & 64) != 0, RRES = EPI == EPI_RESID && (VAR & 128) != 0, RDUAL = EPI == EPI_RESID && (VAR & 256) != 0;
     constexpr bool RCOPY2 = EPI == EPI_RESID && (VAR & 512) != 0, RZIN = EPI == EPI_RESID && (VAR & 1024) != 0;
     static_assert(!RDUAL || (RGATE && RRES), "DUAL: the gated residual projection only");
     static_assert(!(RDUAL && RCOPY2) && !(RZIN && (RGATE || RRES || RDUAL || RCOPY2)), "forms of the residual epilogue");
-    auto z_late_load = [&]() {
+    auto z_late_load = [&](auto SITE_) {
+        long late = 0;
+        asm("; late arguments, site %1" : "+s"(late) : "n"(decltype(SITE_)::value), "s"(a.ts), "s"(a.row_slot), "s"(a.zstat_in), "s"(a.zs_stride), "s"(a.zparts), "s"(a.zt_slot_stride),
+            "s"(a.gate_slot_stride), "s"(a.zg_slot_stride), "s"(a.zG), "s"(a.zC));
+        const float *zG_ = a.zG + late, *zC_ = a.zC + late;
+        const float *rb_ = a.bias + late, *rg_ = a.gate + late, *rz_ = a.zg + late, *rz2_ = a.zg2 + late;
+        const float *rc_ = a.hn.rope_cos, *rs_ = a.hn.rope_sin;
+        if (rc_) { rc_ += late; rs_ += late; }
+        {
+            unsigned long long* ts_ = a.ts ? a.ts + late : nullptr;
+            ts = (ts_ && wave == 0) ? ts_ + 8 * (long)blockIdx.x : nullptr;
+            asm("" : "+s"(zslot));
+            z_shared_slot = a.row_slot == nullptr;
+            z_warm = EPI == EPI_QKV && rc_ && col0 < 2 * a.hn.H * a.hn.dh;
+            zx = nt >= 2 ? ((((ZMC && z_shared_slot) || EPI == EPI_RESID) && wave * 64 < ZNV) ? 1 : 0) + (z_warm ? 1 : 0) : -1;
+        }
         if constexpr (EPI == EPI_QKV) {
             const HeadNormArgs& hn = a.hn;
             if (z_warm) {
@@ -800,8 +849,8 @@
                 const int which = tid / (BN / 4), t4 = tid - which * (BN / 4);
                 int cp = col0 + 4 * t4;
                 cp = cp < a.N - 4 ? cp : a.N - 4;
-                const float* src = which == 0 ? rb_ : which == 1 ? (RGATE ? rg_ + (long)slot0 * a.gate_slot_stride : RZIN ? zG_ : rb_) : which == 2 ? rz_ + (long)slot0 * a.zg_slot_stride
-                                   : ((RDUAL || RCOPY2) ? rz2_ + (long)slot0 * a.zg2_slot_stride : rb_);
+                const float* src = which == 0 ? rb_ : which == 1 ? (RGATE ? rg_ + (long)zslot * a.gate_slot_stride : RZIN ? zG_ : rb_) : which == 2 ? rz_ + (long)zslot * a.zg_slot_stride
+                                   : ((RDUAL || RCOPY2) ? rz2_ + (long)zslot * a.zg2_slot_stride : rb_);
                 __builtin_amdgcn_global_load_lds((const __attribute__((address_space(1))) void*)(src + cp),
                                                  (__attribute__((address_space(3))) void*)(reinterpret_cast<char*>(zgc) + wave * 1024), 16, 0, 0);
             }
@@ -812,15 +861,13 @@
                 const int which = tid >= BN / 4, t4 = tid - which * (BN / 4);
                 int cp = col0 + 4 * t4;
                 cp = cp < a.N - 4 ? cp : a.N - 4;
-                __builtin_amdgcn_global_load_lds((const __attribute__((address_space(1))) void*)((which ? zC_ : zG_) + (long)slot0 * a.zt_slot_stride + cp),
+                __builtin_amdgcn_global_load_lds((const __attribute__((address_space(1))) void*)((which ? zC_ : zG_) + (long)zslot * a.zt_slot_stride + cp),
                                                  (__attribute__((address_space(3))) void*)(reinterpret_cast<char*>(zgc) + wave * 1024), 16, 0, 0);
             }
             const int frow = SCHED == 1 ? row0 + wm * TM + (lane & 15) : row0 + (wm * 2 + grp) * (TM / 2) + (lane & 15);
             z_lane_load<FMR>(a.zstat_in, a.zs_stride, a.zparts, frow, a.M - 1, lane >> 4, zlr);
         }
     };
-    unsigned long long* ts = (a.ts && wave == 0) ? a.ts + 8 * (long)blockIdx.x : nullptr;
-    if (ts && lane == 0) { ts[0] = __builtin_readcyclecounter(); ts[6] = ez_stamp_start(); }
     f32x4 acc[FM][FN];
 #pragma unroll
     for (int i = 0; i < FM; ++i)
@@ -837,17 +884,17 @@
         const int row = q >> 3, c = q & 7;
         if (p < PA) {
             int grow = row0 + row;
-            grow = grow < a.M ? grow : a.M - 1;
-            poff[i] = (uint32_t)(grow * a.lda + ((c ^ ((row >> 1) & 7)) << 3)) * 2u;
+            grow = grow < kM ? grow : kM - 1;
+            poff[i] = (uint32_t)(grow * klda + ((c ^ ((row >> 1) & 7)) << 3)) * 2u;
         } else {
             const int r2 = row - BM;
             int gr = col0 + r2;
-            gr = gr < a.wrows ? gr : a.wrows - 1;
-            poff[i] = (uint32_t)(gr * a.ldw + ((c ^ ((r2 >> 1) & 7)) << 3)) * 2u;
-        }
-    }
-    const char* gA = reinterpret_cast<const char*>(a.A) + (long)kb * (BK * 2);
-    const char* gW = reinterpret_cast<const char*>(a.W) + (long)kb * (BK * 2);
+            gr = gr < kwrows ? gr : kwrows - 1;
+            poff[i] = (uint32_t)(gr * kldw + ((c ^ ((r2 >> 1) & 7)) << 3)) * 2u;
+        }
+    }
+    const char* gA = reinterpret_cast<const char*>(kA) + (long)kb * (BK * 2);
+    const char* gW = reinterpret_cast<const char*>(kW) + (long)kb * (BK * 2);
 
     auto issue = [&](int t, auto PB_, auto PE_) {
         constexpr int PB = decltype(PB_)::value, PE = decltype(PE_)::value;
@@ -947,7 +994,7 @@
 #pragma unroll
             for (int t = 0; t < PD; ++t) {
                 if (t < nt) issue(t, IB{}, IE{});
-                if (t == 0) z_late_load();
+                if (t == 0) z_late_load(G_);
             }
             if (zx < 0) wait_vmcnt<0>(); else wait_younger_x<PG, PD - 1, NZT>((nt < PD ? nt : PD) - 1, zx);
             barrier();
@@ -970,7 +1017,7 @@
                     if (rf || t + 1 < nt) barrier();
                 }
             };
-            if (ts && lane == 0) ts[1] = __builtin_readcyclecounter();
+            if (ts && lane == 0) { const unsigned long long t1 = __builtin_readcyclecounter(); ts[0] = t_start; ts[6] = ez_stamp_tag(t_real); ts[1] = t1; }
             int t = 0;
             for (; t + PD < nt; ++t) step(t, std::true_type{});
             for (; t < nt; ++t) step(t, std::false_type{});
@@ -982,17 +1029,18 @@
         using IB = std::integral_constant<int, 0>;
         using IE = std::integral_constant<int, NP>;
         static_assert(NP * ((PD - 1) / 2 + 1) < 64, "vmcnt range");
+        static_assert(PD >= 2, "the group that does not own tile 0 runs z_late_load behind ITS first tile, K tile 1: the prologue must reach u == 1");
         auto own_younger = [&](int u) {
             const int last = u - 1 + PD < nt - 1 ? u - 1 + PD : nt - 1;
             return last >= u + 2 ? (last - u) / 2 : 0;
         };
         auto run = [&](auto G_) {
             constexpr int G = decltype(G_)::value;
-            if constexpr ((PD & 1) != G) z_late_load();
 #pragma unroll
             for (int u = 0; u < PD; ++u) {
                 if (((u + PD) & 1) == G && u < nt) issue(u, IB{}, IE{});
-                if (u == 0 && (PD & 1) == G) z_late_load();
+                if (u == 0 && (PD & 1) == G) z_late_load(G_);
+                if (u == 1 && (PD & 1) != G) z_late_load(G_);
             }
             {
                 const int last = PD - 1 < nt - 1 ? PD - 1 : nt - 1;
@@ -1023,7 +1071,7 @@
                     barrier();
                 }
             };
-            if (ts && lane == 0) ts[1] = __builtin_readcyclecounter();
+            if (ts && lane == 0) { const unsigned long long t1 = __builtin_readcyclecounter(); ts[0] = t_start; ts[6] = ez_stamp_tag(t_real); ts[1] = t1; }
             int t = G;
             for (; t + 1 + PD < nt; t += 2) step(t, std::true_type{});
             for (; t < nt; t += 2) step(t, std::false_type{});
@@ -1129,14 +1177,14 @@
             static_assert(BN == 144 || BN == 128, "EPI_QKV tiles hold two whole heads (head_dim 72 / 64)");
             static_assert(BM * (BN + 4) * 4 + BM * BN * 2 <= NS * STAGE, "epilogue tile + staging must fit the ring");
             static_assert(BM * (BN + 8) * 2 <= NS * STAGE, "bf16 staging tile must fit the ring");
-            if (a.hn.perm) pp_store_qkv_reg<BM, BN, BN / 2, HF, FN, TM / 2, TN, NT, ZM>(a, half, smem, row0, col0, ewm, lane, tid, zmr, zgc, reinterpret_cast<float*>(smem + NS * STAGE + BM * 8 + 2 * BN * 4 + 8 * 256), slot0, qop, ts);
-            else pp_store_qkv<BM, BN, BN / 2, HF, FN, TM / 2, TN, NT, ZM>(a, half, smem, row0, col0, ewm, wn, lane, tid, zmr, zgc, slot0);
+            if (a.hn.perm) pp_store_qkv_reg<BM, BN, BN / 2, HF, FN, TM / 2, TN, NT, ZM>(a, half, smem, row0, col0, ewm, lane, tid, zmr, zgc, reinterpret_cast<float*>(smem + NS * STAGE + BM * 8 + 2 * BN * 4 + 8 * 256), zslot, qop, ts);
+            else pp_store_qkv<BM, BN, BN / 2, HF, FN, TM / 2, TN, NT, ZM>(a, half, smem, row0, col0, ewm, wn, lane, tid, zmr, zgc, zslot);
         }
         if constexpr (EPI == EPI_GEGLU || EPI == EPI_PARTIAL) {
             constexpr bool lds_ok = BM * ((EPI == EPI_GEGLU ? BN / 2 : BN) + 8) * 2 <= NS * STAGE;
             if constexpr (lds_ok) {
                 if (EPI == EPI_GEGLU || a.part_bf16) {
-                    pp_store_lds<BM, BN, HF, FN, TM / 2, TN, NT, EPI, ZM>(a, half, smem, row0, col0, ewm, wn, lane, tid, z, zmr, zgc, slot0, ts);
+                    pp_store_lds<BM, BN, HF, FN, TM / 2, TN, NT, EPI, ZM>(a, half, smem, row0, col0, ewm, wn, lane, tid, z, zmr, zgc, zslot, ts);
                     if (ts && lane == 0) { ts[3] = __builtin_readcyclecounter(); ts[7] = __builtin_amdgcn_s_memrealtime(); }
                     return;
                 }
@@ -1150,13 +1198,13 @@
             static_assert(BM * (BN + 8) * 2 <= NS * STAGE, "bf16 staging tile must fit the ring");
             QkvOperands<BN / 2, FM> qop;
             qkv_request<BN / 2, FM>(a, col0, row0 + wm * TM + (lane & 15), lane, tid, qop);
-            pp_store_qkv_reg<BM, BN, BN / 2, FM, FN, TM, TN, NT, ZM>(a, acc, smem, row0, col0, wm, lane, tid, zmr, zgc, reinterpret_cast<float*>(smem + NS * STAGE + BM * 8 + 2 * BN * 4 + 8 * 256), slot0, qop, ts);
+            pp_store_qkv_reg<BM, BN, BN / 2, FM, FN, TM, TN, NT, ZM>(a, acc, smem, row0, col0, wm, lane, tid, zmr, zgc, reinterpret_cast<float*>(smem + NS * STAGE + BM * 8 + 2 * BN * 4 + 8 * 256), zslot, qop, ts);
         }
         if constexpr (EPI == EPI_GEGLU || EPI == EPI_PARTIAL) {
             constexpr bool lds_ok = BM * ((EPI == EPI_GEGLU ? BN / 2 : BN) + 8) * 2 <= NS * STAGE;
             if constexpr (lds_ok) {
                 if (EPI == EPI_GEGLU || a.part_bf16) {
-                    pp_store_lds<BM, BN, FM, FN, TM, TN, NT, EPI, ZM>(a, acc, smem, row0, col0, wm, wn, lane, tid, z, zmr, zgc, slot0, ts);
+                    pp_store_lds<BM, BN, FM, FN, TM, TN, NT, EPI, ZM>(a, acc, smem, row0, col0, wm, wn, lane, tid, z, zmr, zgc, zslot, ts);
                     if (ts && lane == 0) { ts[3] = __builtin_readcyclecounter(); ts[7] = __builtin_amdgcn_s_memrealtime(); }
                     return;
                 }
```

Result: faster. 285.5, median of 6 (+2.5%).
